# vfmatzkin/ct-unet

Measured on AMD Instinct MI355X. Metric: voxels/sec fwd+bwd, 128^3 fp32 patch, higher is better.
Workload: dtype f32; 1 GPU; UNet() default (1 in, 2 out, i_size 8, 4 blocks), 128^3 patch, batch 1 per GPU, train step = fwd + Dice/CE loss + bwd + grad all-reduce + Adam(amsgrad); patch=128, per_gpu_batch=1, parallelism=dp1, launch=hipgraph

## Files before the change

### ct-unet_amd/csrc/head_loss.hip

```cpp
#include "common.h"
#include "bn_tail.h"

namespace {

constexpr int HB = 256;
constexpr int MAXCO = 4;

struct HeadP {
    const void* in;
    const float* in_scale;
    const float* in_shift;
    const float* w;
    const float* bias;
    const int32_t* imap;
    int in_cs, in_relu, Ci, Co, act, head_mode, N;
    int64_t V;
    float gscale;
    const float* gscale_dev;
};

template <int CP, class T>
__device__ __forceinline__ void head_point(const HeadP& p, const float* sWp, const float* sB, int64_t gv,
                                           float (&a)[CP], float (&lg)[MAXCO], float (&u)[MAXCO],
                                           float (&y)[MAXCO]) {
    const T* src = reinterpret_cast<const T*>(p.in) + (size_t)gv * p.in_cs;
#pragma unroll
    for (int qd = 0; qd < CP / 4; ++qd) {
        float4 v = ld4<T>(src + qd * 4);
        if (p.in_scale) {
            const float4 sc = *reinterpret_cast<const float4*>(p.in_scale + qd * 4);
            const float4 sh = *reinterpret_cast<const float4*>(p.in_shift + qd * 4);
            v = xform4(v, sc, sh, p.in_relu);
        }
        a[qd * 4 + 0] = v.x; a[qd * 4 + 1] = v.y; a[qd * 4 + 2] = v.z; a[qd * 4 + 3] = v.w;
    }
#pragma unroll
    for (int co = 0; co < MAXCO; ++co) {
        float s = 0.f;
        if (co < p.Co) {
#pragma unroll
            for (int c = 0; c < CP; ++c) s = fmaf(a[c], sWp[co * CP + c], s);
            s += sB[co];
        }
        lg[co] = s;
    }
    if (p.act & 1) {
        float mx = -INFINITY;
#pragma unroll
        for (int co = 0; co < MAXCO; ++co) if (co < p.Co) mx = fmaxf(mx, lg[co]);
        float den = 0.f;
#pragma unroll
        for (int co = 0; co < MAXCO; ++co) { u[co] = (co < p.Co) ? expf(lg[co] - mx) : 0.f; den += u[co]; }
#pragma unroll
        for (int co = 0; co < MAXCO; ++co) u[co] /= den;
    } else {
#pragma unroll
        for (int co = 0; co < MAXCO; ++co) u[co] = lg[co];
    }
#pragma unroll
    for (int co = 0; co < MAXCO; ++co) y[co] = (p.act & 2) ? 1.f / (1.f + expf(-u[co])) : u[co];
}

template <int CP>
__device__ __forceinline__ void head_load_weights(const HeadP& p, float* sWp, float* sB) {
    for (int i = threadIdx.x; i < MAXCO * CP; i += blockDim.x) sWp[i] = 0.f;
    if (threadIdx.x < MAXCO) sB[threadIdx.x] = (threadIdx.x < p.Co && p.bias) ? p.bias[threadIdx.x] : 0.f;
    __syncthreads();
    for (int i = threadIdx.x; i < p.Co * p.Ci; i += blockDim.x) {
        const int co = i / p.Ci, ci = i % p.Ci;
        sWp[co * CP + (p.imap ? p.imap[ci] : ci)] = p.w[i];
    }
    __syncthreads();
}

__device__ __forceinline__ void softmax2(float a, float b, float& sa, float& sb) {
    const float mx = fmaxf(a, b);
    const float ea = expf(a - mx), eb = expf(b - mx);
    sa = ea / (ea + eb); sb = eb / (ea + eb);
}

template <int CP, class T>
__global__ __launch_bounds__(HB) void head_fwd_kernel(HeadP p, float* __restrict__ out0, float* __restrict__ out1) {
    __shared__ float sWp[MAXCO * CP];
    __shared__ float sB[MAXCO];
    head_load_weights<CP>(p, sWp, sB);
    const int64_t total = (int64_t)p.N * p.V;
    for (int64_t gv = (int64_t)blockIdx.x * HB + threadIdx.x; gv < total; gv += (int64_t)gridDim.x * HB) {
        float a[CP], lg[MAXCO], u[MAXCO], y[MAXCO];
        head_point<CP, T>(p, sWp, sB, gv, a, lg, u, y);
        const int64_t n = gv / p.V, v = gv % p.V;
        if (p.head_mode == 0) {
#pragma unroll
            for (int co = 0; co < MAXCO; ++co)
                if (co < p.Co) out0[(n * p.Co + co) * p.V + v] = y[co];
        } else {
            float s0 = y[0], s1 = y[1] + y[2], f0 = 1.f - y[1], f1 = y[1];
            if (p.head_mode == 2) {
                softmax2(s0, s1, s0, s1);
                softmax2(f0, f1, f0, f1);
            }
            out0[(n * 2 + 0) * p.V + v] = s0; out0[(n * 2 + 1) * p.V + v] = s1;
            out1[(n * 2 + 0) * p.V + v] = f0; out1[(n * 2 + 1) * p.V + v] = f1;
        }
    }
}

template <int CP, class T>
__global__ __launch_bounds__(HB) void head_bwd_q_kernel(HeadP p, const float* __restrict__ g0,
                                                        const float* __restrict__ g1, T* __restrict__ gin,
                                                        int gin_cs, float* __restrict__ partials,
                                                        const float* __restrict__ bn_mean, const float* __restrict__ bn_invstd,
                                                        int bn_cp, float* __restrict__ bn_partials) {
    constexpr int Q = CP / 4;
    __shared__ float sWp[MAXCO * CP];
    __shared__ float sB[MAXCO];
    __shared__ float sRed[HB / 64][MAXCO * CP + MAXCO + 2 * CP];
    head_load_weights<CP>(p, sWp, sB);
    const int qd = threadIdx.x % Q;
    const float gscale = p.gscale_dev ? p.gscale_dev[0] : p.gscale;
    float wq[MAXCO][4], dw[MAXCO][4], db[MAXCO];
#pragma unroll
    for (int co = 0; co < MAXCO; ++co) {
        db[co] = 0.f;
#pragma unroll
        for (int j = 0; j < 4; ++j) { wq[co][j] = sWp[co * CP + qd * 4 + j]; dw[co][j] = 0.f; }
    }
    float4 sc = make_float4(1.f, 1.f, 1.f, 1.f), sh = make_float4(0.f, 0.f, 0.f, 0.f);
    if (p.in_scale) {
        sc = *reinterpret_cast<const float4*>(p.in_scale + qd * 4);
        sh = *reinterpret_cast<const float4*>(p.in_shift + qd * 4);
    }
    const int xrelu = p.in_scale ? p.in_relu : 0;
    const bool bnq = bn_partials != nullptr && qd * 4 < bn_cp;
    float4 mu = make_float4(0.f, 0.f, 0.f, 0.f), is = mu, r1 = mu, r2 = mu;
    if (bnq) {
        mu = *reinterpret_cast<const float4*>(bn_mean + qd * 4);
        is = *reinterpret_cast<const float4*>(bn_invstd + qd * 4);
    }
    const int64_t total = (int64_t)p.N * p.V;
    constexpr int VPB = HB / Q;
    for (int64_t gv = (int64_t)blockIdx.x * VPB + threadIdx.x / Q; gv < total; gv += (int64_t)gridDim.x * VPB) {
        const float4 raw = ld4<T>(reinterpret_cast<const T*>(p.in) + (size_t)gv * p.in_cs + qd * 4);
        const float4 a = xform4(raw, sc, sh, xrelu);
        float lg[MAXCO], u[MAXCO], y[MAXCO], gy[MAXCO];
#pragma unroll
        for (int co = 0; co < MAXCO; ++co) {
            float s = 0.f;
            if (co < p.Co) {
                s = fmaf(a.w, wq[co][3], fmaf(a.z, wq[co][2], fmaf(a.y, wq[co][1], a.x * wq[co][0])));
#pragma unroll
                for (int o = 1; o < Q; o <<= 1) s += __shfl_xor(s, o);
                s += sB[co];
            }
            lg[co] = s;
        }
        if (p.act & 1) {
            float mx = -INFINITY;
#pragma unroll
            for (int co = 0; co < MAXCO; ++co) if (co < p.Co) mx = fmaxf(mx, lg[co]);
            float den = 0.f;
#pragma unroll
            for (int co = 0; co < MAXCO; ++co) { u[co] = (co < p.Co) ? expf(lg[co] - mx) : 0.f; den += u[co]; }
#pragma unroll
            for (int co = 0; co < MAXCO; ++co) u[co] /= den;
        } else {
#pragma unroll
            for (int co = 0; co < MAXCO; ++co) u[co] = lg[co];
        }
#pragma unroll
        for (int co = 0; co < MAXCO; ++co) y[co] = (p.act & 2) ? 1.f / (1.f + expf(-u[co])) : u[co];
        const int64_t n = gv / p.V, v = gv % p.V;
        if (p.head_mode == 0) {
#pragma unroll
            for (int co = 0; co < MAXCO; ++co) gy[co] = (co < p.Co) ? g0[(n * p.Co + co) * p.V + v] : 0.f;
        } else {
            float a0 = g0[(n * 2 + 0) * p.V + v], a1 = g0[(n * 2 + 1) * p.V + v];
            float b0 = g1[(n * 2 + 0) * p.V + v], b1 = g1[(n * 2 + 1) * p.V + v];
            if (p.head_mode == 2) {
                float s0, s1, f0, f1;
                softmax2(y[0], y[1] + y[2], s0, s1);
                softmax2(1.f - y[1], y[1], f0, f1);
                const float ds = a0 * s0 + a1 * s1, df = b0 * f0 + b1 * f1;
                a0 = s0 * (a0 - ds); a1 = s1 * (a1 - ds);
                b0 = f0 * (b0 - df); b1 = f1 * (b1 - df);
            }
            gy[0] = a0; gy[1] = a1 - b0 + b1; gy[2] = a1; gy[3] = 0.f;
        }
#pragma unroll
        for (int co = 0; co < MAXCO; ++co) gy[co] *= gscale;
        float gu[MAXCO], gl[MAXCO];
#pragma unroll
        for (int co = 0; co < MAXCO; ++co) gu[co] = (p.act & 2) ? gy[co] * y[co] * (1.f - y[co]) : gy[co];
        if (p.act & 1) {
            float dot = 0.f;
#pragma unroll
            for (int co = 0; co < MAXCO; ++co) if (co < p.Co) dot += gu[co] * u[co];
#pragma unroll
            for (int co = 0; co < MAXCO; ++co) gl[co] = (co < p.Co) ? u[co] * (gu[co] - dot) : 0.f;
        } else {
#pragma unroll
            for (int co = 0; co < MAXCO; ++co) gl[co] = (co < p.Co) ? gu[co] : 0.f;
        }
        float4 o = make_float4(0.f, 0.f, 0.f, 0.f);
        const float av[4] = {a.x, a.y, a.z, a.w};
#pragma unroll
        for (int co = 0; co < MAXCO; ++co) {
            o.x = fmaf(gl[co], wq[co][0], o.x); o.y = fmaf(gl[co], wq[co][1], o.y);
            o.z = fmaf(gl[co], wq[co][2], o.z); o.w = fmaf(gl[co], wq[co][3], o.w);
            if (qd == 0) db[co] += gl[co];
#pragma unroll
            for (int j = 0; j < 4; ++j) dw[co][j] = fmaf(gl[co], av[j], dw[co][j]);
        }
        o = rnd4<T>(o);
        st4<T>(gin + (size_t)gv * gin_cs + qd * 4, o);
        if (bnq) {
            float gz;
            gz = (fmaf(raw.x, sc.x, sh.x) > 0.f) ? o.x : 0.f; r1.x += gz; r2.x += gz * (raw.x - mu.x) * is.x;
            gz = (fmaf(raw.y, sc.y, sh.y) > 0.f) ? o.y : 0.f; r1.y += gz; r2.y += gz * (raw.y - mu.y) * is.y;
            gz = (fmaf(raw.z, sc.z, sh.z) > 0.f) ? o.z : 0.f; r1.z += gz; r2.z += gz * (raw.z - mu.z) * is.z;
            gz = (fmaf(raw.w, sc.w, sh.w) > 0.f) ? o.w : 0.f; r1.w += gz; r2.w += gz * (raw.w - mu.w) * is.w;
        }
    }
    const int lane = threadIdx.x & 63, wave = threadIdx.x >> 6;
    if (bn_partials) {
        const float rv[8] = {r1.x, r1.y, r1.z, r1.w, r2.x, r2.y, r2.z, r2.w};
#pragma unroll
        for (int j = 0; j < 8; ++j) {
            float s = rv[j];
#pragma unroll
            for (int o = 32; o >= Q; o >>= 1) s += __shfl_xor(s, o);
            if (lane < Q) sRed[wave][MAXCO * CP + MAXCO + (j >> 2) * CP + lane * 4 + (j & 3)] = s;
        }
    }
#pragma unroll
    for (int co = 0; co < MAXCO; ++co) {
#pragma unroll
        for (int j = 0; j < 4; ++j) {
            float s = dw[co][j];
#pragma unroll
            for (int o = 32; o >= Q; o >>= 1) s += __shfl_xor(s, o);
            if (lane < Q) sRed[wave][co * CP + lane * 4 + j] = s;
        }
        const float s = wave_sum(db[co]);
        if (lane == 0) sRed[wave][MAXCO * CP + co] = s;
    }
    __syncthreads();
    for (int i = threadIdx.x; i < MAXCO * CP + MAXCO; i += HB) {
        float s = 0.f;
#pragma unroll
        for (int w = 0; w < HB / 64; ++w) s += sRed[w][i];
        partials[(size_t)blockIdx.x * (MAXCO * CP + MAXCO) + i] = s;
    }
    if (bn_partials)
        for (int i = threadIdx.x; i < 2 * bn_cp; i += HB) {
            const int col = MAXCO * CP + MAXCO + (i / bn_cp) * CP + i % bn_cp;
            float s = 0.f;
#pragma unroll
            for (int w = 0; w < HB / 64; ++w) s += sRed[w][col];
            bn_partials[(size_t)blockIdx.x * 2 * bn_cp + i] = s;
        }
}

template <int CP>
__global__ __launch_bounds__(HB) void head_bwd_final_kernel(const float* __restrict__ partials, int nb, int Ci, int Co,
                                                            const int32_t* __restrict__ imap, float* __restrict__ dw,
                                                            float* __restrict__ db, const float* __restrict__ bn_partials,
                                                            int bn_cp, ctu_bn_bwd_tail tail) {
    const int i = blockIdx.x;
    if (i == Co * Ci + Co) {
        bn_bwd_finalize_rows(tail, bn_partials, nb, bn_cp);
        return;
    }
    const int row = MAXCO * CP + MAXCO;
    int col;
    if (i < Co * Ci) {
        const int co = i / Ci, ci = i % Ci;
        col = co * CP + (imap ? imap[ci] : ci);
    } else {
        col = MAXCO * CP + (i - Co * Ci);
    }
    __shared__ double r[HB];
    double s = 0.0;
    for (int b = threadIdx.x; b < nb; b += HB) s += (double)partials[(size_t)b * row + col];
    r[threadIdx.x] = s;
    __syncthreads();
    for (int o = HB / 2; o > 0; o >>= 1) {
        if (threadIdx.x < o) r[threadIdx.x] += r[threadIdx.x + o];
        __syncthreads();
    }
    if (threadIdx.x == 0) {
        if (i < Co * Ci) dw[i] = (float)r[0];
        else db[i - Co * Ci] = (float)r[0];
    }
}

inline int head_blocks(int64_t total) {
    int64_t nb = ceil_div64(total, HB);
    if (nb > 2048) nb = 2048;
    return (int)(nb < 1 ? 1 : nb);
}

constexpr int LOSS_BX = 1024;

__global__ __launch_bounds__(HB) void loss_fwd_kernel(const float* __restrict__ pred, const float* __restrict__ tgt,
                                                      int64_t V, int dice_softmax, float* __restrict__ ws) {
    const int n = blockIdx.y;
    const float* p0 = pred + (size_t)n * 2 * V;
    const float* p1 = p0 + V;
    const float* t0 = tgt + (size_t)n * 2 * V;
    const float* t1 = t0 + V;
    float ce = 0.f, num = 0.f, d1 = 0.f, d2 = 0.f;
    auto point = [&](float a, float b, float ta, float tb) {
        const float mx = fmaxf(a, b);
        const float ea = expf(a - mx), eb = expf(b - mx);
        const float lse = mx + logf(ea + eb);
        ce += lse - ((tb > ta) ? b : a);
        float pa = a, pb = b;
        if (dice_softmax) { pa = ea / (ea + eb); pb = eb / (ea + eb); }
        num += pa * ta + pb * tb;
        d1 += pa * pa + pb * pb;
        d2 += ta * ta + tb * tb;
    };
    const bool vec = (V & 3) == 0 && ((reinterpret_cast<uintptr_t>(pred) | reinterpret_cast<uintptr_t>(tgt)) & 15) == 0;
    if (vec) {
        const int64_t V4 = V >> 2;
        for (int64_t q = (int64_t)blockIdx.x * HB + threadIdx.x; q < V4; q += (int64_t)gridDim.x * HB) {
            const float4 a = reinterpret_cast<const float4*>(p0)[q], b = reinterpret_cast<const float4*>(p1)[q];
            const float4 ta = reinterpret_cast<const float4*>(t0)[q], tb = reinterpret_cast<const float4*>(t1)[q];
            point(a.x, b.x, ta.x, tb.x); point(a.y, b.y, ta.y, tb.y); point(a.z, b.z, ta.z, tb.z); point(a.w, b.w, ta.w, tb.w);
        }
    } else {
        for (int64_t v = (int64_t)blockIdx.x * HB + threadIdx.x; v < V; v += (int64_t)gridDim.x * HB) point(p0[v], p1[v], t0[v], t1[v]);
    }
    __shared__ float red[HB / 64][4];
    const int lane = threadIdx.x & 63, wave = threadIdx.x >> 6;
    ce = wave_sum(ce); num = wave_sum(num); d1 = wave_sum(d1); d2 = wave_sum(d2);
    if (lane == 0) { red[wave][0] = ce; red[wave][1] = num; red[wave][2] = d1; red[wave][3] = d2; }
    __syncthreads();
    if (threadIdx.x < 4) {
        float s = 0.f;
#pragma unroll
        for (int w = 0; w < HB / 64; ++w) s += red[w][threadIdx.x];
        ws[((size_t)n * gridDim.x + blockIdx.x) * 4 + threadIdx.x] = s;
    }
}

__global__ void loss_final_kernel(float* __restrict__ ws, int N, int nbx, int64_t V, float ce_lambda,
                                  float dice_lambda, float* __restrict__ terms) {
    if (blockIdx.x != 0) return;
    const int lane = threadIdx.x;
    const double eps = 0.0000001;
    double ce = 0.0, dsum = 0.0;
    float* tail = ws + (size_t)N * nbx * 4;
    for (int n = 0; n < N; ++n) {
        double c = 0.0, num = 0.0, d1 = 0.0, d2 = 0.0;
        for (int b = lane; b < nbx; b += 64) {
            const float4 r = *reinterpret_cast<const float4*>(ws + ((size_t)n * nbx + b) * 4);
            c += r.x; num += r.y; d1 += r.z; d2 += r.w;
        }
#pragma unroll
        for (int o = 32; o > 0; o >>= 1) {
            c += __shfl_xor(c, o); num += __shfl_xor(num, o); d1 += __shfl_xor(d1, o); d2 += __shfl_xor(d2, o);
        }
        ce += c;
        dsum += (num + eps) / (d1 + d2 + eps);
        if (lane == 0) {
            tail[n * 2 + 0] = (float)(num + eps);
            tail[n * 2 + 1] = (float)(d1 + d2 + eps);
        }
    }
    if (lane == 0) {
        terms[0] = ce_lambda != 0.f ? (float)(ce_lambda * ce / ((double)N * (double)V)) : 0.f;
        terms[1] = dice_lambda != 0.f ? (float)(dice_lambda * (1.0 - 2.0 * dsum / N)) : 0.f;
    }
}

__global__ __launch_bounds__(HB) void loss_bwd_kernel(const float* __restrict__ pred, const float* __restrict__ tgt,
                                                      int N, int64_t V, float ce_lambda, float dice_lambda,
                                                      int dice_softmax, const float* __restrict__ tail,
                                                      const float* __restrict__ gscale_ce,
                                                      const float* __restrict__ gscale_dice, float* __restrict__ gpred,
                                                      int accumulate) {
    const int n = blockIdx.y;
    const float gs_ce = gscale_ce ? gscale_ce[0] : 1.f, gs_d = gscale_dice ? gscale_dice[0] : 1.f;
    const float kce = gs_ce * ce_lambda / ((float)N * (float)V);
    const float nume = tail[n * 2 + 0], dene = tail[n * 2 + 1];
    const float kd = gs_d * dice_lambda * (-2.f / (float)N);
    const float kd_t = kd / dene, kd_p = kd * nume * 2.f / (dene * dene);
    const size_t base = (size_t)n * 2 * V;
    auto point = [&](float a, float b, float ta, float tb, float& ga, float& gb) {
        const float mx = fmaxf(a, b);
        const float ea = expf(a - mx), eb = expf(b - mx);
        const float sa = ea / (ea + eb), sb = eb / (ea + eb);
        const bool cls1 = tb > ta;
        ga = kce * (sa - (cls1 ? 0.f : 1.f));
        gb = kce * (sb - (cls1 ? 1.f : 0.f));
        if (dice_lambda != 0.f) {
            const float pa = dice_softmax ? sa : a, pb = dice_softmax ? sb : b;
            float da = kd_t * ta - kd_p * pa, db = kd_t * tb - kd_p * pb;
            if (dice_softmax) {
                const float dot = da * sa + db * sb;
                da = sa * (da - dot); db = sb * (db - dot);
            }
            ga += da; gb += db;
        }
    };
    const bool vec = (V & 3) == 0 && ((reinterpret_cast<uintptr_t>(pred) | reinterpret_cast<uintptr_t>(tgt) | reinterpret_cast<uintptr_t>(gpred)) & 15) == 0;
    if (vec) {
        const int64_t V4 = V >> 2;
        const float4* a4 = reinterpret_cast<const float4*>(pred + base);
        const float4* b4 = reinterpret_cast<const float4*>(pred + base + V);
        const float4* ta4 = reinterpret_cast<const float4*>(tgt + base);
        const float4* tb4 = reinterpret_cast<const float4*>(tgt + base + V);
        float4* ga4 = reinterpret_cast<float4*>(gpred + base);
        float4* gb4 = reinterpret_cast<float4*>(gpred + base + V);
        for (int64_t q = (int64_t)blockIdx.x * HB + threadIdx.x; q < V4; q += (int64_t)gridDim.x * HB) {
            const float4 a = a4[q], b = b4[q], ta = ta4[q], tb = tb4[q];
            float4 ga, gb;
            point(a.x, b.x, ta.x, tb.x, ga.x, gb.x); point(a.y, b.y, ta.y, tb.y, ga.y, gb.y);
            point(a.z, b.z, ta.z, tb.z, ga.z, gb.z); point(a.w, b.w, ta.w, tb.w, ga.w, gb.w);
            if (accumulate) {
                const float4 oa = ga4[q], ob = gb4[q];
                ga.x += oa.x; ga.y += oa.y; ga.z += oa.z; ga.w += oa.w; gb.x += ob.x; gb.y += ob.y; gb.z += ob.z; gb.w += ob.w;
            }
            ga4[q] = ga; gb4[q] = gb;
        }
        return;
    }
    for (int64_t v = (int64_t)blockIdx.x * HB + threadIdx.x; v < V; v += (int64_t)gridDim.x * HB) {
        float ga, gb;
        point(pred[base + v], pred[base + V + v], tgt[base + v], tgt[base + V + v], ga, gb);
        if (accumulate) { ga += gpred[base + v]; gb += gpred[base + V + v]; }
        gpred[base + v] = ga;
        gpred[base + V + v] = gb;
    }
}

}

static int fill_head(HeadP& p, const void* in, int in_cs, int cin_p, const float* in_scale, const float* in_shift,
                     int in_relu, const float* w, const float* bias, const int32_t* imap, int Ci, int Co, int act,
                     int head_mode, int N, int64_t V, const char* name) {
    CTU_REQUIRE(in && w, "%s: null pointer", name);
    CTU_REQUIRE(cin_p == 8 || cin_p == 16 || cin_p == 32, "%s: cin_p=%d unsupported (8, 16 or 32)", name, cin_p);
    CTU_REQUIRE(Co >= 1 && Co <= MAXCO && Ci >= 1 && Ci <= cin_p, "%s: Co=%d Ci=%d", name, Co, Ci);
    CTU_REQUIRE(head_mode == 0 || Co == 3, "%s: SP re-encoding needs 3 output channels", name);
    CTU_REQUIRE(head_mode >= 0 && head_mode <= 2, "%s: head_mode=%d", name, head_mode);
    CTU_REQUIRE(in_cs >= cin_p && in_cs % 4 == 0, "%s: bad stride", name);
    CTU_REQUIRE((in_scale == nullptr) == (in_shift == nullptr), "%s: scale/shift must come together", name);
    p.in = in; p.in_scale = in_scale; p.in_shift = in_shift; p.w = w; p.bias = bias; p.imap = imap;
    p.in_cs = in_cs; p.in_relu = in_relu; p.Ci = Ci; p.Co = Co; p.act = act; p.head_mode = head_mode; p.N = N; p.V = V; p.gscale = 1.f;
    p.gscale_dev = nullptr;
    return CTU_OK;
}

namespace {

template <class T>
int head_fwd_impl(const T* in, int in_cs, int cin_p, const float* in_scale, const float* in_shift, int in_relu, const float* w,
                  const float* bias, const int32_t* imap, int Ci, int Co, int act, int head_mode, float* out0, float* out1, int N,
                  int64_t nvox_per_item, void* stream) {
    HeadP p;
    int rc = fill_head(p, in, in_cs, cin_p, in_scale, in_shift, in_relu, w, bias, imap, Ci, Co, act, head_mode, N,
                       nvox_per_item, "head_fwd");
    if (rc != CTU_OK) return rc;
    CTU_REQUIRE(out0 && (head_mode == 0 || out1), "head_fwd: null output");
    const int nb = head_blocks((int64_t)N * nvox_per_item);
    hipStream_t st = (hipStream_t)stream;
    if (cin_p == 8) head_fwd_kernel<8, T><<<nb, HB, 0, st>>>(p, out0, out1);
    else if (cin_p == 16) head_fwd_kernel<16, T><<<nb, HB, 0, st>>>(p, out0, out1);
    else head_fwd_kernel<32, T><<<nb, HB, 0, st>>>(p, out0, out1);
    CTU_CHECK_LAUNCH("head_fwd");
    return CTU_OK;
}

template <class T>
int head_bwd_impl(const T* in, int in_cs, int cin_p, const float* in_scale, const float* in_shift, int in_relu, const float* w,
                  const float* bias, const int32_t* imap, int Ci, int Co, int act, int head_mode, const float* g0, const float* g1,
                  T* gin, int gin_cs, float* dw, float* db, float* ws, int N, int64_t nvox_per_item, const float* bn_mean,
                  const float* bn_invstd, int bn_cp, float* bn_partials, const ctu_bn_bwd_tail* tail, void* stream, float gscale = 1.f,
                  const float* gscale_dev = nullptr) {
    CTU_REQUIRE(!tail || (bn_partials && tail->gamma && tail->invstd && tail->dgamma && tail->dbeta && tail->coef &&
                          tail->C > 0 && tail->C <= bn_cp && tail->count > 0 && (!tail->running_mean || (tail->mean && tail->running_var))),
                "head_bwd: incomplete BatchNorm tail");
    HeadP p;
    int rc = fill_head(p, in, in_cs, cin_p, in_scale, in_shift, in_relu, w, bias, imap, Ci, Co, act, head_mode, N,
                       nvox_per_item, "head_bwd");
    if (rc != CTU_OK) return rc;
    p.gscale = gscale;
    p.gscale_dev = gscale_dev;
    CTU_REQUIRE(g0 && (head_mode == 0 || g1) && gin && dw && db && ws, "head_bwd: null pointer");
    CTU_REQUIRE(gin_cs >= cin_p && gin_cs % 4 == 0, "head_bwd: bad gin stride");
    CTU_REQUIRE(!bn_partials || (bn_mean && bn_invstd && in_scale && in_relu && bn_cp > 0 && bn_cp % 4 == 0 && bn_cp <= cin_p),
                "head_bwd: the BatchNorm reduction needs mean/invstd, a BN+ReLU input transform and bn_cp <= cin_p (bn_cp=%d)", bn_cp);
    const int nb = head_blocks((int64_t)N * nvox_per_item);
    hipStream_t st = (hipStream_t)stream;
    const int nfin = Co * Ci + Co + (tail ? 1 : 0);
    const ctu_bn_bwd_tail tl = bwd_tail_or_off(tail);
    if (cin_p == 8) {
        head_bwd_q_kernel<8, T><<<nb, HB, 0, st>>>(p, g0, g1, gin, gin_cs, ws, bn_mean, bn_invstd, bn_cp, bn_partials);
        head_bwd_final_kernel<8><<<nfin, HB, 0, st>>>(ws, nb, Ci, Co, imap, dw, db, bn_partials, bn_cp, tl);
    } else if (cin_p == 16) {
        head_bwd_q_kernel<16, T><<<nb, HB, 0, st>>>(p, g0, g1, gin, gin_cs, ws, bn_mean, bn_invstd, bn_cp, bn_partials);
        head_bwd_final_kernel<16><<<nfin, HB, 0, st>>>(ws, nb, Ci, Co, imap, dw, db, bn_partials, bn_cp, tl);
    } else {
        head_bwd_q_kernel<32, T><<<nb, HB, 0, st>>>(p, g0, g1, gin, gin_cs, ws, bn_mean, bn_invstd, bn_cp, bn_partials);
        head_bwd_final_kernel<32><<<nfin, HB, 0, st>>>(ws, nb, Ci, Co, imap, dw, db, bn_partials, bn_cp, tl);
    }
    CTU_CHECK_LAUNCH("head_bwd");
    return CTU_OK;
}

}

extern "C" int ctu_head_fwd(const float* in, int in_cs, int cin_p, const float* in_scale, const float* in_shift,
                            int in_relu, const float* w, const float* bias, const int32_t* imap, int Ci, int Co, int act,
                            int head_mode, float* out0, float* out1, int N, int64_t nvox_per_item, void* stream) {
    return head_fwd_impl<float>(in, in_cs, cin_p, in_scale, in_shift, in_relu, w, bias, imap, Ci, Co, act, head_mode, out0, out1, N,
                                nvox_per_item, stream);
}
extern "C" int ctu_lp_head_fwd(int dtype, const void* in, int in_cs, int cin_p, const float* in_scale, const float* in_shift,
                               int in_relu, const float* w, const float* bias, const int32_t* imap, int Ci, int Co, int act,
                               int head_mode, float* out0, float* out1, int N, int64_t nvox_per_item, void* stream) {
    CTU_DISPATCH_LP(dtype, return head_fwd_impl<T>((const T*)in, in_cs, cin_p, in_scale, in_shift, in_relu, w, bias, imap, Ci, Co, act,
                                                   head_mode, out0, out1, N, nvox_per_item, stream));
}

extern "C" size_t ctu_head_bwd_ws_floats(int N, int64_t nvox_per_item, int cin_p, int Co) {
    (void)Co;
    return (size_t)head_blocks((int64_t)N * nvox_per_item) * (MAXCO * cin_p + MAXCO);
}

extern "C" int ctu_head_bwd_num_blocks(int N, int64_t nvox_per_item) { return head_blocks((int64_t)N * nvox_per_item); }

extern "C" int ctu_head_bwd(const float* in, int in_cs, int cin_p, const float* in_scale, const float* in_shift,
                            int in_relu, const float* w, const float* bias, const int32_t* imap, int Ci, int Co, int act,
                            int head_mode, const float* g0, const float* g1, float* gin, int gin_cs, float* dw,
                            float* db, float* ws, int N, int64_t nvox_per_item, void* stream) {
    return head_bwd_impl<float>(in, in_cs, cin_p, in_scale, in_shift, in_relu, w, bias, imap, Ci, Co, act, head_mode, g0, g1, gin,
                                gin_cs, dw, db, ws, N, nvox_per_item, nullptr, nullptr, 0, nullptr, nullptr, stream);
}

extern "C" int ctu_head_bwd_bn(const float* in, int in_cs, int cin_p, const float* in_scale, const float* in_shift,
                               int in_relu, const float* w, const float* bias, const int32_t* imap, int Ci, int Co, int act,
                               int head_mode, const float* g0, const float* g1, float* gin, int gin_cs, float* dw,
                               float* db, float* ws, int N, int64_t nvox_per_item, const float* bn_mean,
                               const float* bn_invstd, int bn_cp, float* bn_partials, const ctu_bn_bwd_tail* tail, void* stream) {
    return head_bwd_impl<float>(in, in_cs, cin_p, in_scale, in_shift, in_relu, w, bias, imap, Ci, Co, act, head_mode, g0, g1, gin,
                                gin_cs, dw, db, ws, N, nvox_per_item, bn_mean, bn_invstd, bn_cp, bn_partials, tail, stream);
}
extern "C" int ctu_lp_head_bwd_bn(int dtype, const void* in, int in_cs, int cin_p, const float* in_scale, const float* in_shift,
                                  int in_relu, const float* w, const float* bias, const int32_t* imap, int Ci, int Co, int act,
                                  int head_mode, const float* g0, const float* g1, void* gin, int gin_cs, float* dw,
                                  float* db, float* ws, int N, int64_t nvox_per_item, const float* bn_mean,
                                  const float* bn_invstd, int bn_cp, float* bn_partials, const ctu_bn_bwd_tail* tail, float gscale,
                                  void* stream) {
    CTU_DISPATCH_LP(dtype, return head_bwd_impl<T>((const T*)in, in_cs, cin_p, in_scale, in_shift, in_relu, w, bias, imap, Ci, Co, act,
                                                   head_mode, g0, g1, (T*)gin, gin_cs, dw, db, ws, N, nvox_per_item, bn_mean,
                                                   bn_invstd, bn_cp, bn_partials, tail, stream, gscale));
}

extern "C" int ctu_lp_head_bwd_bn_dscale(int dtype, const void* in, int in_cs, int cin_p, const float* in_scale,
                                         const float* in_shift, int in_relu, const float* w, const float* bias, const int32_t* imap,
                                         int Ci, int Co, int act, int head_mode, const float* g0, const float* g1, void* gin,
                                         int gin_cs, float* dw, float* db, float* ws, int N, int64_t nvox_per_item,
                                         const float* bn_mean, const float* bn_invstd, int bn_cp, float* bn_partials,
                                         const ctu_bn_bwd_tail* tail, const float* gscale, void* stream) {
    CTU_REQUIRE(gscale, "lp_head_bwd_bn_dscale: null gscale");
    CTU_DISPATCH_LP(dtype, return head_bwd_impl<T>((const T*)in, in_cs, cin_p, in_scale, in_shift, in_relu, w, bias, imap, Ci, Co, act,
                                                   head_mode, g0, g1, (T*)gin, gin_cs, dw, db, ws, N, nvox_per_item, bn_mean,
                                                   bn_invstd, bn_cp, bn_partials, tail, stream, 1.f, gscale));
}

extern "C" size_t ctu_loss_ws_floats(int N, int64_t V) {
    (void)V;
    return (size_t)N * LOSS_BX * 4 + (size_t)N * 2;
}

extern "C" int ctu_loss_fwd(const float* pred, const float* target, int N, int64_t V, float ce_lambda,
                            float dice_lambda, int dice_softmax, float* terms, float* ws, void* stream) {
    CTU_REQUIRE(pred && target && terms && ws && N > 0 && V > 0, "loss_fwd: bad argument");
    hipStream_t st = (hipStream_t)stream;
    loss_fwd_kernel<<<dim3(LOSS_BX, N), HB, 0, st>>>(pred, target, V, dice_softmax, ws);
    CTU_CHECK_LAUNCH("loss_fwd");
    loss_final_kernel<<<1, 64, 0, st>>>(ws, N, LOSS_BX, V, ce_lambda, dice_lambda, terms);
    CTU_CHECK_LAUNCH("loss_final");
    return CTU_OK;
}

extern "C" int ctu_loss_bwd(const float* pred, const float* target, int N, int64_t V, float ce_lambda,
                            float dice_lambda, int dice_softmax, const float* ws, const float* gscale_ce,
                            const float* gscale_dice, float* gpred, int accumulate, void* stream) {
    CTU_REQUIRE(pred && target && ws && gpred && N > 0 && V > 0, "loss_bwd: bad argument");
    loss_bwd_kernel<<<dim3(LOSS_BX, N), HB, 0, (hipStream_t)stream>>>(pred, target, N, V, ce_lambda, dice_lambda,
                                                                      dice_softmax, ws + (size_t)N * LOSS_BX * 4,
                                                                      gscale_ce, gscale_dice, gpred, accumulate);
    CTU_CHECK_LAUNCH("loss_bwd");
    return CTU_OK;
}
```

### ct-unet_amd/ctunet_amd/_lib.py

```python
from __future__ import annotations

import ctypes as C
import os

import torch

_HERE = os.path.dirname(os.path.abspath(__file__))
LIB_PATH = os.environ.get("CTUNET_HIP_LIB") or os.path.join(_HERE, "libctunet_hip.so")

P = C.c_void_p
I = C.c_int
L = C.c_int64
F = C.c_float
D = C.c_double
Z = C.c_size_t
U = C.c_uint64

class PackJob(C.Structure):
    _fields_ = [("w", C.c_void_p), ("wp", C.c_void_p), ("cinv", C.c_void_p), ("kind", C.c_int), ("Co", C.c_int),
                ("Ci", C.c_int), ("k", C.c_int), ("rin_p", C.c_int), ("nout_p", C.c_int), ("mode", C.c_int),
                ("layout", C.c_int)]


class BnTail(C.Structure):
    _fields_ = [("gamma", C.c_void_p), ("beta", C.c_void_p), ("running_mean", C.c_void_p), ("running_var", C.c_void_p),
                ("scale", C.c_void_p), ("shift", C.c_void_p), ("mean", C.c_void_p), ("invstd", C.c_void_p),
                ("num_batches_tracked", C.c_void_p), ("counter", C.c_void_p), ("count", C.c_double),
                ("momentum", C.c_float), ("eps", C.c_float), ("C", C.c_int), ("n_updates", C.c_int)]


class BnBwdTail(C.Structure):
    _fields_ = [("gamma", C.c_void_p), ("invstd", C.c_void_p), ("dgamma", C.c_void_p), ("dbeta", C.c_void_p),
                ("coef", C.c_void_p), ("mean", C.c_void_p), ("running_mean", C.c_void_p), ("running_var", C.c_void_p),
                ("num_batches_tracked", C.c_void_p), ("counter", C.c_void_p), ("count", C.c_double),
                ("momentum", C.c_float), ("eps", C.c_float), ("C", C.c_int)]


class WgradJob(C.Structure):
    _fields_ = [("ws", C.c_void_p), ("dw", C.c_void_p), ("db", C.c_void_p), ("cinv", C.c_void_p), ("kind", C.c_int),
                ("Co", C.c_int), ("Ci", C.c_int), ("cin_p", C.c_int), ("n_ci_g", C.c_int), ("gx", C.c_int),
                ("pairs", C.c_int), ("nmf", C.c_int)]


class SegLossCfg(C.Structure):
    _fields_ = [("ce_lambda", C.c_float), ("dice_lambda", C.c_float), ("tversky_lambda", C.c_float),
                ("boundary_lambda", C.c_float), ("w0", C.c_float), ("w1", C.c_float), ("focal_gamma", C.c_float),
                ("tversky_alpha", C.c_float), ("tversky_beta", C.c_float), ("dice_softmax", C.c_int)]


WGRAD_JOBS_MAX = 4

SIGNATURES = {
    "ctu_last_error": (C.c_char_p, []),
    "ctu_abi_version": (I, []),
    "ctu_arch": (C.c_char_p, []),
    "ctu_ncdhw_to_ndhwc": (I, [P, P, I, I, I, I, I, I, I, P]),
    "ctu_ndhwc_to_ncdhw": (I, [P, P, I, I, I, I, I, I, P]),
    "ctu_conv3d_layout": (I, [I, I, I]),
    "ctu_conv3d_fwd_kernel_name": (C.c_char_p, [I, I, I, I, I, I, I]),
    "ctu_conv3d_wgrad_kernel_name": (C.c_char_p, [I, I, I, I]),
    "ctu_conv3d_packed_floats": (Z, [I, I, I, I]),
    "ctu_conv3d_num_blocks": (I, [I, I, I, I, I, I, I]),
    "ctu_pack_conv3d_weight": (I, [P, P, I, I, I, P, I, I, I, I, P]),
    "ctu_pack_batch": (I, [P, I, P]),
    "ctu_conv3d_fwd": (I, [P, I, I, P, P, I, P, P, I, P, I, I, P, I, I, I, I, I, I, P, P]),
    "ctu_conv3d_wgrad_ws_floats": (Z, [I, I, I, I, I, I, I]),
    "ctu_conv3d_wgrad": (I, [P, I, I, P, P, I, P, I, I, P, P, I, I, P, P, I, I, I, I, I, P]),
    "ctu_conv3d_wgrad_bn_supported": (I, [I, I, I, I, I, I, I]),
    "ctu_conv3d_wgrad_bn": (I, [P, I, I, P, P, I, P, I, I, P, P, P, P, P, P, I, I, P, P, I, I, I, I, I, P]),
    "ctu_conv3d_first_supported": (I, [I, I, I, I]),
    "ctu_conv3d_first_num_blocks": (I, [I, I, I, I]),
    "ctu_conv3d_first_fwd": (I, [P, I, P, P, I, P, I, I, P, I, I, I, I, P, P]),
    "ctu_conv3d_first_bwd_data": (I, [P, I, P, I, I, P, I, I, I, I, P]),
    "ctu_conv3d_first_wgrad_ws_floats": (Z, [I, I, I, I, I]),
    "ctu_conv3d_first_wgrad": (I, [P, I, P, I, P, I, P, I, I, I, I, P]),
    "ctu_conv3d_first_wgrad_bn": (I, [P, I, P, I, P, P, P, P, P, P, I, P, I, I, I, I, P]),
    "ctu_bn_finalize": (I, [P, I, I, I, D, P, P, P, P, F, F, I, P, P, P, P, P, P]),
    "ctu_bn_eval_affine": (I, [P, P, P, P, F, I, I, P, P, P]),
    "ctu_bn_bwd_num_blocks": (I, [L]),
    "ctu_bn_relu_bwd_reduce": (I, [P, I, P, I, I, P, P, P, P, L, P, P, P]),
    "ctu_bn_bwd_finalize": (I, [P, I, I, I, D, P, P, P, P, P, P, P, P, F, F, P, P]),
    "ctu_bn_relu_bwd_apply": (I, [P, I, P, I, I, P, P, P, P, P, L, P]),
    "ctu_conv3d_wgrad_slabs": (I, [P, I, I, P, P, I, P, I, I, P, P, I, I, P, P, I, I, I, I, I, P, P]),
    "ctu_conv3d_wgrad_bn_slabs": (I, [P, I, I, P, P, I, P, I, I, P, P, P, P, P, P, I, I, P, P, I, I, I, I, I, P, P]),
    "ctu_conv3d_first_wgrad_slabs": (I, [P, I, P, I, P, I, P, I, I, I, I, P, P]),
    "ctu_conv3d_first_wgrad_bn_slabs": (I, [P, I, P, I, P, P, P, P, P, P, I, P, I, I, I, I, P, P]),
    "ctu_convt2_wgrad_slabs": (I, [P, I, I, P, P, I, P, I, I, P, P, I, I, P, P, I, I, I, I, P, P]),
    "ctu_bn_bwd_finalize_jobs": (I, [P, I, I, I, D, P, P, P, P, P, P, P, P, F, F, P, P, I, P]),
    "ctu_wgrad_reduce_jobs": (I, [P, I, P]),
    "ctu_maxpool2_fwd": (I, [P, I, I, P, P, I, P, I, I, I, I, I, P]),
    "ctu_maxpool2_bwd": (I, [P, I, I, P, P, I, P, I, P, I, I, I, I, I, I, P]),
    "ctu_maxpool2_bwd_bn_num_blocks": (I, [I, I, I, I, I]),
    "ctu_maxpool2_bwd_bn": (I, [P, I, I, P, P, P, P, P, I, P, I, I, I, I, I, I, P, P, P]),
    "ctu_convt_packed_floats": (Z, [I, I]),
    "ctu_pack_convt_weight": (I, [P, P, I, I, P, I, I, I, P]),
    "ctu_convt2_fwd": (I, [P, I, I, P, P, I, P, P, I, P, I, I, I, I, I, I, P]),
    "ctu_convt2_bwd_data": (I, [P, I, I, P, P, I, I, I, I, I, I, P]),
    "ctu_convt2_wgrad_ws_floats": (Z, [I, I, I, I, I, I]),
    "ctu_convt2_wgrad": (I, [P, I, I, P, P, I, P, I, I, P, P, I, I, P, P, I, I, I, I, P]),
    "ctu_convt2_plan": (C.c_char_p, [I, I, I, I, I, I, I, P]),
    "ctu_convt2_wgrad_plan": (C.c_char_p, [I, I, I, I, I, I, P]),
    "ctu_head_fwd": (I, [P, I, I, P, P, I, P, P, P, I, I, I, I, P, P, I, L, P]),
    "ctu_head_bwd_ws_floats": (Z, [I, L, I, I]),
    "ctu_head_bwd": (I, [P, I, I, P, P, I, P, P, P, I, I, I, I, P, P, P, I, P, P, P, I, L, P]),
    "ctu_head_bwd_num_blocks": (I, [I, L]),
    "ctu_head_bwd_bn": (I, [P, I, I, P, P, I, P, P, P, I, I, I, I, P, P, P, I, P, P, P, I, L, P, P, I, P, P, P]),
    "ctu_loss_ws_floats": (Z, [I, L]),
    "ctu_loss_fwd": (I, [P, P, I, L, F, F, I, P, P, P]),
    "ctu_loss_bwd": (I, [P, P, I, L, F, F, I, P, P, P, P, I, P]),
    "ctu_seg_loss_ws_floats": (Z, [I, L]),
    "ctu_seg_loss_fwd": (I, [P, P, P, I, L, P, P, P, P]),
    "ctu_seg_loss_bwd": (I, [P, P, P, I, L, P, P, P, P, P, P, P, I, P]),
    "ctu_skip_add": (I, [P, I, P, P, I, P, I, P, P, I, P, I, I, L, P]),
    "ctu_upconv_fused_supported": (I, [I, I, I, I, I, I]),
    "ctu_upconv_fused_packed_floats": (Z, [I, I]),
    "ctu_upconv_fused_num_blocks": (I, [I, I, I, I, I]),
    "ctu_upconv_fused_pack_ws_floats": (Z, [I, I]),
    "ctu_upconv_fused_pack": (I, [P, P, P, I, I, P, I, I, P, P, P, P]),
    "ctu_upconv_fused_pack_all": (I, [P, P, P, I, I, P, I, I, P, P, P, P, P]),
    "ctu_upconv_fused_fwd": (I, [P, I, I, P, P, I, P, P, P, I, I, P, I, I, I, I, P, P]),
    "ctu_upconv_fused_wgrad_ws_floats": (Z, [I, I, I, I, I, I]),
    "ctu_upconv_fused_wgrad": (I, [P, I, I, P, P, I, P, I, I, P, P, I, I, I, I, P]),
    "ctu_upconv_fused_wgrad_bn_supported": (I, [I, I, I, I, I, I]),
    "ctu_upconv_fused_wgrad_bn": (I, [P, I, I, P, P, I, P, I, I, P, P, P, P, P, P, P, I, I, I, I, P]),
    "ctu_upconv_fused_project_ws_floats": (Z, [I, L]),
    "ctu_upconv_fused_project": (I, [P, P, I, I, I, I, I, I, P, P, P, I, I, I, P, P, P, P, P]),
    "ctu_upconv_fused_bwd_packed_floats": (Z, [I, I]),
    "ctu_upconv_fused_pack_bwd": (I, [P, I, I, P, P]),
    "ctu_upconv_fused_bwd_data": (I, [P, I, I, P, P, I, I, I, I, I, I, P]),
    "ctu_hard_segm": (I, [P, I, I, L, P, P]),
    "ctu_one_hot": (I, [P, I, I, L, P, P]),
    "ctu_hard_dice_ws_doubles": (Z, [I]),
    "ctu_hard_dice_counts": (I, [P, P, I, I, L, P, P, P]),
    "ctu_hausdorff_ws_bytes": (Z, [I, I, I, I, I]),
    "ctu_hausdorff": (I, [P, P, I, I, I, I, I, P, P, P]),
    "ctu_surface_ws_bytes": (Z, [I, I, I, I, I]),
    "ctu_surface_metrics": (I, [P, I, I, P, I, I, I, I, I, I, I, I, I, P, P, D, P, P, P]),
    "ctu_components_ws_bytes": (Z, [I, I, I, I]),
    "ctu_label_components": (I, [P, I, I, I, I, I, I, P, I, P, P, P, P]),
    "ctu_filter_components": (I, [P, I, I, I, I, I, I, P, I, I, I, P, P, P]),
    "ctu_morphology_ws_bytes": (Z, [I, I, I, I, I]),
    "ctu_binary_morphology": (I, [P, I, I, I, I, I, I, C.c_uint32, I, I, I, L, P, P, P]),
    "ctu_fill_holes": (I, [P, I, I, I, I, I, I, I, L, P, P, P]),
    "ctu_implant_mask": (I, [P, I, P, I, I, I, I, I, C.c_uint32, I, I, I, I, P, P, P]),
    "ctu_distance_ws_bytes": (Z, [I, I, I, I, I, I]),
    "ctu_distance_transform": (I, [P, I, I, I, I, I, I, L, I, I, P, I, P, P, F, P, P]),
    "ctu_thickness_ws_bytes": (Z, [I, I, I, I, I]),
    "ctu_local_thickness": (I, [P, I, I, I, I, I, P, P, P, P]),
    "ctu_thickness_summary_ws_bytes": (Z, [I, L]),
    "ctu_thickness_summary": (I, [P, I, L, F, P, P, P]),
    "ctu_resample": (I, [P, I, I, I, L, I, I, I, I, I, I, P, P, P, P, P]),
    "ctu_affine_resample": (I, [P, I, I, I, L, I, I, I, I, I, I, P, P, P, P, P, D, P, P]),
    "ctu_registration_ws_bytes": (Z, [L]),
    "ctu_registration_init": (I, [P, L, P, P, P]),
    "ctu_registration_accumulate": (I, [P, L, P, I, I, I, P, P, D, P, P]),
    "ctu_registration_update": (I, [L, I, P, P, P, I, P, P]),
    "ctu_mesh_ws_bytes": (Z, [I, I, I]),
    "ctu_mesh_count": (I, [P, I, I, I, I, I, L, F, P, P]),
    "ctu_mesh_emit": (I, [P, I, I, I, I, F, F, P, P, L, L, P, P, P, P]),
    "ctu_mesh_measure": (I, [P, L, P, L, P, P, P, P]),
    "ctu_mesh_adjacency_ws_bytes": (Z, [L, L]),
    "ctu_mesh_adjacency_build": (I, [P, L, L, P, P, P]),
    "ctu_mesh_adjacency_emit": (I, [L, L, L, P, P, P, P]),
    "ctu_mesh_smooth_ws_bytes": (Z, [L]),
    "ctu_mesh_smooth": (I, [P, L, P, P, L, P, I, F, I, F, P, P, P]),
    "ctu_mesh_voxelize_ws_bytes": (Z, [I, I, I]),
    "ctu_mesh_voxelize": (I, [P, L, P, L, I, I, I, P, P, I, P, P, P]),
    "ctu_mesh_grid_ws_bytes": (Z, [L, L]),
    "ctu_mesh_grid_build": (I, [P, L, P, L, F, L, P, P, P]),
    "ctu_mesh_grid_emit": (I, [P, L, L, L, L, P, P, P, P]),
    "ctu_mesh_distance": (I, [P, L, P, P, L, P, I, I, I, P, L, I, I, I, P, P, F, F, P, P, P, P]),
    "ctu_mesh_decimate_ws_bytes": (Z, [L, L, L]),
    "ctu_mesh_decimate_bounds": (I, [P, L, P, L, P, P]),
    "ctu_mesh_decimate_build": (I, [P, L, P, L, P, P, P, L, I, P, P]),
    "ctu_mesh_decimate_emit": (I, [P, L, L, L, L, P, P, P, P, P, P, P]),
    "ctu_gaussian_ws_bytes": (Z, [L, I, I, I, I]),
    "ctu_gaussian_filter": (I, [P, I, L, I, I, I, P, P, I, F, P, P, P]),
    "ctu_minmax_ws_bytes": (Z, [L]),
    "ctu_finite_minmax": (I, [P, I, L, P, P, P]),
    "ctu_histogram": (I, [P, I, L, I, P, D, D, P, P]),
    "ctu_threshold_otsu": (I, [P, I, P, D, D, P, P, P]),
    "ctu_binarize": (I, [P, I, L, P, D, P, D, P, P]),
    "ctu_extract_patches": (I, [P, P, I, I, I, I, I, I, I, I, P, P]),
    "ctu_stitch_patches": (I, [P, P, I, I, I, I, I, I, I, I, P, P]),
    "ctu_window_accumulate": (I, [P, P, P, P, I, I, I, I, I, I, I, I, P, P, P, F, I, I, I, P, P, P]),
    "ctu_window_finalize": (I, [P, P, I, L, P, P, P]),
    "ctu_extract_patches_flip": (I, [P, P, P, I, I, I, I, I, I, I, I, P, P]),
    "ctu_window_accumulate_flip": (I, [P, P, P, P, P, I, I, I, I, I, I, I, I, P, P, P, F, I, I, I, P, P, P, P, P]),
    "ctu_window_finalize_stats": (I, [P, P, P, P, I, L, P, P, P, P, P, P]),
    "ctu_flap_count": (I, [P, I, I, L, P, P]),
    "ctu_flap_draw": (I, [P, I, I, I, I, I, P, I, P, U, F, I, I, I, P, P, U, F, F, I, P, P]),
    "ctu_flap_apply": (I, [P, I, P, I, I, I, I, P, I, P, P, P, U, I, P, I, P, P, P]),
    "ctu_spatial_draw": (I, [I, I, I, I, P, P, U, I, D, D, D, P, I, I, I, I, P, P, P]),
    "ctu_spatial_warp": (I, [P, I, I, I, I, I, I, P, I, I, I, P, P, P, P, P]),
    "ctu_lp_upconv_fused_supported": (I, [I, I, I, I, I, I]),
    "ctu_lp_upconv_fused_packed_elems": (Z, [I]),
    "ctu_lp_upconv_fused_num_blocks": (I, [I, I, I, I]),
    "ctu_lp_upconv_fused_pack": (I, [I, P, I, P, P]),
    "ctu_lp_upconv_fused_fwd": (I, [I, P, I, I, P, P, I, P, P, P, I, P, I, I, I, I, P]),
    "ctu_lp_upconv_fused_wgrad_ws_floats": (Z, [I, I, I, I, I]),
    "ctu_lp_upconv_fused_wgrad": (I, [I, P, I, I, P, P, I, P, I, P, P, I, I, I, I, P]),
    "ctu_lp_upconv_fused_wgrad_bn_supported": (I, [I, I, I, I, I]),
    "ctu_lp_upconv_fused_wgrad_bn": (I, [I, P, I, I, P, P, I, P, I, P, P, P, P, P, P, P, I, I, I, I, P]),
    "ctu_lp_conv3d_wgrad_bn_supported": (I, [I, I, I, I, I, I, I]),
    "ctu_lp_conv3d_wgrad_bn": (I, [I, P, I, I, P, P, I, P, I, I, P, P, P, P, P, P, I, I, P, P, I, I, I, I, I, P]),
    "ctu_lp_upconv_fused_project": (I, [I, P, P, I, I, I, I, I, I, P, P, P, I, I, I, P, P, P, P, P]),
    "ctu_lp_upconv_fused_bwd_data": (I, [I, P, I, P, P, I, I, I, I, I, I, P]),
    "ctu_lp_conv3d_layout": (I, [I, I, I, I]),
    "ctu_lp_conv3d_packed_elems": (Z, [I, I, I]),
    "ctu_lp_conv3d_num_blocks": (I, [I, I, I, I, I, I, I, I]),
    "ctu_lp_pack_conv3d_weight": (I, [I, P, P, I, I, I, P, I, I, I, I, P]),
    "ctu_lp_pack_batch": (I, [I, P, I, P]),
    "ctu_lp_conv3d_fwd": (I, [I, P, I, I, P, P, I, P, P, I, P, I, I, P, I, I, I, I, I, I, P, P]),
    "ctu_lp_conv3d_wgrad_ws_floats": (Z, [I, I, I, I, I, I, I]),
    "ctu_lp_conv3d_wgrad": (I, [I, P, I, I, P, P, I, P, I, I, P, I, I, P, P, I, I, I, I, I, P]),
    "ctu_lp_conv3d_first_fwd": (I, [I, P, I, P, P, I, P, I, I, P, I, I, I, I, P, P]),
    "ctu_lp_conv3d_first_bwd_data": (I, [I, P, I, P, I, I, P, I, I, I, I, P]),
    "ctu_lp_conv3d_first_bwd_data_pair_supported": (I, [I, I]),
    "ctu_lp_conv3d_fwd_kernel_name": (C.c_char_p, [I, I, I, I, I, I, I, I]),
    "ctu_lp_conv3d_wgrad_kernel_name": (C.c_char_p, [I, I, I, I, I, I]),
    "ctu_lp_conv3d_first_bwd_data_pair": (I, [I, P, I, P, I, P, I, I, I, I, P]),
    "ctu_lp_conv3d_first_wgrad": (I, [I, P, I, P, I, P, I, P, I, I, I, I, P]),
    "ctu_lp_convt_packed_elems": (Z, [I, I, I]),
    "ctu_lp_pack_convt_weight": (I, [I, P, P, I, I, P, I, I, I, P]),
    "ctu_lp_convt2_fwd": (I, [I, P, I, I, P, P, I, P, P, I, P, I, I, I, I, I, I, P]),
    "ctu_lp_convt2_bwd_data": (I, [I, P, I, I, P, P, I, I, I, I, I, I, P]),
    "ctu_lp_convt2_wgrad_ws_floats": (Z, [I, I, I, I, I, I]),
    "ctu_lp_convt2_wgrad": (I, [I, P, I, I, P, P, I, P, I, I, P, I, I, P, P, I, I, I, I, P]),
    "ctu_lp_convt2_plan": (C.c_char_p, [I, I, I, I, I, I, I, P]),
    "ctu_lp_convt2_wgrad_plan": (C.c_char_p, [I, I, I, I, I, I, P]),
    "ctu_lp_ncdhw_to_ndhwc": (I, [I, P, P, I, I, I, I, I, I, I, P]),
    "ctu_lp_ndhwc_to_ncdhw": (I, [I, P, P, I, I, I, I, I, I, P]),
    "ctu_lp_bn_relu_bwd_reduce": (I, [I, P, I, P, I, I, P, P, P, P, L, P, P, P]),
    "ctu_lp_bn_relu_bwd_apply": (I, [I, P, I, P, I, I, P, P, P, P, P, L, P]),
    "ctu_lp_maxpool2_fwd": (I, [I, P, I, I, P, P, I, P, I, I, I, I, I, P]),
    "ctu_lp_maxpool2_bwd": (I, [I, P, I, I, P, P, I, P, I, P, I, I, I, I, I, I, P]),
    "ctu_lp_maxpool2_bwd_bn": (I, [I, P, I, I, P, P, P, P, P, I, P, I, I, I, I, I, I, P, P, P]),
    "ctu_lp_skip_add": (I, [I, P, I, P, P, I, P, I, P, P, I, P, I, I, L, P]),
    "ctu_lp_channel_sum": (I, [I, P, I, I, L, P, P, I, P]),
    "ctu_lp_head_fwd": (I, [I, P, I, I, P, P, I, P, P, P, I, I, I, I, P, P, I, L, P]),
    "ctu_lp_head_bwd_bn": (I, [I, P, I, I, P, P, I, P, P, P, I, I, I, I, P, P, P, I, P, P, P, I, L, P, P, I, P, P, F, P]),
    "ctu_lp_head_bwd_bn_dscale": (I, [I, P, I, I, P, P, I, P, P, P, I, I, I, I, P, P, P, I, P, P, P, I, L, P, P, I, P, P, P, P]),
    "ctu_scale_tensors": (I, [P, P, I, F, P, P]),
    "ctu_unscale_tensors": (I, [P, P, I, P, P, P]),
    "ctu_loss_scale_update": (I, [P, P, P, P, F, F, I, P]),
    "ctu_comm_available": (I, []),
    "ctu_comm_unique_id": (I, [P]),
    "ctu_comm_init": (I, [C.POINTER(C.c_void_p), I, I, P]),
    "ctu_comm_allreduce_f32": (I, [P, P, P, Z, I, P]),
    "ctu_comm_destroy": (I, [P]),
    "ctu_channel_sum_num_blocks": (I, [L]),
    "ctu_channel_sum": (I, [P, I, I, L, P, P, I, P]),
    "ctu_adam_amsgrad": (I, [P, P, I, P, D, D, D, D, D, I, P, P]),
    "ctu_adam_amsgrad_dev": (I, [P, P, I, P, P, D, D, D, D, I, P, P, P]),
    "ctu_grad_norm_num_blocks": (I, [P, I]),
    "ctu_grad_clip_coef": (I, [P, P, I, F, P, P, P, P]),
    "ctu_plateau_update": (I, [P, P, P, P, I, I, D, I, D, I, D, D, P]),
    "ctu_sgd": (I, [P, P, I, P, P, D, D, D, D, I, I, P, P, P]),
    "ctu_rmsprop": (I, [P, P, I, P, P, D, D, D, D, D, I, I, P, P, P]),
}

_lib = None
ABI_VERSION = 8


class CtuError(RuntimeError):
    """A libctunet_hip.so entry point returned a non-zero status."""


def load() -> C.CDLL:
    global _lib
    if _lib is not None:
        return _lib
    if not os.path.exists(LIB_PATH):
        raise ImportError(
            f"{LIB_PATH} not found: the MI355X kernels are not built. Run `python __graft_entry__.py` "
            "(or `make -C ct-unet_amd/csrc`). There is no CPU fallback for this path.")
    lib = C.CDLL(LIB_PATH)
    for name, (res, args) in SIGNATURES.items():
        try:
            fn = getattr(lib, name)
        except AttributeError as e:
            raise ImportError(f"{LIB_PATH} does not export {name}; rebuild the library") from e
        fn.restype = res
        fn.argtypes = args
    if lib.ctu_abi_version() != ABI_VERSION:
        raise ImportError(f"{LIB_PATH} is ABI v{lib.ctu_abi_version()}, this package binds v{ABI_VERSION}: "
                          "a stale build -- run `python __graft_entry__.py` (or `make -C ct-unet_amd/csrc`)")
    _lib = lib
    return lib


def check(status: int, what: str) -> None:
    if status != 0:
        msg = load().ctu_last_error().decode("utf-8", "replace")
        raise CtuError(f"{what} failed (status {status}): {msg}")


DTYPE_CODE = {torch.float32: 0, torch.uint8: 3, torch.bool: 3, torch.int64: 4, torch.int16: 5, torch.int32: 6}


class on(torch.cuda.device):

    def __init__(self, device: torch.device):
        super().__init__(device.index)

    def __enter__(self):
        super().__enter__()
        self._stream = torch.cuda.current_stream().cuda_stream
        return self._run

    def _run(self, name: str, *args, what: str = None) -> None:
        status = getattr(_lib or load(), name)(*args, self._stream)
        if status:
            check(status, what or name[4:])


def check_device(message: str, *tensors) -> None:
    for t in tensors:
        if not t.is_cuda:
            raise ValueError(message)


def as_bytes(t):
    t = t.contiguous()
    return t.view(torch.uint8) if t.dtype == torch.bool else t


def array(ctype, values):
    if values is None:
        return None
    values = list(values)
    return (ctype * len(values))(*values)


def float_array(values):
    return array(C.c_float, values)


def double_array(values):
    return array(C.c_double, values)
```

### ct-unet_amd/ctunet_amd/engine.py

```python
from __future__ import annotations

import os
from dataclasses import dataclass
from typing import Dict, List, Optional, Tuple

import torch

from . import ops
from .ops import CL, pad8

BN_EPS = 1e-5
FUSE_UP = os.environ.get("CTUNET_FUSE_UP", "1") != "0"
FUSE_UP_MAX_CO = int(os.environ.get("CTUNET_FUSE_UP_MAXCO", "16"))
POOL_BN = os.environ.get("CTUNET_POOL_BN", "1") != "0"
LP_FUSE_UP = os.environ.get("CTUNET_LP_FUSE_UP", "1") != "0"
BN_MOMENTUM = 0.1
LAZY_BN = os.environ.get("CTUNET_LAZY_BN", "1") != "0"
LAZY_BN_LP = os.environ.get("CTUNET_LAZY_BN_LP", "0") != "0"
BN_TAIL = os.environ.get("CTUNET_BN_TAIL", "0") != "0"
DEFER_WGRAD_REDUCE = os.environ.get("CTUNET_DEFER_WGRAD_REDUCE", "1") != "0"


@dataclass
class BlockPlan:
    prefix: str
    first: int
    cin: int
    cout: int


@dataclass
class NetPlan:
    k: int
    conv_bias: bool
    in_ch: int
    out_ch: int
    enc: List[BlockPlan]
    center: BlockPlan
    center_live: bool
    dec: List[BlockPlan]
    head: str
    act: int
    head_mode: int
    skip: str = "cat"


@dataclass(slots=True)
class _ConvRec:
    x: Optional[CL]
    y: CL
    vec: torch.Tensor
    stats: Optional[torch.Tensor]
    nblk: int
    conv: str
    bn: str
    cin: int
    cout: int
    imap: Optional[torch.Tensor]
    bias: bool
    first: Optional[torch.Tensor] = None


class _WgradWs:

    def __init__(self, floats: int, device, defer: bool):
        self.jobs = ops.WgradJobs() if defer else None
        self.bufs = [torch.empty(floats, dtype=torch.float32, device=device) for _ in range(2 if defer else 1)]
        self.i = 0

    def take(self) -> torch.Tensor:
        self.i = (self.i + 1) % len(self.bufs)
        ws = self.bufs[self.i]
        if self.jobs is not None:
            if self.jobs.uses(ws):
                self.jobs.flush()
            assert not self.jobs.uses(ws)
        return ws

    def flush(self) -> None:
        if self.jobs is not None:
            self.jobs.flush()


class UNetEngine:
    def __init__(self, plan: NetPlan, dtype: torch.dtype = torch.float32, loss_scale: Optional[float] = None):
        if dtype not in ops.ACT_DTYPES:
            raise ValueError(f"ctunet_amd: activation dtype {dtype} not supported (float32, bfloat16, float16)")
        self.plan = plan
        self.dtype = dtype
        self.loss_scale = loss_scale
        self.scaler = None
        self._pack_cache: Dict[Tuple, Tuple[int, torch.Tensor]] = {}
        self._replay_stats = False
        self._up_cache: Dict[str, Tuple] = {}
        self._imaps: Dict[Tuple, torch.Tensor] = {}
        self._tail_words: Dict[str, torch.Tensor] = {}
        self._tail_slots: Dict[Tuple[str, str], int] = {}
        self._overflow: Dict[str, torch.Tensor] = {}
        self._gy_bufs: Dict[int, Tuple[torch.Tensor, torch.Tensor]] = {}

    def overflow_flag(self, device) -> torch.Tensor:
        f = self._overflow.get(str(device))
        if f is None:
            f = self._overflow[str(device)] = torch.zeros(1, dtype=torch.float32, device=device)
        return f

    def _counter(self, layer: str, direction: str, device) -> Optional[torch.Tensor]:
        if not BN_TAIL:
            return None
        words = self._tail_words.get(str(device))
        if words is None:
            words = self._tail_words[str(device)] = torch.zeros(1024, dtype=torch.int32, device=device)
        slot = self._tail_slots.setdefault((layer, direction), len(self._tail_slots))
        if slot >= words.numel():
            raise RuntimeError("ctunet_amd: more than 1024 BatchNorm tails in one engine")
        return words[slot:slot + 1]

    def _maps(self, segs: Tuple[Tuple[int, int], ...], cp: int, device):
        idx: List[int] = []
        for n, start in segs:
            idx += list(range(start, start + n))
        if idx == list(range(len(idx))):
            return None, None
        key = (segs, cp, str(device))
        t = self._imaps.get(key)
        if t is None:
            inv = [-1] * cp
            for logical, pos in enumerate(idx):
                inv[pos] = logical
            t = (torch.tensor(idx, dtype=torch.int32, device=device), torch.tensor(inv, dtype=torch.int32, device=device))
            self._imaps[key] = t
        return t

    def _packed(self, name: str, w: torch.Tensor, kind: str, imap, rin_p: int, nout_p: int, mode: int,
                layout: int = 0) -> torch.Tensor:
        key = (name, kind, mode, rin_p, nout_p, layout, self.dtype)
        hit = self._pack_cache.get(key)
        ver = (w._version, w.data_ptr())
        if hit is not None and hit[0] == ver:
            return hit[1]
        wd = w.detach()
        if self.dtype != torch.float32:
            wp = self._pack_lp(kind, wd, imap, rin_p, nout_p, mode, hit[1] if hit is not None else None, layout)
        else:
            wp = hit[1] if hit is not None else torch.empty(ops.packed_floats(kind, w.shape[2], rin_p, nout_p, layout),
                                                            dtype=torch.float32, device=w.device)
            ops.pack_batch([(kind, wd.contiguous(), wp, imap, rin_p, nout_p, mode, layout)], self.dtype)
        self._pack_cache[key] = (ver, wp, imap)
        return wp

    def _pack_lp(self, kind, wd, imap, rin_p, nout_p, mode, into, layout=0):
        if kind == "conv":
            return ops.pack_conv_w_lp(wd, imap, rin_p, nout_p, mode, self.dtype, into, layout)
        return ops.pack_convt_w_lp(wd, imap, rin_p, nout_p, mode, self.dtype, into)

    def refresh_packs(self, P: Dict[str, torch.Tensor]) -> None:
        force = P and next(iter(P.values())).is_cuda and torch.cuda.is_current_stream_capturing()
        jobs = []
        for key, ent in self._pack_cache.items():
            name, kind, mode, rin_p, nout_p, layout, dt = key
            w = P.get(name + ".weight")
            if w is None or w.device != ent[1].device or dt != self.dtype:
                continue
            ver = (w._version, w.data_ptr())
            if force or ent[0] != ver:
                jobs.append((kind, w.detach().contiguous(), ent[1], ent[2], rin_p, nout_p, mode, layout))
                self._pack_cache[key] = (ver, ent[1], ent[2])
        ops.pack_batch(jobs, self.dtype)

    def invalidate_packs(self) -> None:
        for key, ent in self._pack_cache.items():
            self._pack_cache[key] = (None,) + tuple(ent[1:])
        for prefix, hit in self._up_cache.items():
            self._up_cache[prefix] = (None,) + tuple(hit[1:])

    def _fwd_tail(self, P, bn: str, c: int, nvox: int, n_upd: int, vec4: torch.Tensor, device):
        counter = self._counter(bn, "fwd", device)
        if counter is None:
            return None
        return ops.make_bn_tail(c, nvox, P[bn + ".weight"], P[bn + ".bias"], P[bn + ".running_mean"], P[bn + ".running_var"],
                                BN_MOMENTUM, BN_EPS, n_upd, vec4, P.get(bn + ".num_batches_tracked") if n_upd else None,
                                counter)

    def _bn_stage(self, P, bn: str, out: CL, vec4: torch.Tensor, nvox: int, c: int, training: bool, n_upd: int, nblk: int,
                  launch, tail_ok: bool = True) -> Tuple[CL, Optional[torch.Tensor]]:
        wb = (P[bn + ".weight"], P[bn + ".bias"], P[bn + ".running_mean"], P[bn + ".running_var"])
        if training:
            stats = torch.empty((nblk, 2, out.cp), dtype=torch.float32, device=out.buf.device)
            tail = self._fwd_tail(P, bn, c, nvox, n_upd, vec4, out.buf.device) if tail_ok else None
            launch(stats, tail)
            if tail is None:
                ops.bn_finalize_into(stats, nblk, c, out.cp, nvox, *wb, BN_MOMENTUM, BN_EPS, n_upd, vec4,
                                     P.get(bn + ".num_batches_tracked") if n_upd else None)
        else:
            stats = None
            launch(None, None)
            ops.bn_eval_affine_into(*wb, BN_EPS, c, out.cp, vec4)
        return out.with_xf(vec4[0], vec4[1], True), stats

    def _conv_bn(self, P, x: CL, conv: str, bn: str, cin: int, cout: int, imap, out: CL, vec4: torch.Tensor,
                 training: bool, n_upd: int, save: bool) -> Tuple[CL, Optional[_ConvRec]]:
        k = self.plan.k
        w = P[conv + ".weight"]
        bias = P.get(conv + ".bias")
        lay = ops.conv_layout(k, out.cp, x.dims[3], self.dtype, x.cp)
        if bias is not None and self.dtype != torch.float32:
            lay = 0
        wp = self._packed(conv, w, "conv", imap, x.cp, out.cp, 0, lay)
        bias_p = None if bias is None else bias.detach()
        nblk = ops.conv_num_blocks(x.dims, out.cp, lay, k, self.dtype, x.cp) if training else 0
        y, stats = self._bn_stage(P, bn, out, vec4, x.nvox, cout, training, n_upd, nblk,
                                  lambda stats, tail: ops.conv3d_fwd(x, wp, bias_p, out, k, stats, (cin, cout), lay, tail))
        rec = _ConvRec(x, out.raw(), vec4, stats, nblk, conv, bn, cin, cout, imap, bias is not None) if save else None
        return y, rec

    def _fuse_up(self, x: CL, nout_p: int) -> bool:
        if not (self.plan.k == 3 and not self.plan.conv_bias and nout_p <= FUSE_UP_MAX_CO and FUSE_UP):
            return False
        if self.dtype == torch.float32:
            return ops.upconv_fused_supported(x.dims, 3, x.cp, nout_p)
        return LP_FUSE_UP and ops.lp_upconv_fused_supported(x.dims, 3, x.cp, nout_p)

    def _upconv_bn(self, P, x: CL, prefix: str, ct: int, cout: int, cinv, out: CL, vec4: torch.Tensor, training: bool,
                   n_upd: int, save: bool) -> Tuple[CL, Optional[_ConvRec]]:
        conv, bn = f"{prefix}.1", f"{prefix}.2"
        wt, bt, w3 = P[f"{prefix}.0.weight"], P[f"{prefix}.0.bias"], P[conv + ".weight"]
        lp = bool(x.lp)
        ver = tuple((t._version, t.data_ptr()) for t in (wt, bt, w3))
        hit = self._up_cache.get(prefix)
        if hit is None or hit[0] != ver or hit[3] != (x.cp, out.cp, self.dtype) or torch.cuda.is_current_stream_capturing():
            same = hit is not None and hit[3] == (x.cp, out.cp, self.dtype)
            if lp:
                wp, beff, pws = ops.upconv_fused_pack(wt, bt, w3, cinv, x.cp, out.cp, (hit[1], hit[2], hit[4]) if same else None)
                wpd = ops.lp_upconv_fused_pack(wp, x.cp, self.dtype, hit[5] if same else None)
            else:
                wp, beff, pws, wpd = ops.upconv_fused_pack_all(wt, bt, w3, cinv, x.cp, out.cp,
                                                               (hit[1], hit[2], hit[4], hit[5]) if same else None)
            self._up_cache[prefix] = (ver, wp, beff, (x.cp, out.cp, self.dtype), pws, wpd)
        else:
            wp, beff, wpd = hit[1], hit[2], hit[5]
        if lp:
            nblk = ops.lp_upconv_fused_num_blocks(x.dims) if training else 0
            launch = lambda stats, tail: ops.lp_upconv_fused_fwd(x, wpd, beff, out, stats, (ct, cout))
        else:
            nblk = ops.upconv_fused_num_blocks(x.dims, out.cp) if training else 0
            launch = lambda stats, tail: ops.upconv_fused_fwd(x, wp, beff, out, stats, (ct, cout), tail)
        y, stats = self._bn_stage(P, bn, out, vec4, 8 * x.nvox, cout, training, n_upd, nblk, launch, tail_ok=not lp)
        rec = _ConvRec(None, out.raw(), vec4, stats, nblk, conv, bn, ct, cout, None, False) if save else None
        return y, rec

    def _first_conv_bn(self, P, x: torch.Tensor, conv: str, bn: str, cin: int, cout: int, out: CL, vec4: torch.Tensor,
                       training: bool, n_upd: int, save: bool):
        w = P[conv + ".weight"].detach()
        bias = P.get(conv + ".bias")
        bias_p = None if bias is None else bias.detach()
        nblk = ops.conv_first_num_blocks(out.dims) if training else 0
        y, stats = self._bn_stage(P, bn, out, vec4, out.nvox, cout, training, n_upd, nblk,
                                  lambda stats, tail: ops.conv_first_fwd(x, w, bias_p, out, stats, tail))
        rec = _ConvRec(None, out.raw(), vec4, stats, nblk, conv, bn, cin, cout, None, bias is not None, x) if save else None
        return y, rec

    def forward(self, P: Dict[str, torch.Tensor], x: torch.Tensor, training: bool, save: bool, chk: bool):
        plan = self.plan
        dev = x.device
        n, cin, d, h, w = x.shape
        nlev = len(plan.enc)
        if cin != plan.in_ch:
            raise RuntimeError(f"ctunet_amd: expected {plan.in_ch} input channels, got {cin}")
        if any(s % (1 << nlev) for s in (d, h, w)):
            raise RuntimeError(f"ctunet_amd: spatial size {(d, h, w)} must be divisible by {1 << nlev}")
        if training and n * (d >> nlev) * (h >> nlev) * (w >> nlev) <= 1:
            raise ValueError("Expected more than 1 value per channel when training (centre block)")
        ctx = {"recs": {}, "levels": [], "training": training, "chk": chk} if save else None
        n_upd = 1 if training else 0
        self.refresh_packs(P)

        x = x.contiguous()
        e0 = plan.enc[0]
        first_direct = plan.conv_bias is False and ops.conv_first_supported(plan.k, cin, pad8(e0.cout), w)
        adt = self.dtype
        cur = None if first_direct else ops.ncdhw_to_cl(x, dtype=adt)
        x_cl = cur
        cat: List[torch.Tensor] = []
        xf: List[torch.Tensor] = []
        pooled: List[CL] = []
        dskip: List[CL] = []
        dd, hh, ww = d, h, w
        recs = {}
        xf_sizes = [8 * pad8(blk.cout) for blk in plan.enc]
        xf_all = torch.zeros(sum(xf_sizes), dtype=torch.float32, device=dev)
        xf_off = 0
        for i, blk in enumerate(plan.enc):
            cp = pad8(blk.cout)
            cat.append(torch.empty((n, dd, hh, ww, 2 * cp), dtype=adt, device=dev))
            xf.append(xf_all[xf_off:xf_off + 8 * cp].view(4, 2 * cp))
            xf_off += 8 * cp
            t1 = CL(torch.empty((n, dd, hh, ww, cp), dtype=adt, device=dev), 0, cp)
            v1 = torch.empty((4, cp), dtype=torch.float32, device=dev)
            imap = None
            if i == 0 and first_direct:
                a1, recs[(blk.prefix, 1)] = self._first_conv_bn(P, x, f"{blk.prefix}.{blk.first}",
                                                                f"{blk.prefix}.{blk.first + 1}", blk.cin, blk.cout, t1,
                                                                v1, training, n_upd, save)
            else:
                a1, recs[(blk.prefix, 1)] = self._conv_bn(P, cur, f"{blk.prefix}.{blk.first}",
                                                          f"{blk.prefix}.{blk.first + 1}", blk.cin, blk.cout, imap, t1,
                                                          v1, training, n_upd, save)
            a2, recs[(blk.prefix, 2)] = self._conv_bn(P, a1, f"{blk.prefix}.{blk.first + 3}", f"{blk.prefix}.{blk.first + 4}",
                                                      blk.cout, blk.cout, None, CL(cat[i], cp, cp), xf[i][:, cp:],
                                                      training, n_upd, save)
            dskip.append(a2)
            dd, hh, ww = dd // 2, hh // 2, ww // 2
            pl = CL(torch.empty((n, dd, hh, ww, cp), dtype=adt, device=dev), 0, cp)
            ops.maxpool_fwd(a2, pl)
            pooled.append(pl)
            cur = pl
        cb = plan.center
        cpc = pad8(cb.cout)
        center_out = None
        if plan.center_live or training:
            live = plan.center_live
            c1 = CL(torch.empty((n, dd, hh, ww, cpc), dtype=adt, device=dev), 0, cpc)
            c2 = CL(torch.empty((n, dd, hh, ww, cpc), dtype=adt, device=dev), 0, cpc)
            v1 = torch.empty((4, cpc), dtype=torch.float32, device=dev)
            v2 = torch.empty((4, cpc), dtype=torch.float32, device=dev)
            a1, r1 = self._conv_bn(P, cur, f"{cb.prefix}.{cb.first}", f"{cb.prefix}.{cb.first + 1}", cb.cin, cb.cout,
                                   None, c1, v1, training, n_upd, save and live)
            a2, r2 = self._conv_bn(P, a1, f"{cb.prefix}.{cb.first + 3}", f"{cb.prefix}.{cb.first + 4}", cb.cout, cb.cout,
                                   None, c2, v2, training, n_upd, save and live)
            if live:
                recs[(cb.prefix, 1)], recs[(cb.prefix, 2)] = r1, r2
                center_out = a2
        cur = center_out if plan.center_live else pooled[-1]
        cur_segs = ((cb.cout if plan.center_live else plan.enc[-1].cout, 0),)
        dec_in: List[CL] = []
        ups: List[CL] = []
        for j, blk in enumerate(plan.dec):
            i = nlev - 1 - j
            cp = pad8(blk.cout)
            dd, hh, ww = dd * 2, hh * 2, ww * 2
            ct = blk.cin
            ctp = pad8(ct)
            imap_t, cinv_t = self._maps(cur_segs, cur.cp, dev)
            wt = P[f"{blk.prefix}.0.weight"]
            dec_in.append(cur)
            t1 = CL(torch.empty((n, dd, hh, ww, cp), dtype=adt, device=dev), 0, cp)
            v1 = torch.empty((4, cp), dtype=torch.float32, device=dev)
            if self._fuse_up(cur, cp):
                ups.append(None)
                a1, recs[(blk.prefix, 1)] = self._upconv_bn(P, cur, blk.prefix, ct, blk.cout, cinv_t, t1, v1, training,
                                                            n_upd, save)
            else:
                up = CL(torch.empty((n, dd, hh, ww, ctp), dtype=adt, device=dev), 0, ctp)
                wpt = self._packed(f"{blk.prefix}.0", wt, "convt", cinv_t, cur.cp, ctp, 0)
                ops.convt_fwd(cur, wpt, P[f"{blk.prefix}.0.bias"].detach(), up)
                ups.append(up)
                a1, recs[(blk.prefix, 1)] = self._conv_bn(P, up, f"{blk.prefix}.1", f"{blk.prefix}.2", ct, blk.cout, None,
                                                          t1, v1, training, n_upd, save)
            a2, recs[(blk.prefix, 2)] = self._conv_bn(P, a1, f"{blk.prefix}.4", f"{blk.prefix}.5", blk.cout, blk.cout, None,
                                                      CL(cat[i], 0, cp), xf[i][:, :cp], training, n_upd, save)
            if plan.skip == "cat":
                cur = CL(cat[i], 0, 2 * cp, xf[i][0], xf[i][1], True)
                cur_segs = ((blk.cout, 0), (blk.cout, cp))
            elif plan.skip == "none":
                cur = CL(cat[i], 0, cp, xf[i][0][:cp], xf[i][1][:cp], True)
                cur_segs = ((blk.cout, 0),)
            else:
                cur = CL(torch.empty((n, dd, hh, ww, cp), dtype=adt, device=dev), 0, cp)
                ops.skip_add(CL(cat[i], 0, cp, xf[i][0][:cp], xf[i][1][:cp], True),
                             CL(cat[i], cp, cp, xf[i][0][cp:], xf[i][1][cp:], True), cur)
                cur_segs = ((blk.cout, 0),)
        imap_h, _ = self._maps(cur_segs, cur.cp, dev)
        wl, bl = P[plan.head + ".weight"], P[plan.head + ".bias"]
        w2 = wl.detach().reshape(wl.shape[0], wl.shape[1])
        out0, out1 = ops.head_fwd(cur, w2, bl.detach(), imap_h, plan.act, plan.head_mode)
        if save:
            ctx.update(recs=recs, x_cl=x_cl, cat=cat, xf=xf, pooled=pooled, dskip=dskip, dec_in=dec_in, ups=ups,
                       head_in=cur, imap_h=imap_h, center_out=center_out, dims=(n, d, h, w))
        return out0, out1, ctx

    def _replay(self, P, rec: _ConvRec):
        return ((P[rec.bn + ".running_mean"], P[rec.bn + ".running_var"], BN_MOMENTUM, BN_EPS,
                 P.get(rec.bn + ".num_batches_tracked")) if self._replay_stats else None)

    def _bwd_fin(self, P, rec: _ConvRec, device):
        counter = self._counter(rec.bn, "bwd", device)
        return None if counter is None else (P[rec.bn + ".weight"].detach(), rec.cout, self._replay(P, rec), counter)

    def _gy_like(self, ga: CL) -> CL:
        ent = self._gy_bufs.get(id(ga.buf))
        if ent is None:
            ent = self._gy_bufs[id(ga.buf)] = (ga.buf, torch.empty_like(ga.buf))
        return CL(ent[1], ga.c0, ga.cp)

    def _conv_bn_bwd(self, P, rec: _ConvRec, ga: CL, gin: Optional[CL], grads: Dict[str, torch.Tensor], ws: _WgradWs, part,
                     pre_reduced: Optional[int] = None, finalized=None, up_in: Optional[CL] = None):
        k = self.plan.k
        can = LAZY_BN and ga.cs == rec.y.cs and (not ga.lp or LAZY_BN_LP)
        if up_in is not None:
            lazy = can and (ops.lp_upconv_fused_wgrad_bn_supported(up_in.dims, up_in.cp) if ga.lp else
                            ops.upconv_fused_wgrad_bn_supported(up_in.dims, up_in.cp, ga.cp))
        elif rec.first is not None:
            lazy = can and not rec.bias and not ga.lp
        else:
            lazy = can and not rec.bias and rec.x is not None and ops.conv3d_wgrad_bn_supported(ga.dims, k, rec.x.cp, ga.cp, self.dtype)
        jobs = ws.jobs
        res = ops.bn_relu_bwd(rec.y, ga, rec.vec, P[rec.bn + ".weight"].detach(), rec.cout, part, self._replay(P, rec),
                              pre_reduced, self._counter(rec.bn, "bwd", ga.buf.device), finalized, lazy, jobs)
        grads[rec.bn + ".weight"], grads[rec.bn + ".bias"] = res[0], res[1]
        if up_in is not None:
            return (rec.y, rec.vec, res[2], self._gy_like(ga)) if lazy else None
        if rec.first is not None:
            if lazy:
                gy = self._gy_like(ga)
                grads[rec.conv + ".weight"] = ops.conv_first_wgrad_bn(rec.first, ga, rec.y, rec.vec, res[2], gy, rec.cout,
                                                                      ws.take(), jobs)
                ga = gy
            else:
                grads[rec.conv + ".weight"] = ops.conv_first_wgrad(rec.first, ga, rec.cout, ws.take(), jobs)
            return ops.conv_first_bwd_data(ga, P[rec.conv + ".weight"].detach(), rec.cin) if gin is not None else None
        if lazy:
            gy = self._gy_like(ga)
            grads[rec.conv + ".weight"] = ops.conv3d_wgrad_bn(rec.x, ga, rec.y, rec.vec, res[2], gy, rec.cout, rec.cin, k,
                                                             rec.imap, ws.take(), jobs)
            ga = gy
        elif rec.x is not None:
            dw, dbias = ops.conv3d_wgrad(rec.x, ga, rec.cout, rec.cin, k, rec.imap, ws.take(), rec.bias, jobs)
            grads[rec.conv + ".weight"] = dw
            if rec.bias:
                grads[rec.conv + ".bias"] = dbias
        if gin is not None:
            lay = ops.conv_layout(k, gin.cp, ga.dims[3], self.dtype, ga.cp)
            wpd = self._packed(rec.conv, P[rec.conv + ".weight"], "conv", rec.imap, ga.cp, gin.cp, 1, lay)
            ops.conv3d_fwd(ga, wpd, None, gin, k, None, (rec.cout, rec.cin), lay)

    def backward(self, P: Dict[str, torch.Tensor], ctx, g0: torch.Tensor, g1: Optional[torch.Tensor],
                 need_dx: bool, sync=None):
        plan = self.plan
        recs = ctx["recs"]
        n, d, h, w = ctx["dims"]
        dev = g0.device
        nlev = len(plan.enc)
        gs = 1.0
        flag = None
        dyn = self.scaler if self.dtype == torch.float16 else None
        if dyn is not None:
            dyn.prepare(dev, n * d * h * w)
            flag = dyn.found_inf
        elif self.dtype == torch.float16:
            gs = self.loss_scale if self.loss_scale else float(2 ** max(0, (n * d * h * w).bit_length() - 5))
            flag = self.overflow_flag(dev)
            flag.zero_()
        grads: Dict[str, torch.Tensor] = {}
        emitted: set = set()
        self._gy_bufs = {}

        def unscale(tensors):
            if dyn is not None:
                ops.unscale_tensors(tensors, dyn.scale, flag)
            elif gs != 1.0:
                ops.scale_tensors(tensors, 1.0 / gs, flag)

        def emit():
            new = [(nm, g) for nm, g in grads.items() if nm not in emitted and g is not None]
            emitted.update(nm for nm, _ in new)
            if sync is not None or dyn is not None or gs != 1.0:
                ws.flush()
            unscale([g for _, g in new])
            if sync is not None:
                sync.push(new)
        k = plan.k
        ws_n, part_n = 1, 1
        for r in recs.values():
            if r is None:
                continue
            if r.first is not None:
                ws_n = max(ws_n, ops.conv_first_wgrad_ws(r.y.dims, r.cin))
                part_n = max(part_n, ops.bn_bwd_partials_floats(r.y.nvox, r.y.cp))
                continue
            ws_n = max(ws_n, ops.conv3d_wgrad_ws(r.y.dims, k, r.x.cp if r.x is not None else pad8(r.cin), r.y.cp, self.dtype))
            part_n = max(part_n, ops.bn_bwd_partials_floats(r.y.nvox, r.y.cp))
        for x_in, blk in zip(ctx["dec_in"], plan.dec):
            ws_n = max(ws_n, ops.convt_wgrad_ws(x_in.dims, x_in.cp, pad8(blk.cin), self.dtype))
        for dsk in ctx["dskip"]:
            part_n = max(part_n, ops.maxpool_bwd_bn_blocks(dsk.dims, dsk.cp) * 2 * dsk.cp)
        part_n = max(part_n, ops.head_bwd_blocks(ctx["head_in"].dims) * 2 * pad8(plan.dec[-1].cout))
        ws = _WgradWs(ws_n, dev, DEFER_WGRAD_REDUCE and self.dtype == torch.float32 and ops.TIMER is None)
        part = torch.empty(part_n, dtype=torch.float32, device=dev)

        self._replay_stats = bool(ctx["training"] and ctx["chk"])

        cat, head_in = ctx["cat"], ctx["head_in"]
        gcat = [torch.empty_like(c) for c in cat]
        wl, bl = P[plan.head + ".weight"], P[plan.head + ".bias"]
        w2 = wl.detach().reshape(wl.shape[0], wl.shape[1])
        gsd = None if dyn is None else dyn.scale
        def g_skip_target(level: int) -> CL:
            full = gcat[level].shape[-1]
            return CL(gcat[level], 0, full if plan.skip == "cat" else full // 2)

        def g_skip_fanout(level: int):
            if plan.skip == "add":
                half = gcat[level].shape[-1] // 2
                ops.skip_add(CL(gcat[level], 0, half), None, CL(gcat[level], half, half))

        r_last = recs[(plan.dec[-1].prefix, 2)]
        head_rows, head_fin = None, None
        if (POOL_BN and head_in.scale is not None and head_in.relu and head_in.scale.data_ptr() == r_last.vec[0].data_ptr()
                and head_in.c0 == r_last.y.c0 and head_in.buf is r_last.y.buf):
            fin = self._bwd_fin(P, r_last, head_in.buf.device)
            res = ops.head_bwd(head_in, w2, bl.detach(), ctx["imap_h"], plan.act, plan.head_mode, g0.contiguous(),
                               None if g1 is None else g1.contiguous(), g_skip_target(0), (r_last.vec, part), fin, gscale=gs,
                               gscale_dev=gsd)
            dwl, dbl, head_rows = res[:3]
            head_fin = res[3] if fin is not None else None
        else:
            dwl, dbl = ops.head_bwd(head_in, w2, bl.detach(), ctx["imap_h"], plan.act, plan.head_mode, g0.contiguous(),
                                    None if g1 is None else g1.contiguous(), g_skip_target(0), gscale=gs,
                                    gscale_dev=gsd)
        g_skip_fanout(0)
        grads[plan.head + ".weight"], grads[plan.head + ".bias"] = dwl.reshape(wl.shape), dbl
        emit()

        g_deep: Optional[CL] = None
        for j in range(nlev - 1, -1, -1):
            blk = plan.dec[j]
            i = nlev - 1 - j
            cp = pad8(blk.cout)
            r1, r2 = recs[(blk.prefix, 1)], recs[(blk.prefix, 2)]
            g_u2 = CL(gcat[i], 0, cp)
            g_u1 = CL(torch.empty_like(r1.y.buf), 0, cp)
            self._conv_bn_bwd(P, r2, g_u2, g_u1, grads, ws, part, head_rows if j == nlev - 1 else None,
                              head_fin if j == nlev - 1 else None)
            x_in = ctx["dec_in"][j]
            ct = blk.cin
            if j > 0 and plan.skip == "cat":
                segs = ((plan.dec[j - 1].cout, 0), (plan.dec[j - 1].cout, pad8(plan.dec[j - 1].cout)))
            else:
                segs = ((ct, 0),)
            imap_t, cinv_t = self._maps(segs, x_in.cp, dev)
            wt = P[f"{blk.prefix}.0.weight"]
            up = ctx["ups"][j]
            if j > 0:
                gin = g_skip_target(i + 1)
            else:
                gin = CL(torch.empty_like(x_in.buf), 0, x_in.cp)
                g_deep = gin
            if up is None:
                lz = self._conv_bn_bwd(P, r1, g_u1, None, grads, ws, part, up_in=x_in)
                gq = g_u1
                up_wgrad = ops.lp_upconv_fused_wgrad if g_u1.lp else ops.upconv_fused_wgrad
                dwt, dbt, dw3 = up_wgrad(x_in, gq, ct, blk.cout, P[f"{blk.prefix}.0.bias"], self._up_cache[blk.prefix][4], imap_t, lz)
                if lz is not None:
                    gq = lz[3]
                grads[f"{blk.prefix}.1.weight"] = dw3
                grads[f"{blk.prefix}.0.weight"], grads[f"{blk.prefix}.0.bias"] = dwt, dbt
                if g_u1.lp:
                    ops.lp_upconv_fused_bwd_data(gq, self._up_cache[blk.prefix][5], gin, (ct, blk.cout))
                else:
                    ops.upconv_fused_bwd_data(gq, self._up_cache[blk.prefix][5], gin, (ct, blk.cout))
            else:
                g_up = CL(torch.empty_like(up.buf), 0, up.cp)
                self._conv_bn_bwd(P, r1, g_u1, g_up, grads, ws, part)
                dwt, dbt = ops.convt_wgrad(x_in, g_up, ct, ct, imap_t, ws.take(), ws.jobs)
                grads[f"{blk.prefix}.0.weight"], grads[f"{blk.prefix}.0.bias"] = dwt, dbt
                wpd = self._packed(f"{blk.prefix}.0", wt, "convt", cinv_t, g_up.cp, x_in.cp, 1)
                ops.convt_bwd_data(g_up, wpd, gin)
            if j > 0:
                g_skip_fanout(i + 1)
            emit()
        g_pool = g_deep
        if plan.center_live:
            cb = plan.center
            r1, r2 = recs[(cb.prefix, 1)], recs[(cb.prefix, 2)]
            g_c1 = CL(torch.empty_like(r1.y.buf), 0, r1.y.cp)
            self._conv_bn_bwd(P, r2, g_deep, g_c1, grads, ws, part)
            g_pool = CL(torch.empty_like(ctx["pooled"][-1].buf), 0, ctx["pooled"][-1].cp)
            self._conv_bn_bwd(P, r1, g_c1, g_pool, grads, ws, part)
            emit()
        dx = None
        for i in range(nlev - 1, -1, -1):
            blk = plan.enc[i]
            cp = pad8(blk.cout)
            r1, r2 = recs[(blk.prefix, 1)], recs[(blk.prefix, 2)]
            g_d2 = CL(gcat[i], cp, cp)
            dsk = ctx["dskip"][i]
            fuse = (POOL_BN and dsk.scale is not None and dsk.relu and dsk.scale.data_ptr() == r2.vec[0].data_ptr()
                    and ops.maxpool_bwd_bn_blocks(dsk.dims, dsk.cp) > 0)
            fin = self._bwd_fin(P, r2, dsk.buf.device) if fuse else None
            nb = ops.maxpool_bwd(dsk, g_pool, g_d2, plan.skip != "none", (r2.vec, part) if fuse else None, fin)
            nb, done = nb if fin is not None else (nb, None)
            g_d1 = CL(torch.empty_like(r1.y.buf), 0, cp)
            self._conv_bn_bwd(P, r2, g_d2, g_d1, grads, ws, part, nb, done)
            if i > 0:
                g_pool = CL(torch.empty_like(ctx["pooled"][i - 1].buf), 0, ctx["pooled"][i - 1].cp)
                self._conv_bn_bwd(P, r1, g_d1, g_pool, grads, ws, part)
            elif need_dx and r1.first is not None:
                dx = self._conv_bn_bwd(P, r1, g_d1, True, grads, ws, part)
            elif need_dx:
                g_x = CL(torch.empty_like(ctx["x_cl"].buf), 0, ctx["x_cl"].cp)
                self._conv_bn_bwd(P, r1, g_d1, g_x, grads, ws, part)
                dx = ops.cl_to_ncdhw(g_x, plan.in_ch)
            else:
                self._conv_bn_bwd(P, r1, g_d1, None, grads, ws, part)
            emit()
        ws.flush()
        emit()
        unscale([dx])
        if sync is not None:
            if flag is not None:
                sync.push([("__overflow__", flag.clone())])
            grads.update(sync.finish())
            red = grads.pop("__overflow__", None)
            if red is not None:
                flag.copy_(red.reshape(1))
        self._gy_bufs = {}
        return grads, dx


class _UNetFn(torch.autograd.Function):
    @staticmethod
    def forward(fctx, module, engine, names, x_req, x, *params):
        P = _tensor_dict(module)
        out0, out1, ctx = engine.forward(P, x, module.training, True, bool(getattr(module, "chk", False)))
        fctx.engine, fctx.module, fctx.names, fctx.ctx = engine, module, names, ctx
        fctx.two = out1 is not None
        fctx.x_req = x_req
        fctx.versions = _versions(P, names)
        if out1 is None:
            return out0
        return out0, out1

    @staticmethod
    def backward(fctx, *gouts):
        if fctx.ctx is None:
            raise RuntimeError("ctunet_amd: backward through the same forward twice is not supported")
        g0 = gouts[0]
        g1 = gouts[1] if fctx.two else None
        ctx = fctx.ctx
        if g0 is None:
            g0 = torch.zeros(_out_shape(ctx, fctx, 0), device=ctx["cat"][0].device)
        if fctx.two and g1 is None:
            g1 = torch.zeros_like(g0)
        P = _tensor_dict(fctx.module)
        for nm, then, now in zip(fctx.names, fctx.versions, _versions(P, fctx.names)):
            if then != now:
                raise RuntimeError(f"ctunet_amd: parameter {nm} needed for gradient computation has been modified since the "
                                   f"forward pass (version {then[0]} then, {now[0]} now): run backward before changing weights")
        from .parallel import make_sync
        with torch.no_grad():
            grads, dx = fctx.engine.backward(P, ctx, g0, g1, fctx.x_req, make_sync(fctx.module))
        fctx.ctx = None
        return (None, None, None, None, dx) + tuple(grads.get(nm) for nm in fctx.names)


def _out_shape(ctx, fctx, idx):
    n, d, h, w = ctx["dims"]
    c = 2 if fctx.two else fctx.engine.plan.out_ch
    return (n, c, d, h, w)


def _versions(P: Dict[str, torch.Tensor], names) -> Tuple[Tuple[int, int], ...]:
    return tuple((P[nm]._version, P[nm].data_ptr()) for nm in names)


def _tensor_dict(module) -> Dict[str, torch.Tensor]:
    P = dict(module.named_parameters())
    P.update(dict(module.named_buffers()))
    return P


def check_input(module, x: torch.Tensor) -> None:
    if not isinstance(x, torch.Tensor) or x.dim() != 5:
        raise RuntimeError("ctunet_amd: expected a [N, C, D, H, W] tensor")
    if not x.is_cuda:
        raise RuntimeError("ctunet_amd: this model runs on the MI355X only (input is on %s); there is no CPU path"
                           % x.device)
    if x.dtype != torch.float32:
        raise RuntimeError(f"ctunet_amd: fp32 input expected, got {x.dtype}")
    for p in module.parameters():
        if p.device != x.device:
            raise RuntimeError("ctunet_amd: module parameters and input must be on the same GPU (call .to(device))")


def run_network(module, engine: UNetEngine, x: torch.Tensor):
    check_input(module, x)
    names, params = zip(*module.named_parameters())
    need_grad = torch.is_grad_enabled() and (x.requires_grad or any(p.requires_grad for p in params))
    if not need_grad:
        with torch.no_grad():
            out0, out1, _ = engine.forward(_tensor_dict(module), x, module.training, False, False)
        return out0 if out1 is None else (out0, out1)
    return _UNetFn.apply(module, engine, names, x.requires_grad, x, *params)
```

### ct-unet_amd/ctunet_amd/ops.py

```python
from __future__ import annotations

import contextlib
import ctypes
import gc
import os

from dataclasses import dataclass
from typing import Optional, Sequence, Tuple

import torch

from . import _lib


def pad8(c: int) -> int:
    return (c + 7) // 8 * 8


LP_CODE = {torch.bfloat16: 1, torch.float16: 2}
ACT_DTYPES = (torch.float32, torch.bfloat16, torch.float16)


def _need_cuda(t: torch.Tensor, name: str) -> None:
    if not t.is_cuda:
# ... 105 lines not shown
        return ts[len(ts) // 2] if ts else 0.0

    def begin(self):
        ev = torch.cuda.Event(enable_timing=True)
        ev.record()
        return ev

    def end(self, tag, flops, nbytes, start, detail=None):
        ev = torch.cuda.Event(enable_timing=True)
        ev.record()
        self.records.append((tag, flops, nbytes, start, ev))
        self.details.append(detail)
        if len(self.records) % 16 == 1:
            a = torch.cuda.Event(enable_timing=True)
            b = torch.cuda.Event(enable_timing=True)
            a.record()
            b.record()
            self._empty.append((a, b))

    def by_layer(self):
        out = {}
        ovh = self._overhead_ms()
        for (tag, fl, nb, a, b), det in zip(self.records, self.details):
            d = out.setdefault((tag, det), dict(launches=0, total_ms=0.0, flops=0.0))
            d["launches"] += 1
            d["total_ms"] += max(a.elapsed_time(b) - ovh, 1e-4)
            d["flops"] += fl
        return out

    def summary(self):
        sites = {}
        ovh = self._overhead_ms()
        for (tag, fl, nb, a, b), det in zip(self.records, self.details):
            sites.setdefault((tag, det, fl, nb), []).append(max(a.elapsed_time(b) - ovh, 1e-4))
        out = {}
        for (tag, det, fl, nb), ts in sites.items():
            ts.sort()
            med = ts[len(ts) // 2] if len(ts) % 2 else 0.5 * (ts[len(ts) // 2 - 1] + ts[len(ts) // 2])
            d = out.setdefault(tag, dict(launches=0, total_ms=0.0, flops=0.0, bytes=0.0))
            d["launches"] += len(ts)
            d["total_ms"] += med * len(ts)
            d["flops"] += fl * len(ts)
            d["bytes"] += nb * len(ts)
        for d in out.values():
            d["avg_ms"] = d["total_ms"] / d["launches"]
        return out


TIMER: Optional[KernelTimer] = None
FIRST_WGRAD_MFMA_MIN_VOX = int(os.environ.get("CTUNET_FIRST_WGRAD_MFMA_MIN_VOX", "4000000"))


class _timed:
    __slots__ = ("record", "t0")

    def __init__(self, record):
        self.record = record

    def __enter__(self):
        self.t0 = TIMER.begin() if TIMER is not None else None

    def __exit__(self, exc_type, exc, tb):
        if self.t0 is not None and exc_type is None:
            tag, flops, nbytes, detail = self.record()
            TIMER.end(tag, flops, nbytes, self.t0, detail)


class WgradJobs:

    def __init__(self):
        self.items = []

    def __len__(self) -> int:
        return len(self.items)

    def uses(self, ws: torch.Tensor) -> bool:
        return any(keep[0] is ws for _, keep in self.items)

    def add(self, job, ws: torch.Tensor, *outs) -> None:
        if not job.kind:
            return
        if len(self.items) == _lib.WGRAD_JOBS_MAX:
            self.flush()
        self.items.append((job, (ws,) + outs))

    def take(self):
        n = len(self.items)
        arr = (_lib.WgradJob * max(n, 1))(*(j for j, _ in self.items))
        self.items = []
        return arr, n

    def flush(self) -> None:
        if self.items:
            arr, n = self.take()
            _lib.check(_lib.load().ctu_wgrad_reduce_jobs(arr, n, _stream()), "wgrad_reduce_jobs")


def _deferred(jobs: Optional[WgradJobs], code: int = 0) -> bool:
    return jobs is not None and not code and TIMER is None


@dataclass
class CL:
    buf: torch.Tensor
    c0: int = 0
    cp: int = 0
    scale: Optional[torch.Tensor] = None
    shift: Optional[torch.Tensor] = None
    relu: bool = False

    def __post_init__(self):
        if self.cp == 0:
            self.cp = self.buf.shape[-1] - self.c0
        assert self.buf.dim() == 5 and self.buf.is_contiguous() and self.buf.dtype in ACT_DTYPES
        assert self.cp % 8 == 0 and self.c0 % 4 == 0 and self.c0 + self.cp <= self.buf.shape[-1]
        assert self.buf.dtype == torch.float32 or (self.c0 % 8 == 0 and self.buf.shape[-1] % 8 == 0)

    @property
    def dtype(self) -> torch.dtype:
        return self.buf.dtype

    @property
    def lp(self) -> int:
        return LP_CODE.get(self.buf.dtype, 0)

    @property
    def cs(self) -> int:
        return self.buf.shape[-1]

    @property
    def dims(self) -> Tuple[int, int, int, int]:
        n, d, h, w, _ = self.buf.shape
        return n, d, h, w

    @property
    def nvox(self) -> int:
        n, d, h, w = self.dims
        return n * d * h * w

    @property
    def ptr(self):
        return _ptr(self.buf, self.c0)

    def slice(self, c0: int, cp: int) -> "CL":
        sc = None if self.scale is None else self.scale[c0:c0 + cp]
        sh = None if self.shift is None else self.shift[c0:c0 + cp]
        return CL(self.buf, self.c0 + c0, cp, sc, sh, self.relu)

    def raw(self) -> "CL":
        return CL(self.buf, self.c0, self.cp)

    def with_xf(self, scale, shift, relu=True) -> "CL":
        return CL(self.buf, self.c0, self.cp, scale, shift, relu)


def new_cl(n, d, h, w, cs, device, zero=False, dtype=torch.float32) -> torch.Tensor:
    f = torch.zeros if zero else torch.empty
    return f((n, d, h, w, cs), dtype=dtype, device=device)


def ncdhw_to_cl(x: torch.Tensor, cp: Optional[int] = None, dtype=torch.float32) -> CL:
    _need_cuda(x, "input")
    x = x.contiguous()
    n, c, d, h, w = x.shape
    cp = cp or pad8(c)
    out = new_cl(n, d, h, w, cp, x.device, dtype=dtype)
    _dual(lp(dtype), "ncdhw_to_ndhwc", x.data_ptr(), out.data_ptr(), n, c, d, h, w, cp, cp, _stream())
    return CL(out, 0, cp)


def cl_to_ncdhw(a: CL, c: int) -> torch.Tensor:
    n, d, h, w = a.dims
    out = torch.empty((n, c, d, h, w), dtype=torch.float32, device=a.buf.device)
    _dual(a.lp, "ndhwc_to_ncdhw", a.ptr, out.data_ptr(), n, c, d, h, w, a.cs, _stream())
    return out


def conv_layout(k: int, nout_p: int, w: int, dtype=torch.float32, rin_p: int = 0) -> int:
    if lp(dtype):
        return _lib.load().ctu_lp_conv3d_layout(k, rin_p, nout_p, w)
    return _lib.load().ctu_conv3d_layout(k, nout_p, w)


def pack_conv_w(w: torch.Tensor, cinv: Optional[torch.Tensor], rin_p: int, nout_p: int, mode: int,
                layout: int = 0) -> torch.Tensor:
    _need_cuda(w, "conv weight")
    co, ci, k = w.shape[0], w.shape[1], w.shape[2]
    lib = _lib.load()
    n = lib.ctu_conv3d_packed_floats(k, rin_p, nout_p, layout)
    wp = torch.empty(n, dtype=torch.float32, device=w.device)
    _lib.check(lib.ctu_pack_conv3d_weight(w.contiguous().data_ptr(), wp.data_ptr(), co, ci, k, _ptr(cinv), rin_p,
                                          nout_p, mode, layout, _stream()), "pack_conv3d_weight")
    return wp


def packed_floats(kind: str, k: int, rin_p: int, nout_p: int, layout: int) -> int:
    lib = _lib.load()
    return lib.ctu_conv3d_packed_floats(k, rin_p, nout_p, layout) if kind == "conv" else \
        lib.ctu_convt_packed_floats(rin_p, nout_p)


def pack_batch(jobs, dtype: torch.dtype = torch.float32) -> None:
    if not jobs:
        return
    code = 0 if dtype == torch.float32 else LP_CODE[dtype]
    arr = (_lib.PackJob * len(jobs))()
    for a, (kind, w, wp, cinv, rin_p, nout_p, mode, layout) in zip(arr, jobs):
        _need_cuda(w, "weight")
        assert w.is_contiguous() and (not code or wp.dtype == dtype)
        a.w, a.wp, a.cinv = w.data_ptr(), wp.data_ptr(), (None if cinv is None else cinv.data_ptr())
        if kind == "conv":
            a.kind, a.Co, a.Ci, a.k = 0, w.shape[0], w.shape[1], w.shape[2]
        else:
            a.kind, a.Ci, a.Co, a.k = 1, w.shape[0], w.shape[1], 2
            if code:
                layout = 0
        a.rin_p, a.nout_p, a.mode, a.layout = rin_p, nout_p, mode, layout
    _dual(code, "pack_batch", arr, len(jobs), _stream())


def conv_num_blocks(dims, nout_p: int, layout: int = 0, k: int = 3, dtype=torch.float32, rin_p: int = 32) -> int:
    n, d, h, w = dims
    if lp(dtype):
        return _lib.load().ctu_lp_conv3d_num_blocks(n, d, h, w, k, rin_p, nout_p, layout)
    return _lib.load().ctu_conv3d_num_blocks(n, d, h, w, k, nout_p, layout)


def conv3d_fwd(x: CL, wp: torch.Tensor, bias: Optional[torch.Tensor], out: CL, k: int,
               stats: Optional[torch.Tensor] = None, algo_ch: Optional[Tuple[int, int]] = None, layout: int = 0,
               tail=None) -> None:
    n, d, h, w = x.dims
    assert out.dims == x.dims
    code = x.lp
    assert not code or (out.dtype == x.dtype and wp.dtype == x.dtype), (x.dtype, out.dtype, wp.dtype)

    def record():
        ci, co = algo_ch if algo_ch is not None else (x.cp, out.cp)
        vox = n * d * h * w
        if code:
            name = _lib.load().ctu_lp_conv3d_fwd_kernel_name(n, d, h, w, k, x.cp, out.cp, layout).decode()
            tag = f"{name}<{_lp_name(code)}, {k}>"
        else:
            tag = _lib.load().ctu_conv3d_fwd_kernel_name(n, d, h, w, k, out.cp, layout).decode()
        return tag, 2.0 * ci * co * k ** 3 * vox, (2.0 if code else 4.0) * vox * (ci + co), (w, x.cp, out.cp)
    with _timed(record):
        _dual(code, "conv3d_fwd", x.ptr, x.cs, x.cp, _ptr(x.scale), _ptr(x.shift), int(x.relu), wp.data_ptr(), _ptr(bias),
              0 if bias is None else bias.numel(), out.ptr, out.cs, out.cp, _ptr(stats), n, d, h, w, k, layout,
              _tail_arg(tail), _stream())


def _wgrad_setup(x: CL, g: CL, co: int, ci: int, k: int, ws: torch.Tensor):
    n, d, h, w = x.dims
    code = x.lp
    assert not code or g.dtype == x.dtype
    need = _query(code, "conv3d_wgrad_ws_floats", n, d, h, w, k, x.cp, g.cp)
    assert ws.numel() >= need, (ws.numel(), need)
    dw = torch.empty((co, ci, k, k, k), dtype=torch.float32, device=x.buf.device)

    def record():
        vox = n * d * h * w
        if code:
            name = _lib.load().ctu_lp_conv3d_wgrad_kernel_name(d, h, w, k, x.cp, g.cp).decode()
            tag = f"{name}<{_lp_name(code)}, {k}> (+slab reduce)"
        else:
            tag = _lib.load().ctu_conv3d_wgrad_kernel_name(w, k, x.cp, g.cp).decode() + " (+slab reduce)"
        return tag, 2.0 * ci * co * k ** 3 * vox, (2.0 if code else 4.0) * vox * (ci + co), (w, x.cp, g.cp)
    return dw, _timed(record)


def conv3d_wgrad(x: CL, g: CL, co: int, ci: int, k: int, cinv: Optional[torch.Tensor], ws: torch.Tensor,
                 want_bias: bool, jobs: Optional[WgradJobs] = None) -> Tuple[torch.Tensor, Optional[torch.Tensor]]:
    n, d, h, w = x.dims
    code = x.lp
    dw, timed = _wgrad_setup(x, g, co, ci, k, ws)
    db = torch.empty(co, dtype=torch.float32, device=x.buf.device) if want_bias and not code else None
    if _deferred(jobs, code):
        job = _lib.WgradJob()
        _dual(0, "conv3d_wgrad_slabs", x.ptr, x.cs, x.cp, _ptr(x.scale), _ptr(x.shift), int(x.relu), g.ptr, g.cs, g.cp,
              dw.data_ptr(), _ptr(db), co, ci, _ptr(cinv), ws.data_ptr(), n, d, h, w, k, ctypes.byref(job), _stream())
        jobs.add(job, ws, dw, cinv)
        return dw, db
    with timed:
        _dual(code, "conv3d_wgrad", x.ptr, x.cs, x.cp, _ptr(x.scale), _ptr(x.shift), int(x.relu), g.ptr, g.cs, g.cp,
              dw.data_ptr(), *(() if code else (_ptr(db),)), co, ci, _ptr(cinv), ws.data_ptr(), n, d, h, w, k, _stream())
    if want_bias and code:
        db = channel_sum(g, co)
    return dw, db


def conv3d_wgrad_bn_supported(dims, k: int, cin_p: int, cout_p: int, dtype=torch.float32) -> bool:
    n, d, h, w = dims
    return bool(_query(lp(dtype), "conv3d_wgrad_bn_supported", n, d, h, w, k, cin_p, cout_p))


def conv3d_wgrad_bn(x: CL, ga: CL, y: CL, vec: torch.Tensor, coef: torch.Tensor, gy: CL, co: int, ci: int, k: int,
                    cinv: Optional[torch.Tensor], ws: torch.Tensor, jobs: Optional[WgradJobs] = None) -> torch.Tensor:
    n, d, h, w = x.dims
    assert ga.dims == x.dims and y.dims == x.dims and gy.dims == x.dims and ga.dtype == x.dtype == y.dtype == gy.dtype
    assert y.cs == ga.cs == gy.cs and y.cp == ga.cp == gy.cp and gy.buf.data_ptr() != ga.buf.data_ptr()
    dw, timed = _wgrad_setup(x, ga, co, ci, k, ws)
    if _deferred(jobs, x.lp):
        job = _lib.WgradJob()
        _dual(0, "conv3d_wgrad_bn_slabs", x.ptr, x.cs, x.cp, _ptr(x.scale), _ptr(x.shift), int(x.relu), ga.ptr, ga.cs, ga.cp,
              y.ptr, vec[0].data_ptr(), vec[1].data_ptr(), coef.data_ptr(), gy.ptr, dw.data_ptr(), co, ci, _ptr(cinv),
              ws.data_ptr(), n, d, h, w, k, ctypes.byref(job), _stream())
        jobs.add(job, ws, dw, cinv)
# ... 137 lines not shown
    vec = torch.empty((2, cp), dtype=torch.float32, device=gamma.device)
    bn_eval_affine_into(gamma, beta, rmean, rvar, eps, c, cp, vec)
    return vec


def bn_relu_bwd(y: CL, ga: CL, vec: torch.Tensor, gamma: torch.Tensor, c: int, partials: torch.Tensor,
                replay=None, pre_reduced: Optional[int] = None, counter: Optional[torch.Tensor] = None, finalized=None,
                lazy: bool = False, jobs: Optional[WgradJobs] = None):
    lib = _lib.load()
    nvox = y.nvox
    cp = y.cp
    sc, sh, mu, istd = (vec[i].data_ptr() for i in range(4))
    st = _stream()
    if jobs is not None and (finalized is not None or (counter is not None and pre_reduced is None)):
        jobs.flush()
    if finalized is not None:
        dgb, coef = finalized
        if lazy:
            return dgb[0], dgb[1], coef
        _dual(y.lp, "bn_relu_bwd_apply", y.ptr, y.cs, ga.ptr, ga.cs, cp, sc, sh, mu, istd, coef.data_ptr(), nvox, st)
        return dgb[0], dgb[1]
    nb = lib.ctu_bn_bwd_num_blocks(nvox) if pre_reduced is None else pre_reduced
    assert partials.numel() >= nb * 2 * cp
    tail, (dgb, coef) = _bn_bwd_outputs(c, cp, nvox, gamma, vec, replay, counter, y.buf.device,
                                        tail=counter is not None and pre_reduced is None)
    if pre_reduced is None:
        assert ga.dtype == y.dtype
        _dual(y.lp, "bn_relu_bwd_reduce", y.ptr, y.cs, ga.ptr, ga.cs, cp, sc, sh, mu, istd, nvox, partials.data_ptr(),
              _tail_arg(tail), st)
    if tail is None:
        rm, rv, mom, eps, nbt = _replay_args(replay)
        fin = (partials.data_ptr(), nb, c, cp, float(nvox), gamma.data_ptr(), istd, dgb[0].data_ptr(), dgb[1].data_ptr(),
               coef.data_ptr(), mu, _ptr(rm), _ptr(rv), mom, eps, None if nbt is None else nbt.data_ptr())
        if jobs:
            arr, n = jobs.take()
            _lib.check(lib.ctu_bn_bwd_finalize_jobs(*fin, arr, n, st), "bn_bwd_finalize_jobs")
        else:
            _lib.check(lib.ctu_bn_bwd_finalize(*fin, st), "bn_bwd_finalize")
    if lazy:
        return dgb[0], dgb[1], coef
    _dual(y.lp, "bn_relu_bwd_apply", y.ptr, y.cs, ga.ptr, ga.cs, cp, sc, sh, mu, istd, coef.data_ptr(), nvox, st)
    return dgb[0], dgb[1]


def bn_bwd_partials_floats(nvox: int, cp: int) -> int:
    return _lib.load().ctu_bn_bwd_num_blocks(nvox) * 2 * cp


def maxpool_fwd(x: CL, out: CL) -> None:
    n, d, h, w = x.dims
    assert out.dtype == x.dtype
    _dual(x.lp, "maxpool2_fwd", x.ptr, x.cs, x.cp, _ptr(x.scale), _ptr(x.shift), int(x.relu), out.ptr, out.cs, n, d, h, w,
          _stream())


def maxpool_bwd_bn_blocks(dims, cp: int) -> int:
    n, d, h, w = dims
    return _lib.load().ctu_maxpool2_bwd_bn_num_blocks(n, d, h, w, cp)


def maxpool_bwd(x: CL, gout: CL, gin: CL, accumulate: bool, bn=None, fin=None):
    n, d, h, w = x.dims
    if bn is not None:
        vec, partials = bn
        nb = maxpool_bwd_bn_blocks(x.dims, x.cp)
        assert x.scale is not None and x.relu and partials.numel() >= nb * 2 * x.cp
        assert vec[0].data_ptr() == x.scale.data_ptr() and vec[1].data_ptr() == x.shift.data_ptr()
        tail, done = None, None
        if fin is not None:
            gamma, c, replay, counter = fin
            tail, done = _bn_bwd_outputs(c, x.cp, x.nvox, gamma, vec, replay, counter, x.buf.device)
        _dual(x.lp, "maxpool2_bwd_bn", x.ptr, x.cs, x.cp, vec[0].data_ptr(), vec[1].data_ptr(), vec[2].data_ptr(),
              vec[3].data_ptr(), gout.ptr, gout.cs, gin.ptr, gin.cs, int(accumulate), n, d, h, w, partials.data_ptr(),
              _tail_arg(tail), _stream())
        return nb if fin is None else (nb, done)
    _dual(x.lp, "maxpool2_bwd", x.ptr, x.cs, x.cp, _ptr(x.scale), _ptr(x.shift), int(x.relu), gout.ptr, gout.cs, gin.ptr,
          gin.cs, int(accumulate), n, d, h, w, _stream())


def pack_convt_w(w: torch.Tensor, cinv, rin_p: int, nout_p: int, mode: int) -> torch.Tensor:
    _need_cuda(w, "convT weight")
    ci, co = w.shape[0], w.shape[1]
    lib = _lib.load()
    wp = torch.empty(lib.ctu_convt_packed_floats(rin_p, nout_p), dtype=torch.float32, device=w.device)
    _lib.check(lib.ctu_pack_convt_weight(w.contiguous().data_ptr(), wp.data_ptr(), ci, co, _ptr(cinv), rin_p, nout_p,
                                         mode, _stream()), "pack_convt_weight")
    return wp


def pack_convt_w_lp(w: torch.Tensor, cinv, rin_p: int, nout_p: int, mode: int, dtype: torch.dtype,
                    into: Optional[torch.Tensor] = None) -> torch.Tensor:
    _need_cuda(w, "convT weight")
    ci, co = w.shape[0], w.shape[1]
    lib = _lib.load()
    n = lib.ctu_lp_convt_packed_elems(rin_p, nout_p, mode)
    wp = into if into is not None else torch.empty(n, dtype=dtype, device=w.device)
    assert wp.numel() == n and wp.dtype == dtype
    _lib.check(lib.ctu_lp_pack_convt_weight(LP_CODE[dtype], w.contiguous().data_ptr(), wp.data_ptr(), ci, co, _ptr(cinv), rin_p,
                                            nout_p, mode, _stream()), "lp_pack_convt_weight")
    return wp


def _convt_bracket(name: str, x: CL, x_cp: int, o_cp: int, dims) -> _timed:
    n, d, h, w = dims
    vox = n * d * h * w
    return _timed(lambda: (name + ("_lp" if x.lp else ""), 16.0 * x_cp * o_cp * vox,
                           float(x.buf.element_size()) * vox * (x_cp + 8 * o_cp), (w, x_cp, o_cp)))


def convt_fwd(x: CL, wp: torch.Tensor, bias: Optional[torch.Tensor], out: CL) -> None:
    n, d, h, w = x.dims
    with _convt_bracket("convt2_fwd", x, x.cp, out.cp, x.dims):
        assert not x.lp or (out.dtype == x.dtype and wp.dtype == x.dtype)
        _dual(x.lp, "convt2_fwd", x.ptr, x.cs, x.cp, _ptr(x.scale), _ptr(x.shift), int(x.relu), wp.data_ptr(), _ptr(bias),
              0 if bias is None else bias.numel(), out.ptr, out.cs, out.cp, n, d, h, w, _stream())


def convt_bwd_data(gout: CL, wp: torch.Tensor, gin: CL) -> None:
    n, d, h, w = gin.dims
    with _convt_bracket("convt2_bwd_data", gout, gin.cp, gout.cp, gin.dims):
        assert not gout.lp or (gin.dtype == gout.dtype and wp.dtype == gout.dtype)
        _dual(gout.lp, "convt2_bwd_data", gout.ptr, gout.cs, gout.cp, wp.data_ptr(), gin.ptr, gin.cs, gin.cp, n, d, h, w,
              _stream())


def convt_wgrad(x: CL, g: CL, ci: int, co: int, imap, ws: torch.Tensor, jobs: Optional[WgradJobs] = None):
    n, d, h, w = x.dims
    if _deferred(jobs, x.lp):
        assert ws.numel() >= convt_wgrad_ws(x.dims, x.cp, g.cp, x.dtype)
        dw = torch.empty((ci, co, 2, 2, 2), dtype=torch.float32, device=x.buf.device)
        db = torch.empty(co, dtype=torch.float32, device=x.buf.device)
        job = _lib.WgradJob()
        _dual(0, "convt2_wgrad_slabs", x.ptr, x.cs, x.cp, _ptr(x.scale), _ptr(x.shift), int(x.relu), g.ptr, g.cs, g.cp,
              dw.data_ptr(), db.data_ptr(), ci, co, _ptr(imap), ws.data_ptr(), n, d, h, w, ctypes.byref(job), _stream())
        jobs.add(job, ws, dw, db, imap)
        return dw, db
    with _convt_bracket("convt2_wgrad", x, x.cp, g.cp, x.dims):
        assert not x.lp or g.dtype == x.dtype
        assert ws.numel() >= convt_wgrad_ws(x.dims, x.cp, g.cp, x.dtype)
        dw = torch.empty((ci, co, 2, 2, 2), dtype=torch.float32, device=x.buf.device)
        db = None if x.lp else torch.empty(co, dtype=torch.float32, device=x.buf.device)
        _dual(x.lp, "convt2_wgrad", x.ptr, x.cs, x.cp, _ptr(x.scale), _ptr(x.shift), int(x.relu), g.ptr, g.cs, g.cp,
              dw.data_ptr(), *(() if x.lp else (db.data_ptr(),)), ci, co, _ptr(imap), ws.data_ptr(), n, d, h, w, _stream())
        if x.lp:
            db = channel_sum(g, co)
    return dw, db


def convt_wgrad_ws(dims, cin_p, cout_p, dtype=torch.float32) -> int:
    n, d, h, w = dims
    return _query(lp(dtype), "convt2_wgrad_ws_floats", n, d, h, w, cin_p, cout_p)


def head_fwd(x: CL, w: torch.Tensor, b: torch.Tensor, imap, act: int, head_mode: int):
    n, d, h, w_ = x.dims
    co, ci = w.shape[0], w.shape[1]
    v = d * h * w_
    dev = x.buf.device
    if head_mode == 0:
        out0 = torch.empty((n, co, d, h, w_), dtype=torch.float32, device=dev)
        out1 = None
    else:
        out0 = torch.empty((n, 2, d, h, w_), dtype=torch.float32, device=dev)
        out1 = torch.empty((n, 2, d, h, w_), dtype=torch.float32, device=dev)
    _dual(x.lp, "head_fwd", x.ptr, x.cs, x.cp, _ptr(x.scale), _ptr(x.shift), int(x.relu), w.data_ptr(), b.data_ptr(),
          _ptr(imap), ci, co, act, head_mode, out0.data_ptr(), _ptr(out1), n, v, _stream())
    return out0, out1


def head_bwd(x: CL, w: torch.Tensor, b: torch.Tensor, imap, act: int, head_mode: int, g0: torch.Tensor,
             g1: Optional[torch.Tensor], gin: CL, bn=None, fin=None, gscale: float = 1.0,
             gscale_dev: Optional[torch.Tensor] = None):
    assert gscale == 1.0 or x.lp, "gscale is the 16-bit path's loss scale"
    assert gscale_dev is None or (x.lp and gscale_dev.is_cuda and gscale_dev.dtype == torch.float32), \
        "gscale_dev is the 16-bit path's device loss scale"
    n, d, h, w_ = x.dims
    co, ci = w.shape[0], w.shape[1]
    v = d * h * w_
    dev = x.buf.device
    lib = _lib.load()
    ws = torch.empty(lib.ctu_head_bwd_ws_floats(n, v, x.cp, co), dtype=torch.float32, device=dev)
    dw = torch.empty_like(w)
    db = torch.empty_like(b)
    bn_args, tail, done = (None, None, 0, None), None, None
    if bn is not None:
        vec, partials = bn
        bn_cp = vec.shape[1]
        rows = lib.ctu_head_bwd_num_blocks(n, v)
        assert x.scale is not None and x.relu and vec[0].data_ptr() == x.scale.data_ptr() and partials.numel() >= rows * 2 * bn_cp
        bn_args = (vec[2].data_ptr(), vec[3].data_ptr(), bn_cp, partials.data_ptr())
        if fin is not None:
            gamma, c, replay = fin[:3]
            tail, done = _bn_bwd_outputs(c, bn_cp, n * v, gamma, vec, replay, None, dev)
    entry, scale = "head_bwd_bn", ((float(gscale),) if x.lp else ())
    if gscale_dev is not None:
        entry, scale = "head_bwd_bn_dscale", (gscale_dev.data_ptr(),)
    _dual(x.lp, entry, x.ptr, x.cs, x.cp, _ptr(x.scale), _ptr(x.shift), int(x.relu), w.data_ptr(), b.data_ptr(), _ptr(imap),
          ci, co, act, head_mode, g0.data_ptr(), _ptr(g1), gin.ptr, gin.cs, dw.data_ptr(), db.data_ptr(), ws.data_ptr(), n, v,
          *bn_args, _tail_arg(tail), *scale, _stream())
    if bn is None:
        return dw, db
    return (dw, db, rows) if fin is None else (dw, db, rows, done)


def head_bwd_blocks(dims) -> int:
    n, d, h, w_ = dims
    return _lib.load().ctu_head_bwd_num_blocks(n, d * h * w_)


def loss_fwd(pred: torch.Tensor, target: torch.Tensor, ce_lambda: float, dice_lambda: float, dice_softmax: bool):
    _need_cuda(pred, "prediction")
    _need_cuda(target, "target")
    assert pred.shape == target.shape and pred.shape[1] == 2, "loss kernel handles 2-channel maps"
    pred, target = pred.contiguous(), target.contiguous()
    n = pred.shape[0]
    v = pred[0, 0].numel()
    lib = _lib.load()
    ws = torch.empty(lib.ctu_loss_ws_floats(n, v), dtype=torch.float32, device=pred.device)
    terms = torch.empty(2, dtype=torch.float32, device=pred.device)
    _lib.check(lib.ctu_loss_fwd(pred.data_ptr(), target.data_ptr(), n, v, ce_lambda, dice_lambda, int(dice_softmax),
                                terms.data_ptr(), ws.data_ptr(), _stream()), "loss_fwd")
    return terms, ws


def loss_bwd(pred, target, ce_lambda, dice_lambda, dice_softmax, ws, g_ce: Optional[torch.Tensor],
             g_dice: Optional[torch.Tensor], out: Optional[torch.Tensor] = None, accumulate: bool = False) -> torch.Tensor:
    pred, target = pred.contiguous(), target.contiguous()
    for g_ in (g_ce, g_dice):
        assert g_ is None or (g_.is_cuda and g_.dtype == torch.float32 and g_.numel() == 1)
    n = pred.shape[0]
    v = pred[0, 0].numel()
    g = out if out is not None else torch.empty_like(pred)
    lib = _lib.load()
    _lib.check(lib.ctu_loss_bwd(pred.data_ptr(), target.data_ptr(), n, v, ce_lambda, dice_lambda, int(dice_softmax),
                                ws.data_ptr(), _ptr(g_ce), _ptr(g_dice), g.data_ptr(), int(accumulate), _stream()),
               "loss_bwd")
    return g


def _seg_loss_args(pred, target, lambdas, dice_softmax, class_weight, focal_gamma, tversky_ab, boundary):
    _need_cuda(pred, "prediction")
    _need_cuda(target, "target")
    assert pred.shape == target.shape and pred.dim() == 5 and pred.shape[1] == 2, "loss kernel handles 2-channel maps"
    pred, target = pred.contiguous(), target.contiguous()
    n, v = pred.shape[0], pred[0, 0].numel()
    ce, dice, tv, bd = (float(x) for x in lambdas)
    if bd != 0.0:
        if boundary is None:
            raise ValueError("ctunet_amd: boundary_lambda != 0 needs a boundary (signed distance) map")
        _need_cuda(boundary, "boundary map")
        if boundary.dtype != torch.float32 or tuple(boundary.shape) not in ((n,) + tuple(pred.shape[2:]),
                                                                            (n, 1) + tuple(pred.shape[2:])):
            raise ValueError(f"ctunet_amd: the boundary map must be float32 [N,D,H,W] or [N,1,D,H,W] of the prediction's "
                             f"grid, got {boundary.dtype} {tuple(boundary.shape)} for {tuple(pred.shape)}")
        boundary = boundary.contiguous()
    else:
        boundary = None
    cfg = _lib.SegLossCfg(ce, dice, tv, bd, float(class_weight[0]), float(class_weight[1]), float(focal_gamma),
                          float(tversky_ab[0]), float(tversky_ab[1]), int(bool(dice_softmax)))
    return pred, target, boundary, n, v, cfg


def seg_loss_fwd(pred: torch.Tensor, target: torch.Tensor, lambdas: Sequence[float], dice_softmax: bool,
                 class_weight: Sequence[float] = (1.0, 1.0), focal_gamma: float = 0.0,
                 tversky_ab: Sequence[float] = (0.5, 0.5), boundary: Optional[torch.Tensor] = None):
    pred, target, boundary, n, v, cfg = _seg_loss_args(pred, target, lambdas, dice_softmax, class_weight, focal_gamma,
                                                      tversky_ab, boundary)
    lib = _lib.load()
    ws = torch.empty(lib.ctu_seg_loss_ws_floats(n, v), dtype=torch.float32, device=pred.device)
    terms = torch.empty(4, dtype=torch.float32, device=pred.device)
    _lib.check(lib.ctu_seg_loss_fwd(pred.data_ptr(), target.data_ptr(), _ptr(boundary), n, v, ctypes.byref(cfg),
                                    terms.data_ptr(), ws.data_ptr(), _stream()), "seg_loss_fwd")
    return terms, ws


def seg_loss_bwd(pred, target, lambdas, dice_softmax, ws, upstream: Sequence[Optional[torch.Tensor]] = (None,) * 4,
                 class_weight: Sequence[float] = (1.0, 1.0), focal_gamma: float = 0.0,
                 tversky_ab: Sequence[float] = (0.5, 0.5), boundary: Optional[torch.Tensor] = None,
                 out: Optional[torch.Tensor] = None, accumulate: bool = False) -> torch.Tensor:
    pred, target, boundary, n, v, cfg = _seg_loss_args(pred, target, lambdas, dice_softmax, class_weight, focal_gamma,
                                                      tversky_ab, boundary)
    assert len(upstream) == 4
    for g_ in upstream:
        assert g_ is None or (g_.is_cuda and g_.dtype == torch.float32 and g_.numel() == 1)
    g = out if out is not None else torch.empty_like(pred)
    lib = _lib.load()
    _lib.check(lib.ctu_seg_loss_bwd(pred.data_ptr(), target.data_ptr(), _ptr(boundary), n, v, ctypes.byref(cfg),
                                    ws.data_ptr(), *(_ptr(g_) for g_ in upstream), g.data_ptr(), int(accumulate),
                                    _stream()), "seg_loss_bwd")
    return g



def skip_add(a: CL, b: Optional[CL], out: CL) -> None:
    assert out.dims == a.dims and out.cp == a.cp and (b is None or (b.dims == a.dims and b.cp == a.cp))
    assert out.dtype == a.dtype and (b is None or b.dtype == a.dtype)
    _dual(a.lp, "skip_add", a.ptr, a.cs, _ptr(a.scale), _ptr(a.shift), int(a.relu), 0 if b is None else b.ptr,
          0 if b is None else b.cs, _ptr(b.scale) if b is not None else 0, _ptr(b.shift) if b is not None else 0,
          int(b.relu) if b is not None else 0, out.ptr, out.cs, out.cp, a.nvox, _stream())


def channel_sum(x: CL, c: int) -> torch.Tensor:
    lib = _lib.load()
    nb = lib.ctu_channel_sum_num_blocks(x.nvox)
    part = torch.empty(nb * x.cp, dtype=torch.float32, device=x.buf.device)
    out = torch.empty(c, dtype=torch.float32, device=x.buf.device)
    _dual(x.lp, "channel_sum", x.ptr, x.cs, x.cp, x.nvox, part.data_ptr(), out.data_ptr(), c, _stream())
    return out


def upconv_fused_supported(dims, k: int, cin_p: int, nout_p: int) -> bool:
    n, d, h, w = dims
    return bool(_lib.load().ctu_upconv_fused_supported(k, d, h, w, cin_p, nout_p))


def upconv_fused_pack(wt: torch.Tensor, bt: torch.Tensor, w3: torch.Tensor, cinv, cin_p: int, nout_p: int,
                      into=None):
    return _upconv_pack(wt, bt, w3, cinv, cin_p, nout_p, into, False)


def upconv_fused_pack_all(wt: torch.Tensor, bt: torch.Tensor, w3: torch.Tensor, cinv, cin_p: int, nout_p: int,
                          into=None):
    return _upconv_pack(wt, bt, w3, cinv, cin_p, nout_p, into, True)


def _upconv_pack(wt, bt, w3, cinv, cin_p, nout_p, into, with_wpd: bool):
    lib = _lib.load()
    c, co = wt.shape[0], w3.shape[0]
    assert wt.shape == (c, c, 2, 2, 2) and w3.shape == (co, c, 3, 3, 3) and bt.shape == (c,)
    if into is not None:
        bufs = tuple(into)
        assert len(bufs) == 3 + with_wpd
    else:
        new = lambda n: torch.empty(n, dtype=torch.float32, device=wt.device)
        bufs = (new(lib.ctu_upconv_fused_packed_floats(cin_p, nout_p)), new((27, nout_p)),
                new(lib.ctu_upconv_fused_pack_ws_floats(c, nout_p)))
        if with_wpd:
            bufs += (new(lib.ctu_upconv_fused_bwd_packed_floats(cin_p, nout_p)),)
    wp, beff, ws = bufs[:3]
    _lib.check(lib.ctu_upconv_fused_pack_all(wt.detach().contiguous().data_ptr(), bt.detach().contiguous().data_ptr(),
                                             w3.detach().contiguous().data_ptr(), c, co, _ptr(cinv), cin_p, nout_p, wp.data_ptr(),
                                             beff.data_ptr(), ws.data_ptr(), bufs[3].data_ptr() if with_wpd else None, _stream()),
               "upconv_fused_pack")
    return bufs


def upconv_fused_num_blocks(dims, nout_p: int) -> int:
    n, d, h, w = dims
    return _lib.load().ctu_upconv_fused_num_blocks(n, d, h, w, nout_p)


# ... 454 lines not shown
```

### include/ctunet_hip.h

```cpp
#ifndef CTUNET_HIP_H
#define CTUNET_HIP_H

#include <stddef.h>
#include <stdint.h>

#ifdef __cplusplus
extern "C" {
#endif

#define CTU_OK 0
#define CTU_EINVAL (-1)
#define CTU_ELAUNCH (-2)

#define CTU_F32 0
#define CTU_BF16 1
#define CTU_F16 2

typedef struct ctu_bn_tail {
    const float* gamma; const float* beta;
    float* running_mean; float* running_var;
    float* scale; float* shift; float* mean; float* invstd;
    long long* num_batches_tracked;
    unsigned int* counter;
    double count;
// ... 26 lines not shown
size_t ctu_conv3d_packed_floats(int k, int rin_p, int nout_p, int layout);
int ctu_conv3d_num_blocks(int N, int D, int H, int W, int k, int nout_p, int layout);

int ctu_pack_conv3d_weight(const float* w, float* wp, int Co, int Ci, int k,
                           const int32_t* cinv, int rin_p, int nout_p, int mode, int layout,
                           void* stream);

typedef struct {
    const float* w;
    float* wp;
    const int32_t* cinv;
    int kind, Co, Ci, k, rin_p, nout_p, mode, layout;
} ctu_pack_job;
int ctu_pack_batch(const ctu_pack_job* jobs, int n, void* stream);

int ctu_conv3d_fwd(const float* in, int in_cs, int rin_p,
                   const float* in_scale, const float* in_shift, int in_relu,
                   const float* wp, const float* bias, int nbias,
                   float* out, int out_cs, int nout_p, float* stats,
                   int N, int D, int H, int W, int k, int layout, const ctu_bn_tail* tail, void* stream);

size_t ctu_conv3d_wgrad_ws_floats(int N, int D, int H, int W, int k, int cin_p, int cout_p);
int ctu_conv3d_wgrad(const float* in, int in_cs, int cin_p,
                     const float* in_scale, const float* in_shift, int in_relu,
                     const float* gout, int g_cs, int cout_p,
                     float* dw, float* dbias, int Co, int Ci, const int32_t* cinv,
                     float* ws, int N, int D, int H, int W, int k, void* stream);
int ctu_conv3d_wgrad_bn_supported(int N, int D, int H, int W, int k, int cin_p, int cout_p);
int ctu_conv3d_wgrad_bn(const float* in, int in_cs, int cin_p,
                        const float* in_scale, const float* in_shift, int in_relu,
                        const float* ga, int g_cs, int cout_p, const float* y,
                        const float* bn_scale, const float* bn_shift, const float* coef, float* gy_out,
                        float* dw, int Co, int Ci, const int32_t* cinv,
                        float* ws, int N, int D, int H, int W, int k, void* stream);

int ctu_conv3d_first_supported(int k, int cin, int nout_p, int W);
int ctu_conv3d_first_num_blocks(int N, int D, int H, int W);
int ctu_conv3d_first_fwd(const float* x, int cin, const float* w, const float* bias, int nbias,
                         float* out, int out_cs, int Co, float* stats,
                         int N, int D, int H, int W, const ctu_bn_tail* tail, void* stream);
int ctu_conv3d_first_bwd_data(const float* g, int g_cs, const float* w, int cin, int Co, float* dx,
                              int N, int D, int H, int W, void* stream);
size_t ctu_conv3d_first_wgrad_ws_floats(int N, int D, int H, int W, int cin);
int ctu_conv3d_first_wgrad(const float* x, int cin, const float* g, int g_cs, float* dw, int Co,
                           float* ws, int N, int D, int H, int W, void* stream);
int ctu_conv3d_first_wgrad_bn(const float* x, int cin, const float* ga, int g_cs, const float* y, const float* bn_scale,
                              const float* bn_shift, const float* coef, float* gy_out, float* dw, int Co, float* ws,
                              int N, int D, int H, int W, void* stream);

int ctu_bn_finalize(const float* stats, int nblocks, int C, int cp, double count,
                    const float* gamma, const float* beta,
                    float* running_mean, float* running_var, float momentum, float eps,
                    int n_updates, float* scale, float* shift, float* mean_out,
                    float* invstd_out, long long* num_batches_tracked, void* stream);
int ctu_bn_eval_affine(const float* gamma, const float* beta, const float* running_mean,
                       const float* running_var, float eps, int C, int cp,
                       float* scale, float* shift, void* stream);

int ctu_bn_bwd_num_blocks(int64_t nvox);
int ctu_bn_relu_bwd_reduce(const float* y, int y_cs, const float* ga, int g_cs, int cp,
                           const float* scale, const float* shift, const float* mean,
                           const float* invstd, int64_t nvox, float* partials, const ctu_bn_bwd_tail* tail, void* stream);
int ctu_bn_bwd_finalize(const float* partials, int nb, int C, int cp, double count,
                        const float* gamma, const float* invstd,
                        float* dgamma, float* dbeta, float* coef, const float* mean,
                        float* running_mean, float* running_var, float momentum, float eps,
                        long long* num_batches_tracked, void* stream);
int ctu_bn_relu_bwd_apply(const float* y, int y_cs, float* ga, int g_cs, int cp,
                          const float* scale, const float* shift, const float* mean,
                          const float* invstd, const float* coef, int64_t nvox, void* stream);

#define CTU_WGRAD_JOBS_MAX 4
typedef struct ctu_wgrad_job {
    const float* ws;
    float* dw; float* db;
    const int32_t* cinv;
    int kind;
    int Co, Ci, cin_p, n_ci_g, gx, pairs, nmf;
} ctu_wgrad_job;
int ctu_conv3d_wgrad_slabs(const float* in, int in_cs, int cin_p,
                           const float* in_scale, const float* in_shift, int in_relu,
                           const float* gout, int g_cs, int cout_p,
                           float* dw, float* dbias, int Co, int Ci, const int32_t* cinv,
                           float* ws, int N, int D, int H, int W, int k, ctu_wgrad_job* job, void* stream);
int ctu_conv3d_wgrad_bn_slabs(const float* in, int in_cs, int cin_p,
                              const float* in_scale, const float* in_shift, int in_relu,
                              const float* ga, int g_cs, int cout_p, const float* y,
                              const float* bn_scale, const float* bn_shift, const float* coef, float* gy_out,
                              float* dw, int Co, int Ci, const int32_t* cinv,
                              float* ws, int N, int D, int H, int W, int k, ctu_wgrad_job* job, void* stream);
int ctu_conv3d_first_wgrad_slabs(const float* x, int cin, const float* g, int g_cs, float* dw, int Co,
                                 float* ws, int N, int D, int H, int W, ctu_wgrad_job* job, void* stream);
int ctu_conv3d_first_wgrad_bn_slabs(const float* x, int cin, const float* ga, int g_cs, const float* y, const float* bn_scale,
                                    const float* bn_shift, const float* coef, float* gy_out, float* dw, int Co, float* ws,
                                    int N, int D, int H, int W, ctu_wgrad_job* job, void* stream);
int ctu_convt2_wgrad_slabs(const float* in, int in_cs, int cin_p, const float* in_scale,
                           const float* in_shift, int in_relu, const float* gout, int g_cs,
                           int cout_p, float* dw, float* dbias, int Ci, int Co,
                           const int32_t* imap, float* ws, int N, int D, int H, int W, ctu_wgrad_job* job, void* stream);
int ctu_bn_bwd_finalize_jobs(const float* partials, int nb, int C, int cp, double count,
                             const float* gamma, const float* invstd,
                             float* dgamma, float* dbeta, float* coef, const float* mean,
                             float* running_mean, float* running_var, float momentum, float eps,
                             long long* num_batches_tracked, const ctu_wgrad_job* jobs, int njobs, void* stream);
int ctu_wgrad_reduce_jobs(const ctu_wgrad_job* jobs, int njobs, void* stream);

int ctu_maxpool2_fwd(const float* in, int in_cs, int cp, const float* in_scale,
                     const float* in_shift, int in_relu, float* out, int out_cs,
                     int N, int D, int H, int W, void* stream);
int ctu_maxpool2_bwd(const float* in, int in_cs, int cp, const float* in_scale,
                     const float* in_shift, int in_relu, const float* gout, int gout_cs,
                     float* gin, int gin_cs, int accumulate, int N, int D, int H, int W,
                     void* stream);
int ctu_maxpool2_bwd_bn_num_blocks(int N, int D, int H, int W, int cp);
int ctu_maxpool2_bwd_bn(const float* in, int in_cs, int cp, const float* in_scale, const float* in_shift,
                        const float* mean, const float* invstd, const float* gout, int gout_cs, float* gin,
                        int gin_cs, int accumulate, int N, int D, int H, int W, float* partials, const ctu_bn_bwd_tail* tail, void* stream);

size_t ctu_convt_packed_floats(int rin_p, int nout_p);
int ctu_pack_convt_weight(const float* w, float* wp, int Ci, int Co, const int32_t* cinv,
                          int rin_p, int nout_p, int mode, void* stream);
int ctu_convt2_fwd(const float* in, int in_cs, int rin_p, const float* in_scale,
                   const float* in_shift, int in_relu, const float* wp, const float* bias,
                   int nbias, float* out, int out_cs, int nout_p, int N, int D, int H, int W,
                   void* stream);
int ctu_convt2_bwd_data(const float* gout, int g_cs, int rout_p, const float* wp,
                        float* gin, int gin_cs, int nin_p, int N, int D, int H, int W,
                        void* stream);
size_t ctu_convt2_wgrad_ws_floats(int N, int D, int H, int W, int cin_p, int cout_p);
int ctu_convt2_wgrad(const float* in, int in_cs, int cin_p, const float* in_scale,
                     const float* in_shift, int in_relu, const float* gout, int g_cs,
                     int cout_p, float* dw, float* dbias, int Ci, int Co,
                     const int32_t* imap, float* ws, int N, int D, int H, int W, void* stream);
const char* ctu_convt2_plan(int mode, int rin_p, int nout_p, int N, int D, int H, int W, int* plan);
const char* ctu_convt2_wgrad_plan(int cin_p, int cout_p, int N, int D, int H, int W, int* plan);

int ctu_head_fwd(const float* in, int in_cs, int cin_p, const float* in_scale,
                 const float* in_shift, int in_relu, const float* w, const float* bias,
                 const int32_t* imap, int Ci, int Co, int act, int head_mode,
                 float* out0, float* out1, int N, int64_t nvox_per_item, void* stream);
size_t ctu_head_bwd_ws_floats(int N, int64_t nvox_per_item, int cin_p, int Co);
int ctu_head_bwd(const float* in, int in_cs, int cin_p, const float* in_scale,
                 const float* in_shift, int in_relu, const float* w, const float* bias,
                 const int32_t* imap, int Ci, int Co, int act, int head_mode,
                 const float* g0, const float* g1, float* gin, int gin_cs,
                 float* dw, float* db, float* ws, int N, int64_t nvox_per_item, void* stream);
int ctu_head_bwd_num_blocks(int N, int64_t nvox_per_item);
int ctu_head_bwd_bn(const float* in, int in_cs, int cin_p, const float* in_scale,
                    const float* in_shift, int in_relu, const float* w, const float* bias,
                    const int32_t* imap, int Ci, int Co, int act, int head_mode,
                    const float* g0, const float* g1, float* gin, int gin_cs,
                    float* dw, float* db, float* ws, int N, int64_t nvox_per_item,
                    const float* bn_mean, const float* bn_invstd, int bn_cp, float* bn_partials, const ctu_bn_bwd_tail* tail, void* stream);

size_t ctu_loss_ws_floats(int N, int64_t V);
int ctu_loss_fwd(const float* pred, const float* target, int N, int64_t V, float ce_lambda,
                 float dice_lambda, int dice_softmax, float* terms, float* ws, void* stream);
int ctu_loss_bwd(const float* pred, const float* target, int N, int64_t V, float ce_lambda,
                 float dice_lambda, int dice_softmax, const float* ws, const float* gscale_ce,
                 const float* gscale_dice, float* gpred, int accumulate, void* stream);

typedef struct ctu_seg_loss_cfg {
    float ce_lambda, dice_lambda, tversky_lambda, boundary_lambda;
    float w0, w1;
    float focal_gamma;
    float tversky_alpha, tversky_beta;
    int dice_softmax;
} ctu_seg_loss_cfg;
size_t ctu_seg_loss_ws_floats(int N, int64_t V);
int ctu_seg_loss_fwd(const float* pred, const float* target, const float* phi, int N, int64_t V,
                     const ctu_seg_loss_cfg* cfg, float* terms, float* ws, void* stream);
int ctu_seg_loss_bwd(const float* pred, const float* target, const float* phi, int N, int64_t V,
                     const ctu_seg_loss_cfg* cfg, const float* ws, const float* g_ce, const float* g_dice,
                     const float* g_tversky, const float* g_boundary, float* gpred, int accumulate, void* stream);

int ctu_skip_add(const float* a, int a_cs, const float* a_scale, const float* a_shift, int a_relu,
                 const float* b, int b_cs, const float* b_scale, const float* b_shift, int b_relu,
                 float* out, int out_cs, int cp, int64_t nvox, void* stream);
int ctu_upconv_fused_supported(int k, int D, int H, int W, int cin_p, int nout_p);
size_t ctu_upconv_fused_packed_floats(int cin_p, int nout_p);
int ctu_upconv_fused_num_blocks(int N, int D, int H, int W, int nout_p);
size_t ctu_upconv_fused_pack_ws_floats(int C, int nout_p);
int ctu_upconv_fused_pack(const float* wt, const float* bt, const float* w3, int C, int Co, const int32_t* cinv,
                          int cin_p, int nout_p, float* wp, float* beff, float* ws, void* stream);
int ctu_upconv_fused_pack_all(const float* wt, const float* bt, const float* w3, int C, int Co, const int32_t* cinv,
                              int cin_p, int nout_p, float* wp, float* beff, float* ws, float* wpd, void* stream);
int ctu_upconv_fused_fwd(const float* in, int in_cs, int cin_p, const float* in_scale, const float* in_shift,
                         int in_relu, const float* wp, const float* beff, float* out, int out_cs, int nout_p,
                         float* stats, int N, int D, int H, int W, const ctu_bn_tail* tail, void* stream);

size_t ctu_upconv_fused_wgrad_ws_floats(int N, int D, int H, int W, int cin_p, int nout_p);
int ctu_upconv_fused_wgrad(const float* in, int in_cs, int cin_p, const float* in_scale, const float* in_shift,
                           int in_relu, const float* gout, int g_cs, int nout_p, float* dweff, float* ws,
                           int N, int D, int H, int W, void* stream);
int ctu_upconv_fused_wgrad_bn_supported(int N, int D, int H, int W, int cin_p, int nout_p);
int ctu_upconv_fused_wgrad_bn(const float* in, int in_cs, int cin_p, const float* in_scale, const float* in_shift,
                              int in_relu, const float* ga, int g_cs, int nout_p, const float* y,
                              const float* bn_scale, const float* bn_shift, const float* coef, float* gy_out,
                              float* dweff, float* ws, int N, int D, int H, int W, void* stream);
size_t ctu_upconv_fused_project_ws_floats(int nout_p, int64_t fine_nvox);
int ctu_upconv_fused_project(const float* dweff, const float* gout, int g_cs, int nout_p, int N, int D, int H, int W,
                             const float* bt, const float* pack_ws, const int32_t* imap, int C, int Co, int cin_p,
                             float* dwt, float* dbt, float* dw3, float* ws, void* stream);

size_t ctu_upconv_fused_bwd_packed_floats(int cin_p, int nout_p);
int ctu_upconv_fused_pack_bwd(const float* wp, int cin_p, int nout_p, float* wpd, void* stream);
int ctu_upconv_fused_bwd_data(const float* gout, int g_cs, int nout_p, const float* wpd, float* gin, int gin_cs,
                              int cin_p, int N, int D, int H, int W, void* stream);

int ctu_hard_segm(const float* prob, int N, int C, int64_t nvox_per_item, float* seg, void* stream);
int ctu_one_hot(const float* label, int N, int C, int64_t nvox_per_item, float* out, void* stream);
size_t ctu_hard_dice_ws_doubles(int N);
int ctu_hard_dice_counts(const float* pred, const float* target, int N, int C, int64_t nvox_per_item,
                         double* counts, double* ws, void* stream);

size_t ctu_hausdorff_ws_bytes(int N, int C, int D, int H, int W);
int ctu_hausdorff(const float* pred, const float* target, int N, int C, int D, int H, int W, float* out, void* ws,
                  void* stream);

#define CTU_U8 3
#define CTU_I64 4
size_t ctu_surface_ws_bytes(int N, int Cs, int D, int H, int W);
int ctu_surface_metrics(const void* pred, int pred_dtype, int pred_onehot, const void* target, int target_dtype,
                        int target_onehot, int N, int C, int cls0, int Cs, int D, int H, int W, const float* spacing,
                        const double* tau, double percentile, float* out, void* ws, void* stream);

#define CTU_CC_LARGEST 0
#define CTU_CC_MIN_SIZE 1
size_t ctu_components_ws_bytes(int N, int D, int H, int W);
int ctu_label_components(const void* in, int dtype, int N, int D, int H, int W, int connectivity, const int64_t* applied,
                         int n_applied, int32_t* labels, int32_t* num, void* ws, void* stream);
int ctu_filter_components(const void* in, int dtype, int N, int D, int H, int W, int connectivity,
                          const int64_t* applied, int n_applied, int mode, int param, void* out, void* ws, void* stream);

#define CTU_MORPH_ERODE 0
#define CTU_MORPH_DILATE 1
#define CTU_MORPH_OPEN 2
#define CTU_MORPH_CLOSE 3
#define CTU_MORPH_WS_MORPH 0
#define CTU_MORPH_WS_FILL 1
#define CTU_MORPH_WS_IMPLANT 2
size_t ctu_morphology_ws_bytes(int N, int D, int H, int W, int kind);
int ctu_binary_morphology(const void* in, int dtype, int N, int D, int H, int W, int mode, uint32_t structure,
                          int iterations, int border, int has_label, int64_t label, uint8_t* out, void* ws, void* stream);
int ctu_fill_holes(const void* in, int dtype, int N, int D, int H, int W, int connectivity, int has_label, int64_t label,
                   uint8_t* out, void* ws, void* stream);
int ctu_implant_mask(const void* full, int full_dtype, const void* defective, int defective_dtype, int N, int D, int H,
                     int W, uint32_t structure, int opening_iterations, int fill_holes, int connectivity,
                     int num_components, uint8_t* out, void* ws, void* stream);

#define CTU_DIST_EDT 0
#define CTU_DIST_SQUARED 1
#define CTU_DIST_SIGNED 2
#define CTU_DIST_BALL 3
size_t ctu_distance_ws_bytes(int N, int D, int H, int W, int out_kind, int want_indices);
int ctu_distance_transform(const void* in, int dtype, int N, int D, int H, int W, int has_label, int64_t label, int invert,
                           int border_background, const float* spacing, int out_kind, void* out, int32_t* indices,
                           float ball_r2, void* ws, void* stream);

size_t ctu_thickness_ws_bytes(int N, int D, int H, int W, int is_float);
int ctu_local_thickness(const void* d2, int is_float, int N, int D, int H, int W, const float* spacing, void* out, void* ws,
                        void* stream);
size_t ctu_thickness_summary_ws_bytes(int N, int64_t V);
int ctu_thickness_summary(const float* thickness, int N, int64_t V, float min_thickness, double* out, void* ws, void* stream);

#define CTU_I16 5
#define CTU_I32 6
#define CTU_RESAMPLE_NEAREST 0
#define CTU_RESAMPLE_LINEAR 1
#define CTU_RESAMPLE_LABEL_LINEAR 2
int ctu_resample(const void* in, int dtype, int mode, int num_classes, int64_t N, int D, int H, int W, int d, int h, int w,
                 const int32_t* i0, const float* wt, const int32_t* near, void* out, void* stream);

int ctu_affine_resample(const void* in, int dtype, int mode, int num_classes, int64_t N, int D, int H, int W, int d, int h,
                        int w, const double* out_to_in, const double* spacing, const double* origin,
                        const double* out_spacing, const double* out_origin, double fill, void* out, void* stream);

#define CTU_REG_MAX_BLOCKS 1024
#define CTU_REG_MIN_INLIERS 6
size_t ctu_registration_ws_bytes(int64_t P);
int ctu_registration_init(const float* points, int64_t P, const double* init, void* ws, void* stream);
int ctu_registration_accumulate(const float* points, int64_t P, const float* field, int D, int H, int W,
                                const double* spacing, const double* origin, double max_distance, void* ws, void* stream);
int ctu_registration_update(int64_t P, int it, double* matrix, double* inverse, double* history, int history_rows, void* ws,
                            void* stream);

#define CTU_MESH_SCAN_BLOCK 1024
#define CTU_MESH_MEASURE_WS 16384
size_t ctu_mesh_ws_bytes(int D, int H, int W);
int ctu_mesh_count(const void* volume, int dtype, int D, int H, int W, int has_label, int64_t label, float level, void* ws,
                   void* stream);
int ctu_mesh_emit(const void* volume, int dtype, int D, int H, int W, float level, float fill_value, const float* spacing,
                  const float* origin, int64_t V, int64_t F, float* vertices, int32_t* faces, void* ws, void* stream);
int ctu_mesh_measure(const float* vertices, int64_t V, const int32_t* faces, int64_t F, double* out, float* normals, void* ws,
                     void* stream);

#define CTU_MESH_ADJ_SCAN_CHUNK 4096
#define CTU_MESH_SMOOTH_MAX_ITERATIONS 10000
size_t ctu_mesh_adjacency_ws_bytes(int64_t V, int64_t F);
int ctu_mesh_adjacency_build(const int32_t* faces, int64_t V, int64_t F, int32_t* offsets, void* ws, void* stream);
int ctu_mesh_adjacency_emit(int64_t V, int64_t F, int64_t E, const int32_t* offsets, int32_t* neighbours, void* ws,
                            void* stream);
size_t ctu_mesh_smooth_ws_bytes(int64_t V);
int ctu_mesh_smooth(const float* vertices, int64_t V, const int32_t* offsets, const int32_t* neighbours, int64_t E,
                    const uint8_t* fixed, int iterations, float lambda, int has_mu, float mu, float* out, void* ws,
                    void* stream);
// ... 37 lines not shown
int ctu_threshold_otsu(const int64_t* hist, int bins, const double* range, double lo, double hi, double* threshold,
                       int64_t* index, void* stream);
int ctu_binarize(const void* in, int dtype, int64_t n, const double* lower_dev, double lower, const double* upper_dev,
                 double upper, uint8_t* out, void* stream);

int ctu_extract_patches(const float* vol, const int32_t* coords, int P, int C, int D, int H, int W, int pd, int ph,
                        int pw, float* out, void* stream);
int ctu_stitch_patches(const float* patches, const int32_t* coords, int P, int C, int D, int H, int W, int pd, int ph,
                       int pw, float* out, void* stream);

int ctu_window_accumulate(const float* patches, const int32_t* coords, const int32_t* valid, const int32_t* box, int B,
                          int K, int D, int H, int W, int pd, int ph, int pw, const float* wz, const float* wy,
                          const float* wx, float wmin, int bz, int by, int bx, float* num, float* wsum, void* stream);
int ctu_window_finalize(const float* num, const float* wsum, int K, int64_t V, float* probs, uint8_t* labels,
                        void* stream);

int ctu_extract_patches_flip(const float* vol, const int32_t* coords, const int32_t* flip, int P, int C, int D, int H,
                             int W, int pd, int ph, int pw, float* out, void* stream);
int ctu_window_accumulate_flip(const float* patches, const int32_t* coords, const int32_t* valid, const int32_t* box,
                               const int32_t* flip, int B, int K, int D, int H, int W, int pd, int ph, int pw,
                               const float* wz, const float* wy, const float* wx, float wmin, int bz, int by, int bx,
                               float* num, float* wsum, float* sq, float* sh, void* stream);
int ctu_window_finalize_stats(const float* num, const float* wsum, const float* sq, const float* sh, int K, int64_t V,
                              float* probs, uint8_t* labels, float* var, float* ent, float* mi, void* stream);

#define CTU_FLAP_CHUNK 8192
#define CTU_FLAP_RECORD 16
#define CTU_FLAP_HOLE 1
#define CTU_FLAP_NOISE 2
#define CTU_FLAP_SPHERE 0
#define CTU_FLAP_BOX 1
#define CTU_FLAP_FLAP 2
int ctu_flap_count(const void* skull, int u8, int N, int64_t V, int32_t* counts, void* stream);
int ctu_flap_draw(const void* skull, int u8, int N, int D, int H, int W, const int32_t* counts, int mode,
                  const int64_t* hole_seq, uint64_t hole_seed, float p_hole, int size_lo, int size_hi, int shapes,
                  const int64_t* noise_seq, const float* noise_nd, uint64_t noise_seed, float p_noise, float salt_ratio,
                  int decay, int32_t* params, void* stream);
int ctu_flap_apply(const void* skull, int u8, const float* atlas, int N, int D, int H, int W, const int32_t* params,
                   int mode, int64_t* hole_seq, int64_t* noise_seq, float* noise_nd, uint64_t noise_seed, int decay,
                   float* x, int C, float* full, float* flap, void* stream);

#define CTU_SPATIAL_RECORD 26
#define CTU_SPATIAL_MIN_POINTS 4
#define CTU_SPATIAL_MAX_POINTS 12
int ctu_spatial_draw(int N, int D, int H, int W, const double* spacing, const int64_t* seq, uint64_t seed, int flip_mask,
                     double flip_p, double affine_p, double elastic_p, const double* ranges, int gz, int gy, int gx,
                     int locked, double* record, double* control, void* stream);
int ctu_spatial_warp(const void* in, int dtype, int N, int C, int D, int H, int W, const double* spacing, int gz, int gy,
                     int gx, const double* record, const double* control, int64_t* seq, void* out, void* stream);

int ctu_lp_conv3d_layout(int k, int rin_p, int nout_p, int W);
size_t ctu_lp_conv3d_packed_elems(int k, int rin_p, int nout_p);
int ctu_lp_conv3d_num_blocks(int N, int D, int H, int W, int k, int rin_p, int nout_p, int layout);
int ctu_lp_pack_conv3d_weight(int dtype, const float* w, void* wp, int Co, int Ci, int k, const int32_t* cinv,
                              int rin_p, int nout_p, int mode, int layout, void* stream);
int ctu_lp_pack_batch(int dtype, const ctu_pack_job* jobs, int n, void* stream);
int ctu_lp_conv3d_fwd(int dtype, const void* in, int in_cs, int rin_p, const float* in_scale, const float* in_shift,
                      int in_relu, const void* wp, const float* bias, int nbias, void* out, int out_cs, int nout_p,
                      float* stats, int N, int D, int H, int W, int k, int layout, const ctu_bn_tail* tail, void* stream);
size_t ctu_lp_conv3d_wgrad_ws_floats(int N, int D, int H, int W, int k, int cin_p, int cout_p);
int ctu_lp_conv3d_wgrad(int dtype, const void* in, int in_cs, int cin_p, const float* in_scale, const float* in_shift,
                        int in_relu, const void* gout, int g_cs, int cout_p, float* dw, int Co, int Ci,
                        const int32_t* cinv, float* ws, int N, int D, int H, int W, int k, void* stream);
int ctu_lp_conv3d_wgrad_bn_supported(int N, int D, int H, int W, int k, int cin_p, int cout_p);
int ctu_lp_conv3d_wgrad_bn(int dtype, const void* in, int in_cs, int cin_p, const float* in_scale, const float* in_shift,
                           int in_relu, const void* ga, int g_cs, int cout_p, const void* y, const float* bn_scale,
                           const float* bn_shift, const float* coef, void* gy_out, float* dw, int Co, int Ci,
                           const int32_t* cinv, float* ws, int N, int D, int H, int W, int k, void* stream);

int ctu_lp_conv3d_first_fwd(int dtype, const float* x, int cin, const float* w, const float* bias, int nbias, void* out,
                            int out_cs, int Co, float* stats, int N, int D, int H, int W, const ctu_bn_tail* tail, void* stream);
int ctu_lp_conv3d_first_bwd_data(int dtype, const void* g, int g_cs, const float* w, int cin, int Co, float* dx, int N,
                                 int D, int H, int W, void* stream);
int ctu_lp_conv3d_first_wgrad(int dtype, const float* x, int cin, const void* g, int g_cs, float* dw, int Co, float* ws,
                              int N, int D, int H, int W, void* stream);
const char* ctu_lp_conv3d_fwd_kernel_name(int N, int D, int H, int W, int k, int rin_p, int nout_p, int layout);
const char* ctu_lp_conv3d_wgrad_kernel_name(int D, int H, int W, int k, int cin_p, int cout_p);
int ctu_lp_conv3d_first_bwd_data_pair_supported(int cin, int W);
int ctu_lp_conv3d_first_bwd_data_pair(int dtype, const void* g, int g_cs, const void* wp, int cin, float* dx,
                                      int N, int D, int H, int W, void* stream);
size_t ctu_lp_convt_packed_elems(int rin_p, int nout_p, int mode);
int ctu_lp_pack_convt_weight(int dtype, const float* w, void* wp, int Ci, int Co, const int32_t* cinv, int rin_p,
                             int nout_p, int mode, void* stream);
int ctu_lp_convt2_fwd(int dtype, const void* in, int in_cs, int rin_p, const float* in_scale, const float* in_shift,
                      int in_relu, const void* wp, const float* bias, int nbias, void* out, int out_cs, int nout_p,
                      int N, int D, int H, int W, void* stream);
int ctu_lp_convt2_bwd_data(int dtype, const void* gout, int g_cs, int rout_p, const void* wp, void* gin, int gin_cs,
                           int nin_p, int N, int D, int H, int W, void* stream);
size_t ctu_lp_convt2_wgrad_ws_floats(int N, int D, int H, int W, int cin_p, int cout_p);
int ctu_lp_convt2_wgrad(int dtype, const void* in, int in_cs, int cin_p, const float* in_scale, const float* in_shift,
                        int in_relu, const void* gout, int g_cs, int cout_p, float* dw, int Ci, int Co,
                        const int32_t* imap, float* ws, int N, int D, int H, int W, void* stream);
const char* ctu_lp_convt2_plan(int mode, int rin_p, int nout_p, int N, int D, int H, int W, int* plan);
const char* ctu_lp_convt2_wgrad_plan(int cin_p, int cout_p, int N, int D, int H, int W, int* plan);
int ctu_lp_upconv_fused_supported(int k, int D, int H, int W, int cin_p, int nout_p);
size_t ctu_lp_upconv_fused_packed_elems(int cin_p);
int ctu_lp_upconv_fused_num_blocks(int N, int D, int H, int W);
int ctu_lp_upconv_fused_pack(int dtype, const float* wp32, int cin_p, void* wp16, void* stream);
int ctu_lp_upconv_fused_fwd(int dtype, const void* in, int in_cs, int cin_p, const float* in_scale, const float* in_shift,
                            int in_relu, const void* wp16, const float* beff, void* out, int out_cs, float* stats,
                            int N, int D, int H, int W, void* stream);
size_t ctu_lp_upconv_fused_wgrad_ws_floats(int N, int D, int H, int W, int cin_p);
int ctu_lp_upconv_fused_wgrad(int dtype, const void* in, int in_cs, int cin_p, const float* in_scale, const float* in_shift,
                              int in_relu, const void* gout, int g_cs, float* dweff, float* ws, int N, int D, int H,
                              int W, void* stream);
int ctu_lp_upconv_fused_wgrad_bn_supported(int N, int D, int H, int W, int cin_p);
int ctu_lp_upconv_fused_wgrad_bn(int dtype, const void* in, int in_cs, int cin_p, const float* in_scale, const float* in_shift,
                                 int in_relu, const void* ga, int g_cs, const void* y, const float* bn_scale,
                                 const float* bn_shift, const float* coef, void* gy_out, float* dweff, float* ws,
                                 int N, int D, int H, int W, void* stream);
int ctu_lp_upconv_fused_project(int dtype, const float* dweff, const void* gout, int g_cs, int nout_p, int N, int D, int H,
                                int W, const float* bt, const float* pack_ws, const int32_t* imap, int C, int Co, int cin_p,
                                float* dwt, float* dbt, float* dw3, float* ws, void* stream);
int ctu_lp_upconv_fused_bwd_data(int dtype, const void* gout, int g_cs, const void* wp16, void* gin, int gin_cs, int cin_p,
                                 int N, int D, int H, int W, void* stream);
int ctu_lp_ncdhw_to_ndhwc(int dtype, const float* src, void* dst, int N, int C, int D, int H, int W, int cp, int cs,
                          void* stream);
int ctu_lp_ndhwc_to_ncdhw(int dtype, const void* src, float* dst, int N, int C, int D, int H, int W, int cs,
                          void* stream);
int ctu_lp_bn_relu_bwd_reduce(int dtype, const void* y, int y_cs, const void* ga, int g_cs, int cp, const float* scale,
                              const float* shift, const float* mean, const float* invstd, int64_t nvox,
                              float* partials, const ctu_bn_bwd_tail* tail, void* stream);
int ctu_lp_bn_relu_bwd_apply(int dtype, const void* y, int y_cs, void* ga, int g_cs, int cp, const float* scale,
                             const float* shift, const float* mean, const float* invstd, const float* coef,
                             int64_t nvox, void* stream);
int ctu_lp_maxpool2_fwd(int dtype, const void* in, int in_cs, int cp, const float* in_scale, const float* in_shift,
                        int in_relu, void* out, int out_cs, int N, int D, int H, int W, void* stream);
int ctu_lp_maxpool2_bwd(int dtype, const void* in, int in_cs, int cp, const float* in_scale, const float* in_shift,
                        int in_relu, const void* gout, int gout_cs, void* gin, int gin_cs, int accumulate,
                        int N, int D, int H, int W, void* stream);
int ctu_lp_maxpool2_bwd_bn(int dtype, const void* in, int in_cs, int cp, const float* in_scale, const float* in_shift,
                           const float* mean, const float* invstd, const void* gout, int gout_cs, void* gin,
                           int gin_cs, int accumulate, int N, int D, int H, int W, float* partials, const ctu_bn_bwd_tail* tail, void* stream);
int ctu_lp_skip_add(int dtype, const void* a, int a_cs, const float* a_scale, const float* a_shift, int a_relu,
                    const void* b, int b_cs, const float* b_scale, const float* b_shift, int b_relu,
                    void* out, int out_cs, int cp, int64_t nvox, void* stream);
int ctu_lp_channel_sum(int dtype, const void* x, int cs, int cp, int64_t nvox, float* partials, float* out, int C,
                       void* stream);
int ctu_lp_head_fwd(int dtype, const void* in, int in_cs, int cin_p, const float* in_scale, const float* in_shift,
                    int in_relu, const float* w, const float* bias, const int32_t* imap, int Ci, int Co, int act,
                    int head_mode, float* out0, float* out1, int N, int64_t nvox_per_item, void* stream);
int ctu_lp_head_bwd_bn(int dtype, const void* in, int in_cs, int cin_p, const float* in_scale, const float* in_shift,
                       int in_relu, const float* w, const float* bias, const int32_t* imap, int Ci, int Co, int act,
                       int head_mode, const float* g0, const float* g1, void* gin, int gin_cs, float* dw,
                       float* db, float* ws, int N, int64_t nvox_per_item, const float* bn_mean,
                       const float* bn_invstd, int bn_cp, float* bn_partials, const ctu_bn_bwd_tail* tail, float gscale,
                       void* stream);
int ctu_lp_head_bwd_bn_dscale(int dtype, const void* in, int in_cs, int cin_p, const float* in_scale, const float* in_shift,
                              int in_relu, const float* w, const float* bias, const int32_t* imap, int Ci, int Co, int act,
                              int head_mode, const float* g0, const float* g1, void* gin, int gin_cs, float* dw,
                              float* db, float* ws, int N, int64_t nvox_per_item, const float* bn_mean,
                              const float* bn_invstd, int bn_cp, float* bn_partials, const ctu_bn_bwd_tail* tail,
                              const float* gscale, void* stream);
int ctu_scale_tensors(void* const* ptrs, const int64_t* sizes, int n, float s, float* nonfinite_flag, void* stream);
int ctu_unscale_tensors(void* const* ptrs, const int64_t* sizes, int n, const float* scale, float* found_inf, void* stream);
int ctu_loss_scale_update(float* scale, int32_t* growth_tracker, float* found_inf, float* skipped, float growth,
                          float backoff, int interval, void* stream);

#define CTU_COMM_ID_BYTES 128
int ctu_comm_available(void);
int ctu_comm_unique_id(void* id_host);
int ctu_comm_init(void** comm, int world, int rank, const void* id_host);
int ctu_comm_allreduce_f32(void* comm, const float* send, float* recv, size_t count, int average, void* stream);
int ctu_comm_destroy(void* comm);

int ctu_channel_sum_num_blocks(int64_t nvox);
int ctu_channel_sum(const float* x, int cs, int cp, int64_t nvox, float* partials,
                    float* out, int C, void* stream);
int ctu_adam_amsgrad(void* const* ptrs, const int64_t* sizes, int n, float* step,
                     double lr, double beta1, double beta2, double eps, double weight_decay,
                     int decoupled, const float* skip_flag, void* stream);

int ctu_adam_amsgrad_dev(void* const* ptrs, const int64_t* sizes, int n, float* step, const double* lr, double beta1,
                         double beta2, double eps, double weight_decay, int decoupled, const float* grad_coef,
                         const float* skip_flag, void* stream);
int ctu_grad_norm_num_blocks(const int64_t* sizes, int n);
int ctu_grad_clip_coef(void* const* gptrs, const int64_t* sizes, int n, float max_norm, float* partials_ws, float* norm_out,
                       float* coef_out, void* stream);
int ctu_plateau_update(const float* metric, double* lr, double* state, int32_t* counters, int mode_max, int threshold_rel,
                       double factor, int patience, double threshold, int cooldown, double min_lr, double eps, void* stream);

int ctu_sgd(void* const* ptrs, const int64_t* sizes, int n, float* step, const double* lr_dev, double lr, double momentum,
            double dampening, double weight_decay, int nesterov, int maximize, const float* grad_coef,
            const float* skip_flag, void* stream);
int ctu_rmsprop(void* const* ptrs, const int64_t* sizes, int n, float* step, const double* lr_dev, double lr, double alpha,
                double eps, double weight_decay, double momentum, int centered, int maximize, const float* grad_coef,
                const float* skip_flag, void* stream);

#ifdef __cplusplus
}
#endif
#endif
```

Measured before the change: 683.3 million voxels/s.

## Fuse decoder concat into head conv via two-segment input kernels

Adds forward and backward variants of the final 1x1 head kernel that read input channels from two separate channels-last buffers and write the input gradient back to two buffers. This lets the last decoder stage skip materialising the channel concatenation of skip and upsampled features, and its gradient split, at full resolution. Python ops accept a CL2 two-segment descriptor to route to the new entry points. It adds kernel variants and per-lane segment selection, and only covers 8 or 16 channels per segment.

```diff
diff --git a/ct-unet_amd/csrc/head_loss.hip b/ct-unet_amd/csrc/head_loss.hip
--- a/ct-unet_amd/csrc/head_loss.hip
+++ b/ct-unet_amd/csrc/head_loss.hip
@@ -8,6 +8,8 @@
 
 struct HeadP {
     const void* in;
+    const void* in_b;
+    int in_cs_b;
     const float* in_scale;
     const float* in_shift;
     const float* w;
@@ -19,14 +21,15 @@
     const float* gscale_dev;
 };
 
-template <int CP, class T>
+template <int CP, class T, bool S2>
 __device__ __forceinline__ void head_point(const HeadP& p, const float* sWp, const float* sB, int64_t gv,
                                            float (&a)[CP], float (&lg)[MAXCO], float (&u)[MAXCO],
                                            float (&y)[MAXCO]) {
     const T* src = reinterpret_cast<const T*>(p.in) + (size_t)gv * p.in_cs;
+    const T* src_b = S2 ? reinterpret_cast<const T*>(p.in_b) + (size_t)gv * p.in_cs_b : nullptr;
 #pragma unroll
     for (int qd = 0; qd < CP / 4; ++qd) {
-        float4 v = ld4<T>(src + qd * 4);
+        float4 v = ld4<T>((S2 && qd >= CP / 8) ? src_b + (qd - CP / 8) * 4 : src + qd * 4);
         if (p.in_scale) {
             const float4 sc = *reinterpret_cast<const float4*>(p.in_scale + qd * 4);
             const float4 sh = *reinterpret_cast<const float4*>(p.in_shift + qd * 4);
@@ -79,15 +82,15 @@
     sa = ea / (ea + eb); sb = eb / (ea + eb);
 }
 
-template <int CP, class T>
-__global__ __launch_bounds__(HB) void head_fwd_kernel(HeadP p, float* __restrict__ out0, float* __restrict__ out1) {
+template <int CP, class T, bool S2>
+__device__ __forceinline__ void head_fwd_body(const HeadP& p, float* __restrict__ out0, float* __restrict__ out1) {
     __shared__ float sWp[MAXCO * CP];
     __shared__ float sB[MAXCO];
     head_load_weights<CP>(p, sWp, sB);
     const int64_t total = (int64_t)p.N * p.V;
     for (int64_t gv = (int64_t)blockIdx.x * HB + threadIdx.x; gv < total; gv += (int64_t)gridDim.x * HB) {
         float a[CP], lg[MAXCO], u[MAXCO], y[MAXCO];
-        head_point<CP, T>(p, sWp, sB, gv, a, lg, u, y);
+        head_point<CP, T, S2>(p, sWp, sB, gv, a, lg, u, y);
         const int64_t n = gv / p.V, v = gv % p.V;
         if (p.head_mode == 0) {
 #pragma unroll
@@ -106,11 +109,20 @@
 }
 
 template <int CP, class T>
-__global__ __launch_bounds__(HB) void head_bwd_q_kernel(HeadP p, const float* __restrict__ g0,
-                                                        const float* __restrict__ g1, T* __restrict__ gin,
-                                                        int gin_cs, float* __restrict__ partials,
-                                                        const float* __restrict__ bn_mean, const float* __restrict__ bn_invstd,
-                                                        int bn_cp, float* __restrict__ bn_partials) {
+__global__ __launch_bounds__(HB) void head_fwd_kernel(HeadP p, float* __restrict__ out0, float* __restrict__ out1) {
+    head_fwd_body<CP, T, false>(p, out0, out1);
+}
+template <int CP, class T>
+__global__ __launch_bounds__(HB) void head_fwd_seg2_kernel(HeadP p, float* __restrict__ out0, float* __restrict__ out1) {
+    head_fwd_body<CP, T, true>(p, out0, out1);
+}
+
+template <int CP, class T, bool S2>
+__device__ __forceinline__ void head_bwd_q_body(const HeadP& p, const float* __restrict__ g0,
+                                                const float* __restrict__ g1, T* __restrict__ gin, int gin_cs,
+                                                T* __restrict__ gin_b, int gin_cs_b, float* __restrict__ partials,
+                                                const float* __restrict__ bn_mean, const float* __restrict__ bn_invstd,
+                                                int bn_cp, float* __restrict__ bn_partials) {
     constexpr int Q = CP / 4;
     __shared__ float sWp[MAXCO * CP];
     __shared__ float sB[MAXCO];
@@ -137,10 +149,13 @@
         mu = *reinterpret_cast<const float4*>(bn_mean + qd * 4);
         is = *reinterpret_cast<const float4*>(bn_invstd + qd * 4);
     }
+    const bool seg_b = S2 && qd >= Q / 2;
+    const int qoff = (seg_b ? qd - Q / 2 : qd) * 4;
     const int64_t total = (int64_t)p.N * p.V;
     constexpr int VPB = HB / Q;
     for (int64_t gv = (int64_t)blockIdx.x * VPB + threadIdx.x / Q; gv < total; gv += (int64_t)gridDim.x * VPB) {
-        const float4 raw = ld4<T>(reinterpret_cast<const T*>(p.in) + (size_t)gv * p.in_cs + qd * 4);
+        const float4 raw = ld4<T>((seg_b ? reinterpret_cast<const T*>(p.in_b) : reinterpret_cast<const T*>(p.in)) +
+                                  (size_t)gv * (seg_b ? p.in_cs_b : p.in_cs) + qoff);
         const float4 a = xform4(raw, sc, sh, xrelu);
         float lg[MAXCO], u[MAXCO], y[MAXCO], gy[MAXCO];
 #pragma unroll
@@ -212,7 +227,7 @@
             for (int j = 0; j < 4; ++j) dw[co][j] = fmaf(gl[co], av[j], dw[co][j]);
         }
         o = rnd4<T>(o);
-        st4<T>(gin + (size_t)gv * gin_cs + qd * 4, o);
+        st4<T>((seg_b ? gin_b : gin) + (size_t)gv * (seg_b ? gin_cs_b : gin_cs) + qoff, o);
         if (bnq) {
             float gz;
             gz = (fmaf(raw.x, sc.x, sh.x) > 0.f) ? o.x : 0.f; r1.x += gz; r2.x += gz * (raw.x - mu.x) * is.x;
@@ -259,6 +274,24 @@
             for (int w = 0; w < HB / 64; ++w) s += sRed[w][col];
             bn_partials[(size_t)blockIdx.x * 2 * bn_cp + i] = s;
         }
+}
+
+template <int CP, class T>
+__global__ __launch_bounds__(HB) void head_bwd_q_kernel(HeadP p, const float* __restrict__ g0,
+                                                        const float* __restrict__ g1, T* __restrict__ gin,
+                                                        int gin_cs, float* __restrict__ partials,
+                                                        const float* __restrict__ bn_mean, const float* __restrict__ bn_invstd,
+                                                        int bn_cp, float* __restrict__ bn_partials) {
+    head_bwd_q_body<CP, T, false>(p, g0, g1, gin, gin_cs, nullptr, 0, partials, bn_mean, bn_invstd, bn_cp, bn_partials);
+}
+template <int CP, class T>
+__global__ __launch_bounds__(HB) void head_bwd_q_seg2_kernel(HeadP p, const float* __restrict__ g0,
+                                                             const float* __restrict__ g1, T* __restrict__ gin,
+                                                             int gin_cs, T* __restrict__ gin_b, int gin_cs_b,
+                                                             float* __restrict__ partials, const float* __restrict__ bn_mean,
+                                                             const float* __restrict__ bn_invstd, int bn_cp,
+                                                             float* __restrict__ bn_partials) {
+    head_bwd_q_body<CP, T, true>(p, g0, g1, gin, gin_cs, gin_b, gin_cs_b, partials, bn_mean, bn_invstd, bn_cp, bn_partials);
 }
 
 template <int CP>
@@ -440,17 +473,34 @@
 
 static int fill_head(HeadP& p, const void* in, int in_cs, int cin_p, const float* in_scale, const float* in_shift,
                      int in_relu, const float* w, const float* bias, const int32_t* imap, int Ci, int Co, int act,
-                     int head_mode, int N, int64_t V, const char* name) {
+                     int head_mode, int N, int64_t V, const char* name, int buf_cp = 0) {
+    if (buf_cp == 0) buf_cp = cin_p;
     CTU_REQUIRE(in && w, "%s: null pointer", name);
     CTU_REQUIRE(cin_p == 8 || cin_p == 16 || cin_p == 32, "%s: cin_p=%d unsupported (8, 16 or 32)", name, cin_p);
     CTU_REQUIRE(Co >= 1 && Co <= MAXCO && Ci >= 1 && Ci <= cin_p, "%s: Co=%d Ci=%d", name, Co, Ci);
     CTU_REQUIRE(head_mode == 0 || Co == 3, "%s: SP re-encoding needs 3 output channels", name);
     CTU_REQUIRE(head_mode >= 0 && head_mode <= 2, "%s: head_mode=%d", name, head_mode);
-    CTU_REQUIRE(in_cs >= cin_p && in_cs % 4 == 0, "%s: bad stride", name);
+    CTU_REQUIRE(in_cs >= buf_cp && in_cs % 4 == 0, "%s: bad stride", name);
     CTU_REQUIRE((in_scale == nullptr) == (in_shift == nullptr), "%s: scale/shift must come together", name);
+    p.in_b = nullptr; p.in_cs_b = 0;
     p.in = in; p.in_scale = in_scale; p.in_shift = in_shift; p.w = w; p.bias = bias; p.imap = imap;
     p.in_cs = in_cs; p.in_relu = in_relu; p.Ci = Ci; p.Co = Co; p.act = act; p.head_mode = head_mode; p.N = N; p.V = V; p.gscale = 1.f;
     p.gscale_dev = nullptr;
+    return CTU_OK;
+}
+
+static int fill_head_seg2(HeadP& p, const void* in_a, int cs_a, const void* in_b, int cs_b, int cp, const float* in_scale,
+                          const float* in_shift, int in_relu, const float* w, const float* bias, const int32_t* imap, int Ci,
+                          int Co, int act, int head_mode, int N, int64_t V, const char* name) {
+    CTU_REQUIRE(in_a && in_b, "%s: null segment", name);
+    CTU_REQUIRE(cp == 4 || cp == 8 || cp == 16, "%s: cp=%d per segment unsupported (4, 8 or 16)", name, cp);
+    CTU_REQUIRE(cs_b >= cp && cs_b % 4 == 0, "%s: bad stride of the second segment", name);
+    CTU_REQUIRE(((reinterpret_cast<uintptr_t>(in_a) | reinterpret_cast<uintptr_t>(in_b)) & 15) == 0,
+                "%s: segments must be 16-byte aligned", name);
+    CTU_REQUIRE(N > 0 && V > 0, "%s: empty volume", name);
+    int rc = fill_head(p, in_a, cs_a, 2 * cp, in_scale, in_shift, in_relu, w, bias, imap, Ci, Co, act, head_mode, N, V, name, cp);
+    if (rc != CTU_OK) return rc;
+    p.in_b = in_b; p.in_cs_b = cs_b;
     return CTU_OK;
 }
 
@@ -475,29 +525,65 @@
 }
 
 template <class T>
+int head_fwd_seg2_impl(const T* in_a, int cs_a, const T* in_b, int cs_b, int cp, const float* in_scale, const float* in_shift,
+                       int in_relu, const float* w, const float* bias, const int32_t* imap, int Ci, int Co, int act,
+                       int head_mode, float* out0, float* out1, int N, int64_t nvox_per_item, void* stream) {
+    HeadP p;
+    int rc = fill_head_seg2(p, in_a, cs_a, in_b, cs_b, cp, in_scale, in_shift, in_relu, w, bias, imap, Ci, Co, act, head_mode, N,
+                            nvox_per_item, "head_fwd_seg2");
+    if (rc != CTU_OK) return rc;
+    CTU_REQUIRE(out0 && (head_mode == 0 || out1), "head_fwd_seg2: null output");
+    const int nb = head_blocks((int64_t)N * nvox_per_item);
+    hipStream_t st = (hipStream_t)stream;
+    if (cp == 4) head_fwd_seg2_kernel<8, T><<<nb, HB, 0, st>>>(p, out0, out1);
+    else if (cp == 8) head_fwd_seg2_kernel<16, T><<<nb, HB, 0, st>>>(p, out0, out1);
+    else head_fwd_seg2_kernel<32, T><<<nb, HB, 0, st>>>(p, out0, out1);
+    CTU_CHECK_LAUNCH("head_fwd_seg2");
+    return CTU_OK;
+}
+
+template <class T>
 int head_bwd_impl(const T* in, int in_cs, int cin_p, const float* in_scale, const float* in_shift, int in_relu, const float* w,
                   const float* bias, const int32_t* imap, int Ci, int Co, int act, int head_mode, const float* g0, const float* g1,
                   T* gin, int gin_cs, float* dw, float* db, float* ws, int N, int64_t nvox_per_item, const float* bn_mean,
                   const float* bn_invstd, int bn_cp, float* bn_partials, const ctu_bn_bwd_tail* tail, void* stream, float gscale = 1.f,
-                  const float* gscale_dev = nullptr) {
+                  const float* gscale_dev = nullptr, const T* in_b = nullptr, int in_cs_b = 0, T* gin_b = nullptr,
+                  int gin_cs_b = 0) {
+    const bool seg2 = in_b != nullptr || gin_b != nullptr;
+    const int seg_cp = seg2 ? cin_p / 2 : cin_p;
     CTU_REQUIRE(!tail || (bn_partials && tail->gamma && tail->invstd && tail->dgamma && tail->dbeta && tail->coef &&
                           tail->C > 0 && tail->C <= bn_cp && tail->count > 0 && (!tail->running_mean || (tail->mean && tail->running_var))),
                 "head_bwd: incomplete BatchNorm tail");
     HeadP p;
-    int rc = fill_head(p, in, in_cs, cin_p, in_scale, in_shift, in_relu, w, bias, imap, Ci, Co, act, head_mode, N,
-                       nvox_per_item, "head_bwd");
+    int rc = seg2 ? fill_head_seg2(p, in, in_cs, in_b, in_cs_b, cin_p / 2, in_scale, in_shift, in_relu, w, bias, imap, Ci, Co, act,
+                                   head_mode, N, nvox_per_item, "head_bwd_seg2")
+                  : fill_head(p, in, in_cs, cin_p, in_scale, in_shift, in_relu, w, bias, imap, Ci, Co, act, head_mode, N,
+                              nvox_per_item, "head_bwd");
     if (rc != CTU_OK) return rc;
     p.gscale = gscale;
     p.gscale_dev = gscale_dev;
     CTU_REQUIRE(g0 && (head_mode == 0 || g1) && gin && dw && db && ws, "head_bwd: null pointer");
-    CTU_REQUIRE(gin_cs >= cin_p && gin_cs % 4 == 0, "head_bwd: bad gin stride");
+    CTU_REQUIRE(gin_cs >= seg_cp && gin_cs % 4 == 0, "head_bwd: bad gin stride");
+    CTU_REQUIRE(!seg2 || (gin_b && gin_cs_b >= seg_cp && gin_cs_b % 4 == 0), "head_bwd_seg2: bad second gradient segment");
+    CTU_REQUIRE(!seg2 || ((reinterpret_cast<uintptr_t>(gin) | reinterpret_cast<uintptr_t>(gin_b)) & 15) == 0,
+                "head_bwd_seg2: gradient segments must be 16-byte aligned");
     CTU_REQUIRE(!bn_partials || (bn_mean && bn_invstd && in_scale && in_relu && bn_cp > 0 && bn_cp % 4 == 0 && bn_cp <= cin_p),
                 "head_bwd: the BatchNorm reduction needs mean/invstd, a BN+ReLU input transform and bn_cp <= cin_p (bn_cp=%d)", bn_cp);
     const int nb = head_blocks((int64_t)N * nvox_per_item);
     hipStream_t st = (hipStream_t)stream;
     const int nfin = Co * Ci + Co + (tail ? 1 : 0);
     const ctu_bn_bwd_tail tl = bwd_tail_or_off(tail);
-    if (cin_p == 8) {
+    if (seg2) {
+        if (cin_p == 8)
+            head_bwd_q_seg2_kernel<8, T><<<nb, HB, 0, st>>>(p, g0, g1, gin, gin_cs, gin_b, gin_cs_b, ws, bn_mean, bn_invstd, bn_cp, bn_partials);
+        else if (cin_p == 16)
+            head_bwd_q_seg2_kernel<16, T><<<nb, HB, 0, st>>>(p, g0, g1, gin, gin_cs, gin_b, gin_cs_b, ws, bn_mean, bn_invstd, bn_cp, bn_partials);
+        else
+            head_bwd_q_seg2_kernel<32, T><<<nb, HB, 0, st>>>(p, g0, g1, gin, gin_cs, gin_b, gin_cs_b, ws, bn_mean, bn_invstd, bn_cp, bn_partials);
+        if (cin_p == 8) head_bwd_final_kernel<8><<<nfin, HB, 0, st>>>(ws, nb, Ci, Co, imap, dw, db, bn_partials, bn_cp, tl);
+        else if (cin_p == 16) head_bwd_final_kernel<16><<<nfin, HB, 0, st>>>(ws, nb, Ci, Co, imap, dw, db, bn_partials, bn_cp, tl);
+        else head_bwd_final_kernel<32><<<nfin, HB, 0, st>>>(ws, nb, Ci, Co, imap, dw, db, bn_partials, bn_cp, tl);
+    } else if (cin_p == 8) {
         head_bwd_q_kernel<8, T><<<nb, HB, 0, st>>>(p, g0, g1, gin, gin_cs, ws, bn_mean, bn_invstd, bn_cp, bn_partials);
         head_bwd_final_kernel<8><<<nfin, HB, 0, st>>>(ws, nb, Ci, Co, imap, dw, db, bn_partials, bn_cp, tl);
     } else if (cin_p == 16) {
@@ -572,6 +658,64 @@
                                                    bn_invstd, bn_cp, bn_partials, tail, stream, 1.f, gscale));
 }
 
+extern "C" int ctu_head_fwd_seg2(const float* in_a, int cs_a, const float* in_b, int cs_b, int cp, const float* in_scale,
+                                 const float* in_shift, int in_relu, const float* w, const float* bias, const int32_t* imap,
+                                 int Ci, int Co, int act, int head_mode, float* out0, float* out1, int N,
+                                 int64_t nvox_per_item, void* stream) {
+    return head_fwd_seg2_impl<float>(in_a, cs_a, in_b, cs_b, cp, in_scale, in_shift, in_relu, w, bias, imap, Ci, Co, act, head_mode,
+                                     out0, out1, N, nvox_per_item, stream);
+}
+extern "C" int ctu_lp_head_fwd_seg2(int dtype, const void* in_a, int cs_a, const void* in_b, int cs_b, int cp,
+                                    const float* in_scale, const float* in_shift, int in_relu, const float* w, const float* bias,
+                                    const int32_t* imap, int Ci, int Co, int act, int head_mode, float* out0, float* out1, int N,
+                                    int64_t nvox_per_item, void* stream) {
+    CTU_DISPATCH_LP(dtype, return head_fwd_seg2_impl<T>((const T*)in_a, cs_a, (const T*)in_b, cs_b, cp, in_scale, in_shift, in_relu, w,
+                                                        bias, imap, Ci, Co, act, head_mode, out0, out1, N, nvox_per_item, stream));
+}
+
+#define CTU_HEAD_SEG2_CHECK(name)                                                                       \
+    CTU_REQUIRE(in_a && in_b && gin_a && gin_b, name ": null segment");                                 \
+    CTU_REQUIRE(cp == 4 || cp == 8 || cp == 16, name ": cp=%d per segment unsupported (4, 8 or 16)", cp)
+
+extern "C" int ctu_head_bwd_bn_seg2(const float* in_a, int cs_a, const float* in_b, int cs_b, int cp, const float* in_scale,
+                                    const float* in_shift, int in_relu, const float* w, const float* bias, const int32_t* imap,
+                                    int Ci, int Co, int act, int head_mode, const float* g0, const float* g1, float* gin_a,
+                                    int gcs_a, float* gin_b, int gcs_b, float* dw, float* db, float* ws, int N,
+                                    int64_t nvox_per_item, const float* bn_mean, const float* bn_invstd, int bn_cp,
+                                    float* bn_partials, const ctu_bn_bwd_tail* tail, void* stream) {
+    CTU_HEAD_SEG2_CHECK("head_bwd_bn_seg2");
+    return head_bwd_impl<float>(in_a, cs_a, 2 * cp, in_scale, in_shift, in_relu, w, bias, imap, Ci, Co, act, head_mode, g0, g1, gin_a,
+                                gcs_a, dw, db, ws, N, nvox_per_item, bn_mean, bn_invstd, bn_cp, bn_partials, tail, stream, 1.f, nullptr,
+                                in_b, cs_b, gin_b, gcs_b);
+}
+extern "C" int ctu_lp_head_bwd_bn_seg2(int dtype, const void* in_a, int cs_a, const void* in_b, int cs_b, int cp,
+                                       const float* in_scale, const float* in_shift, int in_relu, const float* w, const float* bias,
+                                       const int32_t* imap, int Ci, int Co, int act, int head_mode, const float* g0,
+                                       const float* g1, void* gin_a, int gcs_a, void* gin_b, int gcs_b, float* dw, float* db,
+                                       float* ws, int N, int64_t nvox_per_item, const float* bn_mean, const float* bn_invstd,
+                                       int bn_cp, float* bn_partials, const ctu_bn_bwd_tail* tail, float gscale, void* stream) {
+    CTU_HEAD_SEG2_CHECK("lp_head_bwd_bn_seg2");
+    CTU_DISPATCH_LP(dtype, return head_bwd_impl<T>((const T*)in_a, cs_a, 2 * cp, in_scale, in_shift, in_relu, w, bias, imap, Ci, Co, act,
+                                                   head_mode, g0, g1, (T*)gin_a, gcs_a, dw, db, ws, N, nvox_per_item, bn_mean,
+                                                   bn_invstd, bn_cp, bn_partials, tail, stream, gscale, nullptr, (const T*)in_b,
+                                                   cs_b, (T*)gin_b, gcs_b));
+}
+extern "C" int ctu_lp_head_bwd_bn_dscale_seg2(int dtype, const void* in_a, int cs_a, const void* in_b, int cs_b, int cp,
+                                              const float* in_scale, const float* in_shift, int in_relu, const float* w,
+                                              const float* bias, const int32_t* imap, int Ci, int Co, int act, int head_mode,
+                                              const float* g0, const float* g1, void* gin_a, int gcs_a, void* gin_b, int gcs_b,
+                                              float* dw, float* db, float* ws, int N, int64_t nvox_per_item, const float* bn_mean,
+                                              const float* bn_invstd, int bn_cp, float* bn_partials, const ctu_bn_bwd_tail* tail,
+                                              const float* gscale, void* stream) {
+    CTU_HEAD_SEG2_CHECK("lp_head_bwd_bn_dscale_seg2");
+    CTU_REQUIRE(gscale, "lp_head_bwd_bn_dscale_seg2: null gscale");
+    CTU_DISPATCH_LP(dtype, return head_bwd_impl<T>((const T*)in_a, cs_a, 2 * cp, in_scale, in_shift, in_relu, w, bias, imap, Ci, Co, act,
+                                                   head_mode, g0, g1, (T*)gin_a, gcs_a, dw, db, ws, N, nvox_per_item, bn_mean,
+                                                   bn_invstd, bn_cp, bn_partials, tail, stream, 1.f, gscale, (const T*)in_b, cs_b,
+                                                   (T*)gin_b, gcs_b));
+}
+#undef CTU_HEAD_SEG2_CHECK
+
 extern "C" size_t ctu_loss_ws_floats(int N, int64_t V) {
     (void)V;
     return (size_t)N * LOSS_BX * 4 + (size_t)N * 2;
diff --git a/ct-unet_amd/ctunet_amd/_lib.py b/ct-unet_amd/ctunet_amd/_lib.py
--- a/ct-unet_amd/ctunet_amd/_lib.py
+++ b/ct-unet_amd/ctunet_amd/_lib.py
@@ -105,6 +105,8 @@
     "ctu_head_bwd": (I, [P, I, I, P, P, I, P, P, P, I, I, I, I, P, P, P, I, P, P, P, I, L, P]),
     "ctu_head_bwd_num_blocks": (I, [I, L]),
     "ctu_head_bwd_bn": (I, [P, I, I, P, P, I, P, P, P, I, I, I, I, P, P, P, I, P, P, P, I, L, P, P, I, P, P, P]),
+    "ctu_head_fwd_seg2": (I, [P, I, P, I, I, P, P, I, P, P, P, I, I, I, I, P, P, I, L, P]),
+    "ctu_head_bwd_bn_seg2": (I, [P, I, P, I, I, P, P, I, P, P, P, I, I, I, I, P, P, P, I, P, I, P, P, P, I, L, P, P, I, P, P, P]),
     "ctu_loss_ws_floats": (Z, [I, L]),
     "ctu_loss_fwd": (I, [P, P, I, L, F, F, I, P, P, P]),
     "ctu_loss_bwd": (I, [P, P, I, L, F, F, I, P, P, P, P, I, P]),
@@ -241,6 +243,9 @@
     "ctu_lp_head_fwd": (I, [I, P, I, I, P, P, I, P, P, P, I, I, I, I, P, P, I, L, P]),
     "ctu_lp_head_bwd_bn": (I, [I, P, I, I, P, P, I, P, P, P, I, I, I, I, P, P, P, I, P, P, P, I, L, P, P, I, P, P, F, P]),
     "ctu_lp_head_bwd_bn_dscale": (I, [I, P, I, I, P, P, I, P, P, P, I, I, I, I, P, P, P, I, P, P, P, I, L, P, P, I, P, P, P, P]),
+    "ctu_lp_head_fwd_seg2": (I, [I, P, I, P, I, I, P, P, I, P, P, P, I, I, I, I, P, P, I, L, P]),
+    "ctu_lp_head_bwd_bn_seg2": (I, [I, P, I, P, I, I, P, P, I, P, P, P, I, I, I, I, P, P, P, I, P, I, P, P, P, I, L, P, P, I, P, P, F, P]),
+    "ctu_lp_head_bwd_bn_dscale_seg2": (I, [I, P, I, P, I, I, P, P, I, P, P, P, I, I, I, I, P, P, P, I, P, I, P, P, P, I, L, P, P, I, P, P, P, P]),
     "ctu_scale_tensors": (I, [P, P, I, F, P, P]),
     "ctu_unscale_tensors": (I, [P, P, I, P, P, P]),
     "ctu_loss_scale_update": (I, [P, P, P, P, F, F, I, P]),
diff --git a/ct-unet_amd/ctunet_amd/engine.py b/ct-unet_amd/ctunet_amd/engine.py
--- a/ct-unet_amd/ctunet_amd/engine.py
+++ b/ct-unet_amd/ctunet_amd/engine.py
@@ -19,6 +19,13 @@
 LAZY_BN_LP = os.environ.get("CTUNET_LAZY_BN_LP", "0") != "0"
 BN_TAIL = os.environ.get("CTUNET_BN_TAIL", "0") != "0"
 DEFER_WGRAD_REDUCE = os.environ.get("CTUNET_DEFER_WGRAD_REDUCE", "1") != "0"
+SPLIT_CAT0 = os.environ.get("CTUNET_SPLIT_CAT0", "1") != "0"
+
+
+def _cat_halves(buf: torch.Tensor, cp: int):
+    if buf.dim() == 6:
+        return CL(buf[0], 0, cp), CL(buf[1], 0, cp)
+    return CL(buf, 0, cp), CL(buf, cp, cp)
 
 
 @dataclass
@@ -282,6 +289,7 @@
         cur = None if first_direct else ops.ncdhw_to_cl(x, dtype=adt)
         x_cl = cur
         cat: List[torch.Tensor] = []
+        halves = []
         xf: List[torch.Tensor] = []
         pooled: List[CL] = []
         dskip: List[CL] = []
@@ -292,7 +300,9 @@
         xf_off = 0
         for i, blk in enumerate(plan.enc):
             cp = pad8(blk.cout)
-            cat.append(torch.empty((n, dd, hh, ww, 2 * cp), dtype=adt, device=dev))
+            split = SPLIT_CAT0 and i == 0 and cp <= 16
+            cat.append(torch.empty((2, n, dd, hh, ww, cp) if split else (n, dd, hh, ww, 2 * cp), dtype=adt, device=dev))
+            halves.append(_cat_halves(cat[i], cp))
             xf.append(xf_all[xf_off:xf_off + 8 * cp].view(4, 2 * cp))
             xf_off += 8 * cp
             t1 = CL(torch.empty((n, dd, hh, ww, cp), dtype=adt, device=dev), 0, cp)
@@ -307,7 +317,7 @@
                                                           f"{blk.prefix}.{blk.first + 1}", blk.cin, blk.cout, imap, t1,
                                                           v1, training, n_upd, save)
             a2, recs[(blk.prefix, 2)] = self._conv_bn(P, a1, f"{blk.prefix}.{blk.first + 3}", f"{blk.prefix}.{blk.first + 4}",
-                                                      blk.cout, blk.cout, None, CL(cat[i], cp, cp), xf[i][:, cp:],
+                                                      blk.cout, blk.cout, None, halves[i][1], xf[i][:, cp:],
                                                       training, n_upd, save)
             dskip.append(a2)
             dd, hh, ww = dd // 2, hh // 2, ww // 2
@@ -358,17 +368,20 @@
                 a1, recs[(blk.prefix, 1)] = self._conv_bn(P, up, f"{blk.prefix}.1", f"{blk.prefix}.2", ct, blk.cout, None,
                                                           t1, v1, training, n_upd, save)
             a2, recs[(blk.prefix, 2)] = self._conv_bn(P, a1, f"{blk.prefix}.4", f"{blk.prefix}.5", blk.cout, blk.cout, None,
-                                                      CL(cat[i], 0, cp), xf[i][:, :cp], training, n_upd, save)
+                                                      halves[i][0], xf[i][:, :cp], training, n_upd, save)
+            h_dec, h_enc = halves[i]
             if plan.skip == "cat":
-                cur = CL(cat[i], 0, 2 * cp, xf[i][0], xf[i][1], True)
+                if cat[i].dim() == 6:
+                    cur = ops.CL2(h_dec, h_enc, xf[i][0], xf[i][1], True)
+                else:
+                    cur = CL(cat[i], 0, 2 * cp, xf[i][0], xf[i][1], True)
                 cur_segs = ((blk.cout, 0), (blk.cout, cp))
             elif plan.skip == "none":
-                cur = CL(cat[i], 0, cp, xf[i][0][:cp], xf[i][1][:cp], True)
+                cur = h_dec.with_xf(xf[i][0][:cp], xf[i][1][:cp])
                 cur_segs = ((blk.cout, 0),)
             else:
                 cur = CL(torch.empty((n, dd, hh, ww, cp), dtype=adt, device=dev), 0, cp)
-                ops.skip_add(CL(cat[i], 0, cp, xf[i][0][:cp], xf[i][1][:cp], True),
-                             CL(cat[i], cp, cp, xf[i][0][cp:], xf[i][1][cp:], True), cur)
+                ops.skip_add(h_dec.with_xf(xf[i][0][:cp], xf[i][1][:cp]), h_enc.with_xf(xf[i][0][cp:], xf[i][1][cp:]), cur)
                 cur_segs = ((blk.cout, 0),)
         imap_h, _ = self._maps(cur_segs, cur.cp, dev)
         wl, bl = P[plan.head + ".weight"], P[plan.head + ".bias"]
@@ -492,23 +505,26 @@
 
         cat, head_in = ctx["cat"], ctx["head_in"]
         gcat = [torch.empty_like(c) for c in cat]
+        ghalves = [_cat_halves(g, g.shape[-1] // (1 if g.dim() == 6 else 2)) for g in gcat]
         wl, bl = P[plan.head + ".weight"], P[plan.head + ".bias"]
         w2 = wl.detach().reshape(wl.shape[0], wl.shape[1])
         gsd = None if dyn is None else dyn.scale
         def g_skip_target(level: int) -> CL:
-            full = gcat[level].shape[-1]
-            return CL(gcat[level], 0, full if plan.skip == "cat" else full // 2)
+            g_dec, g_enc = ghalves[level]
+            if plan.skip != "cat":
+                return g_dec
+            return ops.CL2(g_dec, g_enc) if gcat[level].dim() == 6 else CL(gcat[level], 0, 2 * g_dec.cp)
 
         def g_skip_fanout(level: int):
             if plan.skip == "add":
-                half = gcat[level].shape[-1] // 2
-                ops.skip_add(CL(gcat[level], 0, half), None, CL(gcat[level], half, half))
+                ops.skip_add(ghalves[level][0], None, ghalves[level][1])
 
         r_last = recs[(plan.dec[-1].prefix, 2)]
         head_rows, head_fin = None, None
+        head_lo = head_in.a if isinstance(head_in, ops.CL2) else head_in
         if (POOL_BN and head_in.scale is not None and head_in.relu and head_in.scale.data_ptr() == r_last.vec[0].data_ptr()
-                and head_in.c0 == r_last.y.c0 and head_in.buf is r_last.y.buf):
-            fin = self._bwd_fin(P, r_last, head_in.buf.device)
+                and head_lo.c0 == r_last.y.c0 and head_lo.buf is r_last.y.buf):
+            fin = self._bwd_fin(P, r_last, dev)
             res = ops.head_bwd(head_in, w2, bl.detach(), ctx["imap_h"], plan.act, plan.head_mode, g0.contiguous(),
                                None if g1 is None else g1.contiguous(), g_skip_target(0), (r_last.vec, part), fin, gscale=gs,
                                gscale_dev=gsd)
@@ -528,7 +544,7 @@
             i = nlev - 1 - j
             cp = pad8(blk.cout)
             r1, r2 = recs[(blk.prefix, 1)], recs[(blk.prefix, 2)]
-            g_u2 = CL(gcat[i], 0, cp)
+            g_u2 = ghalves[i][0]
             g_u1 = CL(torch.empty_like(r1.y.buf), 0, cp)
             self._conv_bn_bwd(P, r2, g_u2, g_u1, grads, ws, part, head_rows if j == nlev - 1 else None,
                               head_fin if j == nlev - 1 else None)
@@ -583,7 +599,7 @@
             blk = plan.enc[i]
             cp = pad8(blk.cout)
             r1, r2 = recs[(blk.prefix, 1)], recs[(blk.prefix, 2)]
-            g_d2 = CL(gcat[i], cp, cp)
+            g_d2 = ghalves[i][1]
             dsk = ctx["dskip"][i]
             fuse = (POOL_BN and dsk.scale is not None and dsk.relu and dsk.scale.data_ptr() == r2.vec[0].data_ptr()
                     and ops.maxpool_bwd_bn_blocks(dsk.dims, dsk.cp) > 0)
diff --git a/ct-unet_amd/ctunet_amd/ops.py b/ct-unet_amd/ctunet_amd/ops.py
--- a/ct-unet_amd/ctunet_amd/ops.py
+++ b/ct-unet_amd/ctunet_amd/ops.py
@@ -281,6 +281,34 @@
 
     def with_xf(self, scale, shift, relu=True) -> "CL":
         return CL(self.buf, self.c0, self.cp, scale, shift, relu)
+
+
+@dataclass
+class CL2:
+    a: CL
+    b: CL
+    scale: Optional[torch.Tensor] = None
+    shift: Optional[torch.Tensor] = None
+    relu: bool = False
+
+    def __post_init__(self):
+        assert self.a.cp == self.b.cp and self.a.dims == self.b.dims and self.a.dtype == self.b.dtype
+        assert self.a.cp in (8, 16), "the two-segment head kernels take at most 16 channels per segment"
+
+    @property
+    def cp(self) -> int:
+        return 2 * self.a.cp
+
+    @property
+    def lp(self) -> int:
+        return self.a.lp
+
+    @property
+    def dims(self) -> Tuple[int, int, int, int]:
+        return self.a.dims
+
+    def seg_args(self):
+        return self.a.ptr, self.a.cs, self.b.ptr, self.b.cs
 
 
 def new_cl(n, d, h, w, cs, device, zero=False, dtype=torch.float32) -> torch.Tensor:
@@ -724,24 +752,26 @@
     return _query(lp(dtype), "convt2_wgrad_ws_floats", n, d, h, w, cin_p, cout_p)
 
 
-def head_fwd(x: CL, w: torch.Tensor, b: torch.Tensor, imap, act: int, head_mode: int):
+def head_fwd(x, w: torch.Tensor, b: torch.Tensor, imap, act: int, head_mode: int):
     n, d, h, w_ = x.dims
     co, ci = w.shape[0], w.shape[1]
     v = d * h * w_
-    dev = x.buf.device
+    dev = w.device
     if head_mode == 0:
         out0 = torch.empty((n, co, d, h, w_), dtype=torch.float32, device=dev)
         out1 = None
     else:
         out0 = torch.empty((n, 2, d, h, w_), dtype=torch.float32, device=dev)
         out1 = torch.empty((n, 2, d, h, w_), dtype=torch.float32, device=dev)
-    _dual(x.lp, "head_fwd", x.ptr, x.cs, x.cp, _ptr(x.scale), _ptr(x.shift), int(x.relu), w.data_ptr(), b.data_ptr(),
-          _ptr(imap), ci, co, act, head_mode, out0.data_ptr(), _ptr(out1), n, v, _stream())
+    seg2 = isinstance(x, CL2)
+    src = (*x.seg_args(), x.a.cp) if seg2 else (x.ptr, x.cs, x.cp)
+    _dual(x.lp, "head_fwd_seg2" if seg2 else "head_fwd", *src, _ptr(x.scale), _ptr(x.shift), int(x.relu), w.data_ptr(),
+          b.data_ptr(), _ptr(imap), ci, co, act, head_mode, out0.data_ptr(), _ptr(out1), n, v, _stream())
     return out0, out1
 
 
-def head_bwd(x: CL, w: torch.Tensor, b: torch.Tensor, imap, act: int, head_mode: int, g0: torch.Tensor,
-             g1: Optional[torch.Tensor], gin: CL, bn=None, fin=None, gscale: float = 1.0,
+def head_bwd(x, w: torch.Tensor, b: torch.Tensor, imap, act: int, head_mode: int, g0: torch.Tensor,
+             g1: Optional[torch.Tensor], gin, bn=None, fin=None, gscale: float = 1.0,
              gscale_dev: Optional[torch.Tensor] = None):
     assert gscale == 1.0 or x.lp, "gscale is the 16-bit path's loss scale"
     assert gscale_dev is None or (x.lp and gscale_dev.is_cuda and gscale_dev.dtype == torch.float32), \
@@ -749,7 +779,9 @@
     n, d, h, w_ = x.dims
     co, ci = w.shape[0], w.shape[1]
     v = d * h * w_
-    dev = x.buf.device
+    dev = w.device
+    seg2 = isinstance(x, CL2)
+    assert seg2 == isinstance(gin, CL2), "head_bwd: input and input gradient are both one buffer or both two segments"
     lib = _lib.load()
     ws = torch.empty(lib.ctu_head_bwd_ws_floats(n, v, x.cp, co), dtype=torch.float32, device=dev)
     dw = torch.empty_like(w)
@@ -767,8 +799,12 @@
     entry, scale = "head_bwd_bn", ((float(gscale),) if x.lp else ())
     if gscale_dev is not None:
         entry, scale = "head_bwd_bn_dscale", (gscale_dev.data_ptr(),)
-    _dual(x.lp, entry, x.ptr, x.cs, x.cp, _ptr(x.scale), _ptr(x.shift), int(x.relu), w.data_ptr(), b.data_ptr(), _ptr(imap),
-          ci, co, act, head_mode, g0.data_ptr(), _ptr(g1), gin.ptr, gin.cs, dw.data_ptr(), db.data_ptr(), ws.data_ptr(), n, v,
+    if seg2:
+        entry, src, dst = entry + "_seg2", (*x.seg_args(), x.a.cp), gin.seg_args()
+    else:
+        src, dst = (x.ptr, x.cs, x.cp), (gin.ptr, gin.cs)
+    _dual(x.lp, entry, *src, _ptr(x.scale), _ptr(x.shift), int(x.relu), w.data_ptr(), b.data_ptr(), _ptr(imap),
+          ci, co, act, head_mode, g0.data_ptr(), _ptr(g1), *dst, dw.data_ptr(), db.data_ptr(), ws.data_ptr(), n, v,
           *bn_args, _tail_arg(tail), *scale, _stream())
     if bn is None:
         return dw, db
diff --git a/include/ctunet_hip.h b/include/ctunet_hip.h
--- a/include/ctunet_hip.h
+++ b/include/ctunet_hip.h
@@ -202,6 +202,16 @@
                     const float* g0, const float* g1, float* gin, int gin_cs,
                     float* dw, float* db, float* ws, int N, int64_t nvox_per_item,
                     const float* bn_mean, const float* bn_invstd, int bn_cp, float* bn_partials, const ctu_bn_bwd_tail* tail, void* stream);
+int ctu_head_fwd_seg2(const float* in_a, int cs_a, const float* in_b, int cs_b, int cp, const float* in_scale,
+                      const float* in_shift, int in_relu, const float* w, const float* bias, const int32_t* imap,
+                      int Ci, int Co, int act, int head_mode, float* out0, float* out1, int N,
+                      int64_t nvox_per_item, void* stream);
+int ctu_head_bwd_bn_seg2(const float* in_a, int cs_a, const float* in_b, int cs_b, int cp, const float* in_scale,
+                         const float* in_shift, int in_relu, const float* w, const float* bias, const int32_t* imap,
+                         int Ci, int Co, int act, int head_mode, const float* g0, const float* g1, float* gin_a,
+                         int gcs_a, float* gin_b, int gcs_b, float* dw, float* db, float* ws, int N,
+                         int64_t nvox_per_item, const float* bn_mean, const float* bn_invstd, int bn_cp,
+                         float* bn_partials, const ctu_bn_bwd_tail* tail, void* stream);
 
 size_t ctu_loss_ws_floats(int N, int64_t V);
 int ctu_loss_fwd(const float* pred, const float* target, int N, int64_t V, float ce_lambda,
@@ -545,6 +555,23 @@
                               float* db, float* ws, int N, int64_t nvox_per_item, const float* bn_mean,
                               const float* bn_invstd, int bn_cp, float* bn_partials, const ctu_bn_bwd_tail* tail,
                               const float* gscale, void* stream);
+int ctu_lp_head_fwd_seg2(int dtype, const void* in_a, int cs_a, const void* in_b, int cs_b, int cp,
+                         const float* in_scale, const float* in_shift, int in_relu, const float* w, const float* bias,
+                         const int32_t* imap, int Ci, int Co, int act, int head_mode, float* out0, float* out1, int N,
+                         int64_t nvox_per_item, void* stream);
+int ctu_lp_head_bwd_bn_seg2(int dtype, const void* in_a, int cs_a, const void* in_b, int cs_b, int cp,
+                            const float* in_scale, const float* in_shift, int in_relu, const float* w, const float* bias,
+                            const int32_t* imap, int Ci, int Co, int act, int head_mode, const float* g0,
+                            const float* g1, void* gin_a, int gcs_a, void* gin_b, int gcs_b, float* dw, float* db,
+                            float* ws, int N, int64_t nvox_per_item, const float* bn_mean, const float* bn_invstd,
+                            int bn_cp, float* bn_partials, const ctu_bn_bwd_tail* tail, float gscale, void* stream);
+int ctu_lp_head_bwd_bn_dscale_seg2(int dtype, const void* in_a, int cs_a, const void* in_b, int cs_b, int cp,
+                                   const float* in_scale, const float* in_shift, int in_relu, const float* w,
+                                   const float* bias, const int32_t* imap, int Ci, int Co, int act, int head_mode,
+                                   const float* g0, const float* g1, void* gin_a, int gcs_a, void* gin_b, int gcs_b,
+                                   float* dw, float* db, float* ws, int N, int64_t nvox_per_item, const float* bn_mean,
+                                   const float* bn_invstd, int bn_cp, float* bn_partials, const ctu_bn_bwd_tail* tail,
+                                   const float* gscale, void* stream);
 int ctu_scale_tensors(void* const* ptrs, const int64_t* sizes, int n, float s, float* nonfinite_flag, void* stream);
 int ctu_unscale_tensors(void* const* ptrs, const int64_t* sizes, int n, const float* scale, float* found_inf, void* stream);
 int ctu_loss_scale_update(float* scale, int32_t* growth_tracker, float* found_inf, float* skipped, float growth,
```

Result: faster. 710.9 million voxels/s (median of 6 runs) (+4.0%).
